# HKUST-Aerial-Robotics/MIND

Hardware: AMD Instinct MI355X
Metric: sim steps/sec (whole node) + scenario-tree nodes expanded/sec, AV2 demo scenes (higher is better)
Workload: dtype f32-class (bf16 hi+mid+lo split operands = 24 significand bits, six products, fp32 accumulate) pair kernel + ActorNet, f32 elsewhere in the predictor, f64 iLQR

## Files before the change

### include/mind_hip.h

```cpp
#ifndef MIND_HIP_H
#define MIND_HIP_H

#include <stddef.h>
#include <stdint.h>

#ifdef __cplusplus
extern "C" {
#endif

#define MIND_OK 0
#define MIND_EINVAL (-1)
#define MIND_ENOMEM (-2)
#define MIND_EHIP (-3)
#define MIND_ESTATE (-4)
#define MIND_ENOTFOUND (-5)

typedef struct mind_ctx mind_ctx;

int mind_ctx_create(int device, void *stream, mind_ctx **out);
int mind_ctx_destroy(mind_ctx *ctx);
const char *mind_last_error_string(mind_ctx *ctx);
int mind_ctx_synchronize(mind_ctx *ctx);

typedef struct {
// ... 31 lines not shown

int mind_predict_batch(mind_ctx *ctx, const mind_scene_batch *in, mind_pred_out *out);

typedef struct {
  float *cov_vel;
  float *param;
} mind_pred_aux;
int mind_predict_batch_aux(mind_ctx *ctx, const mind_scene_batch *in, mind_pred_out *out, const mind_pred_aux *aux);

#define MIND_BASIS_BEZIER 0
#define MIND_BASIS_MONOMIAL 1
int mind_set_decoder_basis(mind_ctx *ctx, int basis);
int mind_get_decoder_basis(mind_ctx *ctx);

#define MIND_CURVE_MAX_POINTS (1LL << 26)
int mind_curve_eval(mind_ctx *ctx, int basis, const float *param, long long n_rows, const double *tau, int n_tau,
                    float *reg, float *vel, float *cov_vel);
int mind_debug_curve_basis(int basis, const double *tau, int n_tau, float *T, float *Tp);

int mind_last_fusion_stats(mind_ctx *ctx, int *n_launches, float *total_ms, double *pairs_processed);
int mind_last_actor_stats(mind_ctx *ctx, int *layerwise, int *n_launches, int *n_chunks, float *total_ms);
int mind_last_token_stats(mind_ctx *ctx, int *layerwise, int *n_launches, int *n_chunks, float *total_ms);
int mind_last_token_stage_ms(mind_ctx *ctx, float *out_ms, int cap);
int mind_last_ilqr_stats(mind_ctx *ctx, float *kernel_ms, int *n_trees, int *workgroups_per_tree);
int mind_last_ilqr_profile(mind_ctx *ctx, double *out9);
int mind_last_ilqr_trace(mind_ctx *ctx, int tree, int phase, double *out, int cap_rows, int *n_rows);
int mind_set_profiling(mind_ctx *ctx, int enable);
int mind_debug_launch_times(mind_ctx *ctx, int kind, float *clock_ms, float *event_ms, int cap, int *n_clock, int *n_event);
int mind_debug_launch_clock(int n_blocks, int block_slots, int rate_khz, const long long *ops, int n_ops, const unsigned long long *stamps,
                            long long n_slots, double *out, int cap);

#define MIND_PAIR_F32 0
#define MIND_PAIR_BF16X3 1
#define MIND_PAIR_BF16 2
#define MIND_PAIR_BF16X6 3
int mind_set_pair_precision(mind_ctx *ctx, int mode);

int mind_set_tuning(mind_ctx *ctx, const char *name, int value);
int mind_get_pair_precision(mind_ctx *ctx);
int mind_debug_pack_bfrag(const float *w, int row_stride, uint32_t *out);

int mind_debug_pair_schedule(const int *scene_tokens, const int *scene_actors, int n_scenes, int n_cu, int last_layer, int *out_jobs, int cap,
                             int *out_info);

int mind_debug_predict_choice(const char *const *knob_names, const int *knob_values, int n_knobs, int pair_prec, int n_cu, int have_side,
                              const int *scene_actors, const int *scene_lanes, int n_scenes, long long *out, int cap);

int mind_debug_ilqr_plan(const char *const *knob_names, const int *knob_values, int n_knobs, int n_cu, int mode, int n_trees, const int *n_nodes,
                         const int32_t *parents, long long *out, int cap, int *bad);

int mind_debug_aime_book(int pred_len, int max_depth, int max_rounds, int n_agents, int world, int rank, int force, int n_rounds, const int *dec_len,
                         const float *dec, int n_tokens, int bytes_per_pair, int plan_chunk_mb, int per_scene, long long *out, int cap, char *msg,
                         int msg_cap);

int mind_debug_wait_word(const unsigned *word, unsigned want, double timeout_s, double (*clock)(void *user), void *user, int spins_per_look);

int mind_debug_actor_lw_plan(int n_actors, int np, int chunk, long long *out_launches, int cap, long long *out_info);

int mind_debug_token_lw_plan(int n_tokens, int mode, int chunk, long long *out_launches, int cap, long long *out_info);

int mind_debug_pack_conv_frag(const float *w, int co, int ci, int ksz, uint32_t *out, size_t cap);

int mind_debug_pack(const char *what, const float *w, int a, int b, int c, float *out, size_t cap);
int mind_debug_weight_image(const mind_tensor_desc *tensors, int n_tensors, float *blob, size_t blob_cap, char *names, size_t names_cap,
                            long long *entries, int entries_cap, long long *out_info, char *msg, int msg_cap);
int mind_debug_weight_bind(const mind_tensor_desc *tensors, int n_tensors, const char *drop, char *msg, int msg_cap);

int mind_debug_trig(mind_ctx *ctx, const double *x, int n, double *out);

int mind_debug_set_layers(mind_ctx *ctx, int n);
int64_t mind_debug_read(mind_ctx *ctx, const char *name, float *host, int64_t max_floats);

typedef struct {
  int n_nodes;
  const int32_t *parent;
  const float *prob;
  int n_agents;
  const float *agent_mean;
  const float *agent_cov;
  const double *field;
  const double *node_w;
} mind_cost_tree;

typedef struct {
  double dt, wheelbase;
  double w_des_state[6];
  double w_state_con[6];
  double state_lower[6], state_upper[6];
  double w_ctrl[2];
  double w_tgt, w_ego, w_ego_cov_offset, w_exo, w_exo_cov_offset, w_exo_cost_offset;
  double grid_res; int grid_w, grid_h;
  int max_iter;
} mind_ilqr_cfg;

typedef struct { int iterations; int converged; double J; double mu; } mind_ilqr_stats;

int mind_ilqr_solve_trees(mind_ctx *ctx, const mind_ilqr_cfg *cfg, const mind_cost_tree *trees,
                          int n_trees, const double *x0, const double *target_lane, int n_lane_pts,
                          double target_vel, int use_exo, const double *us_init, double *xs,
                          double *us, mind_ilqr_stats *stats);

int mind_ilqr_contingency(mind_ctx *ctx, const mind_ilqr_cfg *cfg_warm, const mind_ilqr_cfg *cfg_full,
                          const mind_cost_tree *trees, int n_trees, const double *x0,
                          const double *target_lane, int n_lane_pts, double target_vel, double *xs,
                          double *us, mind_ilqr_stats *stats_warm, mind_ilqr_stats *stats_full);
int mind_ilqr_contingency_begin(mind_ctx *ctx, const mind_ilqr_cfg *cfg_warm, const mind_ilqr_cfg *cfg_full,
// ... 339 lines not shown
```

### mind_amd/_lib.py

```python
import ctypes as C
import os

_HERE = os.path.dirname(os.path.abspath(__file__))
LIB_PATH = os.environ.get("MIND_HIP_LIB", os.path.join(_HERE, "libmind_hip.so"))

WAIT_CLOCK = C.CFUNCTYPE(C.c_double, C.c_void_p)
MIND_OK = 0
MIND_EINVAL, MIND_ENOMEM, MIND_EHIP, MIND_ESTATE, MIND_ENOTFOUND = -1, -2, -3, -4, -5


class TensorDesc(C.Structure):
    _fields_ = [("name", C.c_char_p), ("data", C.POINTER(C.c_float)), ("numel", C.c_int64)]


class SceneBatch(C.Structure):
    _fields_ = [("n_scenes", C.c_int), ("actor_off", C.POINTER(C.c_int32)), ("lane_off", C.POINTER(C.c_int32)),
                ("actors", C.c_void_p), ("lanes", C.c_void_p), ("lane_feat", C.c_void_p),
                ("actor_ctrs", C.c_void_p), ("actor_vecs", C.c_void_p), ("lane_ctrs", C.c_void_p),
                ("lane_vecs", C.c_void_p), ("rpe", C.POINTER(C.c_void_p)), ("tgt_nodes", C.c_void_p),
                ("tgt_rpe", C.c_void_p)]


class PredOut(C.Structure):
    _fields_ = [("cls", C.c_void_p), ("reg", C.c_void_p), ("vel", C.c_void_p), ("lane_feat", C.c_void_p),
# ... 139 lines not shown

class LoopDesc(C.Structure):
    _fields_ = [("n_tracks", C.c_int), ("n_steps", C.c_int), ("clamp_last", C.c_int), ("ego_state", C.c_void_p), ("ego_state_is_f32", C.c_int), ("ego_obs", C.c_void_p), ("ego_trig32", C.c_void_p),
                ("tan_fn", C.c_void_p), ("sincos_fn", C.c_void_p), ("exo_obs", C.c_void_p),
                ("exo_valid", C.c_void_p), ("timestep", C.c_void_p), ("type_slot", C.c_void_p),
                ("sim_step", C.c_double), ("plan_step", C.c_double), ("enable_time", C.c_double),
                ("wheelbase", C.c_double), ("max_speed", C.c_double), ("max_steer", C.c_double), ("max_acc", C.c_double), ("max_dec", C.c_double),
                ("n_lanes", C.c_int), ("lane_pts", C.c_void_p), ("lane_flags", C.c_void_p),
                ("n_lane_pts", C.c_int), ("target_lane", C.c_void_p), ("target_lane_info", C.c_void_p),
                ("time_ahead", C.c_double), ("min_vel", C.c_float), ("dist_thres", C.c_float), ("max_depth", C.c_int), ("max_rounds", C.c_int),
                ("pred_len", C.c_int), ("prob_floor", C.c_float),
                ("cfg_warm", C.c_void_p), ("cfg_full", C.c_void_p), ("solve_n_lane_pts", C.c_int), ("solve_lane", C.c_void_p), ("target_vel", C.c_double),
                ("eval_n_lane_pts", C.c_int), ("eval_lane_is_f32", C.c_int), ("eval_lane", C.c_void_p), ("speculative", C.c_int)]


class LoopTotals(C.Structure):
    _fields_ = [("plans", C.c_longlong), ("expansions", C.c_longlong), ("scen_trees", C.c_longlong), ("rounds", C.c_longlong),
                ("aime_s", C.c_double), ("ilqr_s", C.c_double), ("total_s", C.c_double),
                ("iterations", C.c_longlong), ("node_iterations", C.c_longlong), ("node_iterations_exo", C.c_longlong),
                ("warm_speculated", C.c_longlong), ("warm_hits", C.c_longlong),
                ("pair_ms", C.c_double), ("pair_launches", C.c_longlong), ("scene_n2", C.c_double), ("scene_n_a1", C.c_double),
                ("ilqr_ms", C.c_double), ("ilqr_launches", C.c_longlong), ("ilqr_trees", C.c_longlong), ("ilqr_workgroups_per_tree", C.c_int),
                ("ilqr_prof", C.c_double * 9), ("ilqr_node_steps", C.c_double)]


class LoopOut(C.Structure):
    _fields_ = [("planned", C.c_int), ("enabled", C.c_int), ("n_steps", C.c_longlong), ("n_plans", C.c_longlong), ("episode_steps", C.c_longlong),
                ("sim_time", C.c_double), ("last_trigger", C.c_double), ("state", C.c_double * 4), ("ctrl", C.c_double * 2),
                ("n_agents", C.c_int), ("n_trees", C.c_int), ("best", C.c_int), ("n_expanded", C.c_int), ("n_rounds", C.c_int), ("n_traj_nodes", C.c_int),
                ("costs", C.POINTER(C.c_double)), ("aime_s", C.c_double), ("ilqr_s", C.c_double), ("total_s", C.c_double),
                ("tot", LoopTotals)]


PLANNER_EGO_KEY = -(1 << 63)


class PlannerDesc(C.Structure):
    _fields_ = [("time_ahead", C.c_double), ("min_vel", C.c_float), ("dist_thres", C.c_float), ("max_depth", C.c_int), ("max_rounds", C.c_int),
                ("pred_len", C.c_int), ("prob_floor", C.c_float), ("cfg_warm", C.c_void_p), ("cfg_full", C.c_void_p), ("speculative", C.c_int),
                ("ego_type_slot", C.c_int)]


class PlannerOut(C.Structure):
    _fields_ = [("n_plans", C.c_longlong),
                ("n_agents", C.c_int), ("n_trees", C.c_int), ("best", C.c_int), ("n_expanded", C.c_int), ("n_rounds", C.c_int), ("n_traj_nodes", C.c_int),
                ("costs", C.POINTER(C.c_double)), ("ctrl", C.c_double * 2), ("aime_s", C.c_double), ("ilqr_s", C.c_double), ("total_s", C.c_double),
                ("tot", LoopTotals)]


EXPORTS = ["mind_ctx_create", "mind_ctx_destroy", "mind_last_error_string", "mind_ctx_synchronize",
           "mind_weights_load", "mind_predict_batch", "mind_last_fusion_stats", "mind_last_actor_stats", "mind_debug_actor_lw_plan", "mind_last_token_stats", "mind_last_token_stage_ms", "mind_debug_token_lw_plan", "mind_set_profiling", "mind_debug_launch_times", "mind_debug_launch_clock",
           "mind_ilqr_solve_trees", "mind_ilqr_contingency", "mind_ilqr_solve_fields", "mind_cost_eval", "mind_ilqr_score_trees", "mind_ilqr_gains", "mind_ilqr_policy_rollouts", "mind_lane_dist_field", "mind_aime_world", "mind_aime_rebase", "mind_debug_aime_decide", "mind_debug_set_layers",
           "mind_debug_read", "mind_set_pair_precision", "mind_get_pair_precision", "mind_debug_pack_bfrag", "mind_debug_pack_conv_frag", "mind_debug_pack", "mind_debug_weight_image", "mind_debug_weight_bind", "mind_debug_pair_schedule", "mind_debug_predict_choice", "mind_debug_ilqr_plan", "mind_debug_aime_book", "mind_set_tuning", "mind_last_ilqr_stats", "mind_aime_plan", "mind_last_ilqr_profile", "mind_eval_traj_trees", "mind_last_ilqr_trace", "mind_ilqr_contingency_begin", "mind_ilqr_finish", "mind_fill_tracks", "mind_ilqr_contingency_begin_plan", "mind_debug_trig", "mind_aime_plan_begin", "mind_aime_plan_poll", "mind_aime_plan_finish", "mind_ctx_busy", "mind_ilqr_finish_plan",
           "mind_set_exchange", "mind_last_exchange_stats", "mind_debug_wait_word",
           "mind_predict_batch_aux", "mind_set_decoder_basis", "mind_get_decoder_basis", "mind_curve_eval", "mind_debug_curve_basis",
           "mind_audit_plan", "mind_audit_episode", "mind_debug_box_clearance",
           "mind_forecast_score", "mind_debug_forecast_score",
           "mind_audit_road_plan", "mind_audit_road_episode", "mind_debug_road_margin",
           "mind_loop_create", "mind_loop_destroy", "mind_loop_reset", "mind_loop_advance", "mind_loop_state", "mind_loop_last_plan", "mind_loop_export",
           "mind_planner_create", "mind_planner_destroy", "mind_planner_reset", "mind_planner_observe", "mind_planner_set_lanes", "mind_planner_set_target_lane",
           "mind_planner_set_solve_lane", "mind_planner_set_eval_lane", "mind_planner_plan", "mind_planner_last_plan", "mind_planner_export"]

EXCHANGE_FN = C.CFUNCTYPE(C.c_int, C.c_void_p, C.c_int, C.c_void_p, C.c_void_p, C.c_int64)
XCHG_ALLGATHER, XCHG_ALLREDUCE, XCHG_ALLTOALLV = 0, 1, 2

_lib = None


def load():
    global _lib
    if _lib is not None:
        return _lib
    if not os.path.exists(LIB_PATH):
        raise ImportError(f"{LIB_PATH} is missing: the HIP extension must be built (hipcc --offload-arch=gfx950); "
                          "there is no CPU fallback for the product path")
    lib = C.CDLL(LIB_PATH)
    lib.mind_ctx_create.argtypes = [C.c_int, C.c_void_p, C.POINTER(C.c_void_p)]
    lib.mind_ctx_destroy.argtypes = [C.c_void_p]
    lib.mind_last_error_string.argtypes = [C.c_void_p]
    lib.mind_last_error_string.restype = C.c_char_p
    lib.mind_ctx_synchronize.argtypes = [C.c_void_p]
    lib.mind_weights_load.argtypes = [C.c_void_p, C.POINTER(TensorDesc), C.c_int]
    lib.mind_predict_batch.argtypes = [C.c_void_p, C.POINTER(SceneBatch), C.POINTER(PredOut)]
    lib.mind_predict_batch_aux.argtypes = [C.c_void_p, C.POINTER(SceneBatch), C.POINTER(PredOut), C.POINTER(PredAux)]
    lib.mind_set_decoder_basis.argtypes = [C.c_void_p, C.c_int]
    lib.mind_get_decoder_basis.argtypes = [C.c_void_p]
    lib.mind_curve_eval.argtypes = [C.c_void_p, C.c_int, C.c_void_p, C.c_longlong, C.POINTER(C.c_double), C.c_int, C.c_void_p, C.c_void_p, C.c_void_p]
    lib.mind_debug_curve_basis.argtypes = [C.c_int, C.POINTER(C.c_double), C.c_int, C.POINTER(C.c_float), C.POINTER(C.c_float)]
    lib.mind_last_fusion_stats.argtypes = [C.c_void_p, C.POINTER(C.c_int), C.POINTER(C.c_float), C.POINTER(C.c_double)]
    lib.mind_last_actor_stats.argtypes = [C.c_void_p, C.POINTER(C.c_int), C.POINTER(C.c_int), C.POINTER(C.c_int), C.POINTER(C.c_float)]
    lib.mind_debug_actor_lw_plan.argtypes = [C.c_int, C.c_int, C.c_int, C.POINTER(C.c_longlong), C.c_int, C.POINTER(C.c_longlong)]
    lib.mind_last_token_stats.argtypes = [C.c_void_p, C.POINTER(C.c_int), C.POINTER(C.c_int), C.POINTER(C.c_int), C.POINTER(C.c_float)]
    lib.mind_last_token_stage_ms.argtypes = [C.c_void_p, C.POINTER(C.c_float), C.c_int]
    lib.mind_debug_token_lw_plan.argtypes = [C.c_int, C.c_int, C.c_int, C.POINTER(C.c_longlong), C.c_int, C.POINTER(C.c_longlong)]
    lib.mind_set_profiling.argtypes = [C.c_void_p, C.c_int]
    lib.mind_debug_launch_times.argtypes = [C.c_void_p, C.c_int, C.POINTER(C.c_float), C.POINTER(C.c_float), C.c_int, C.POINTER(C.c_int), C.POINTER(C.c_int)]
    lib.mind_debug_launch_clock.argtypes = [C.c_int, C.c_int, C.c_int, C.POINTER(C.c_longlong), C.c_int, C.POINTER(C.c_ulonglong), C.c_longlong,
                                            C.POINTER(C.c_double), C.c_int]
    lib.mind_ilqr_solve_trees.argtypes = [C.c_void_p, C.POINTER(IlqrCfg), C.POINTER(CostTree), C.c_int,
                                          C.POINTER(C.c_double), C.POINTER(C.c_double), C.c_int, C.c_double, C.c_int,
                                          C.POINTER(C.c_double), C.POINTER(C.c_double), C.POINTER(C.c_double),
                                          C.POINTER(IlqrStats)]
    lib.mind_ilqr_contingency.argtypes = [C.c_void_p, C.POINTER(IlqrCfg), C.POINTER(IlqrCfg), C.POINTER(CostTree), C.c_int,
                                          C.POINTER(C.c_double), C.POINTER(C.c_double), C.c_int, C.c_double,
                                          C.POINTER(C.c_double), C.POINTER(C.c_double), C.POINTER(IlqrStats), C.POINTER(IlqrStats)]
    lib.mind_ilqr_contingency_begin.argtypes = [C.c_void_p, C.POINTER(IlqrCfg), C.POINTER(IlqrCfg), C.POINTER(CostTree), C.c_int,
                                          C.POINTER(C.c_double), C.POINTER(C.c_double), C.c_int, C.c_double,
                                          C.POINTER(C.c_double), C.POINTER(C.c_double), C.POINTER(IlqrStats), C.POINTER(IlqrStats)]
    lib.mind_ilqr_finish.argtypes = [C.c_void_p]
    lib.mind_ilqr_contingency_begin_plan.argtypes = [C.c_void_p, C.POINTER(IlqrCfg), C.POINTER(IlqrCfg), C.c_void_p, C.c_void_p, C.c_int, C.c_double,
                                                     C.c_void_p, C.c_void_p, C.c_void_p, C.c_void_p]
    lib.mind_fill_tracks.argtypes = [C.c_void_p, C.c_int, C.c_int, C.c_void_p, C.c_void_p, C.c_void_p, C.c_void_p, C.c_void_p, C.c_void_p]
    lib.mind_ilqr_solve_fields.argtypes = [C.c_void_p, C.POINTER(IlqrCfg), C.POINTER(FieldGrid), C.POINTER(CostTree), C.c_int,
                                           C.POINTER(C.c_double), C.POINTER(C.c_double), C.POINTER(C.c_double),
                                           C.POINTER(C.c_double), C.POINTER(IlqrStats)]
    lib.mind_cost_eval.argtypes = [C.c_void_p, C.POINTER(IlqrCfg), C.POINTER(FieldGrid), C.POINTER(CostTree),
                                   C.POINTER(C.c_double), C.POINTER(C.c_double), C.c_int, C.c_double, C.c_int, C.c_int,
                                   C.POINTER(C.c_int32), C.POINTER(C.c_double), C.POINTER(C.c_double), C.POINTER(C.c_double)]
    lib.mind_ilqr_score_trees.argtypes = [C.c_void_p, C.POINTER(IlqrCfg), C.POINTER(FieldGrid), C.POINTER(CostTree), C.c_int,
                                          C.POINTER(C.c_double), C.POINTER(C.c_double), C.c_int, C.c_double, C.c_int, C.c_int,
                                          C.POINTER(C.c_double), C.POINTER(C.c_double), C.POINTER(C.c_double), C.POINTER(C.c_double)]
    lib.mind_ilqr_gains.argtypes = [C.c_void_p, C.POINTER(IlqrCfg), C.POINTER(FieldGrid), C.POINTER(CostTree), C.c_int,
                                    C.POINTER(C.c_double), C.POINTER(C.c_double), C.c_int, C.c_double, C.c_int,
                                    C.POINTER(C.c_double), C.POINTER(C.c_double), C.POINTER(IlqrGainsOut)]
    lib.mind_ilqr_policy_rollouts.argtypes = [C.c_void_p, C.POINTER(IlqrCfg), C.POINTER(FieldGrid), C.POINTER(CostTree), C.c_int,
                                              C.POINTER(C.c_double), C.POINTER(C.c_double), C.c_int, C.c_double, C.c_int,
                                              C.POINTER(C.c_double), C.POINTER(C.c_double), C.POINTER(C.c_double), C.c_int,
                                              C.POINTER(C.c_double), C.POINTER(C.c_double), C.POINTER(C.c_double), C.POINTER(C.c_double),
                                              C.POINTER(C.c_double), C.POINTER(C.c_double)]
    lib.mind_lane_dist_field.argtypes = [C.c_void_p, C.POINTER(C.c_double), C.POINTER(C.c_double), C.c_int, C.c_int, C.c_int,
                                         C.c_double] + [C.POINTER(C.c_double)] * 4
    lib.mind_aime_world.argtypes = [C.c_void_p, C.POINTER(WorldIn), C.POINTER(WorldOut)]
    lib.mind_aime_rebase.argtypes = [C.c_void_p, C.POINTER(RebaseIn), C.POINTER(RebaseOut)]
    lib.mind_debug_aime_decide.argtypes = [C.c_void_p, C.c_int, C.POINTER(C.c_int32), C.POINTER(C.c_int32), C.c_void_p, C.POINTER(C.c_float), C.c_void_p,
                                           C.c_void_p, C.c_void_p, C.c_int, C.c_float, C.c_float, C.c_int, C.c_int, C.c_void_p, C.c_void_p, C.c_void_p]
    lib.mind_aime_plan.argtypes = [C.c_void_p, C.POINTER(AimePlanIn), C.POINTER(AimePlanOut)]
    lib.mind_aime_plan_begin.argtypes = [C.c_void_p, C.POINTER(AimePlanIn)]
    lib.mind_aime_plan_poll.argtypes = [C.c_void_p]
    lib.mind_aime_plan_finish.argtypes = [C.c_void_p, C.POINTER(AimePlanOut)]
    lib.mind_ctx_busy.argtypes = [C.c_void_p]
    lib.mind_ilqr_finish_plan.argtypes = [C.c_void_p, C.c_int, C.c_int, C.c_void_p, C.c_void_p, C.c_void_p, C.c_void_p]
    lib.mind_set_pair_precision.argtypes = [C.c_void_p, C.c_int]
    lib.mind_set_tuning.argtypes = [C.c_void_p, C.c_char_p, C.c_int]
    lib.mind_last_ilqr_stats.argtypes = [C.c_void_p, C.POINTER(C.c_float), C.POINTER(C.c_int), C.POINTER(C.c_int)]
    lib.mind_last_ilqr_profile.argtypes = [C.c_void_p, C.POINTER(C.c_double)]
    lib.mind_last_ilqr_trace.argtypes = [C.c_void_p, C.c_int, C.c_int, C.POINTER(C.c_double), C.c_int, C.POINTER(C.c_int)]
    lib.mind_eval_traj_trees.argtypes = [C.POINTER(C.c_double), C.POINTER(C.c_double), C.POINTER(C.c_int32), C.c_int, C.c_void_p, C.c_int, C.c_int,
                                         C.c_double, C.POINTER(C.c_double)]
    lib.mind_get_pair_precision.argtypes = [C.c_void_p]
    lib.mind_debug_pack_bfrag.argtypes = [C.POINTER(C.c_float), C.c_int, C.POINTER(C.c_uint32)]
    lib.mind_debug_pair_schedule.argtypes = [C.POINTER(C.c_int), C.POINTER(C.c_int), C.c_int, C.c_int, C.c_int, C.POINTER(C.c_int), C.c_int, C.POINTER(C.c_int)]
    lib.mind_debug_predict_choice.argtypes = [C.POINTER(C.c_char_p), C.POINTER(C.c_int), C.c_int, C.c_int, C.c_int, C.c_int, C.POINTER(C.c_int), C.POINTER(C.c_int),
                                              C.c_int, C.POINTER(C.c_longlong), C.c_int]
    lib.mind_debug_ilqr_plan.argtypes = [C.POINTER(C.c_char_p), C.POINTER(C.c_int), C.c_int, C.c_int, C.c_int, C.c_int, C.POINTER(C.c_int), C.POINTER(C.c_int32),
                                         C.POINTER(C.c_longlong), C.c_int, C.POINTER(C.c_int)]
    lib.mind_debug_wait_word.argtypes = [C.POINTER(C.c_uint), C.c_uint, C.c_double, WAIT_CLOCK, C.c_void_p, C.c_int]
    lib.mind_debug_aime_book.argtypes = [C.c_int] * 8 + [C.POINTER(C.c_int), C.POINTER(C.c_float)] + [C.c_int] * 4 + [C.POINTER(C.c_longlong), C.c_int, C.c_char_p, C.c_int]
    lib.mind_debug_trig.argtypes = [C.c_void_p, C.POINTER(C.c_double), C.c_int, C.POINTER(C.c_double)]
    lib.mind_debug_pack_conv_frag.argtypes = [C.POINTER(C.c_float), C.c_int, C.c_int, C.c_int, C.POINTER(C.c_uint32), C.c_size_t]
    lib.mind_debug_pack.argtypes = [C.c_char_p, C.POINTER(C.c_float), C.c_int, C.c_int, C.c_int, C.POINTER(C.c_float), C.c_size_t]
    lib.mind_debug_weight_image.argtypes = [C.POINTER(TensorDesc), C.c_int, C.POINTER(C.c_float), C.c_size_t, C.c_char_p, C.c_size_t,
                                            C.POINTER(C.c_longlong), C.c_int, C.POINTER(C.c_longlong), C.c_char_p, C.c_int]
    lib.mind_debug_weight_bind.argtypes = [C.POINTER(TensorDesc), C.c_int, C.c_char_p, C.c_char_p, C.c_int]
    lib.mind_debug_set_layers.argtypes = [C.c_void_p, C.c_int]
    lib.mind_debug_read.argtypes = [C.c_void_p, C.c_char_p, C.POINTER(C.c_float), C.c_int64]
    lib.mind_set_exchange.argtypes = [C.c_void_p, C.c_int, C.c_int, EXCHANGE_FN, C.c_void_p, C.c_int]
    lib.mind_last_exchange_stats.argtypes = [C.c_void_p, C.POINTER(C.c_longlong), C.POINTER(C.c_longlong)]
    lib.mind_loop_create.argtypes = [C.c_void_p, C.POINTER(LoopDesc), C.POINTER(C.c_void_p)]
    lib.mind_loop_destroy.argtypes = [C.c_void_p]
    lib.mind_loop_reset.argtypes = [C.c_void_p]
    lib.mind_loop_advance.argtypes = [C.c_void_p, C.c_int, C.c_double, C.c_longlong, C.POINTER(LoopOut)]
    lib.mind_loop_state.argtypes = [C.c_void_p, C.POINTER(LoopOut)]
    lib.mind_loop_last_plan.argtypes = [C.c_void_p, C.POINTER(AimePlanOut)] + [C.POINTER(C.c_void_p)] * 6 + [C.c_void_p]
    lib.mind_loop_export.argtypes = [C.c_void_p, C.c_int, C.POINTER(C.c_int), C.c_void_p, C.c_void_p, C.c_void_p]
    lib.mind_planner_create.argtypes = [C.c_void_p, C.POINTER(PlannerDesc), C.POINTER(C.c_void_p)]
    lib.mind_planner_destroy.argtypes = [C.c_void_p]
    lib.mind_planner_reset.argtypes = [C.c_void_p]
    lib.mind_planner_observe.argtypes = [C.c_void_p, C.c_int, C.c_void_p, C.c_int, C.c_void_p, C.c_void_p, C.c_void_p]
    lib.mind_planner_set_lanes.argtypes = [C.c_void_p, C.c_int, C.c_void_p, C.c_void_p]
    lib.mind_planner_set_target_lane.argtypes = [C.c_void_p, C.c_int, C.c_void_p, C.c_void_p]
    lib.mind_planner_set_solve_lane.argtypes = [C.c_void_p, C.c_int, C.c_void_p, C.c_double]
    lib.mind_planner_set_eval_lane.argtypes = [C.c_void_p, C.c_int, C.c_void_p, C.c_int]
    lib.mind_planner_plan.argtypes = [C.c_void_p, C.c_void_p, C.c_void_p, C.POINTER(PlannerOut)]
    lib.mind_planner_last_plan.argtypes = [C.c_void_p, C.POINTER(AimePlanOut)] + [C.POINTER(C.c_void_p)] * 6 + [C.c_void_p]
    lib.mind_planner_export.argtypes = [C.c_void_p, C.c_int, C.POINTER(C.c_int), C.c_void_p, C.c_void_p, C.c_void_p]
    lib.mind_audit_plan.argtypes = [C.c_void_p, C.POINTER(AuditBox), C.c_double, C.POINTER(CostTree), C.c_int, C.c_int, C.POINTER(C.c_double),
                                    C.POINTER(AuditPlanOut)]
    lib.mind_audit_episode.argtypes = [C.c_void_p, C.POINTER(AuditBox), C.c_int, C.c_int, C.c_int, C.POINTER(C.c_double), C.POINTER(C.c_double),
                                       C.POINTER(C.c_uint8), C.POINTER(C.c_double), C.POINTER(AuditEpisodeOut)]
    lib.mind_debug_box_clearance.argtypes = [C.c_int, C.c_int, C.POINTER(C.c_double), C.POINTER(C.c_double), C.POINTER(C.c_double), C.POINTER(C.c_double)]
    fc_tail = [C.POINTER(ForecastCfg), C.c_int, C.POINTER(C.c_int32), C.c_void_p, C.c_void_p, C.POINTER(C.c_double), C.POINTER(C.c_uint8),
               C.POINTER(C.c_uint8), C.POINTER(ForecastOut)]
    lib.mind_forecast_score.argtypes = [C.c_void_p] + fc_tail
    lib.mind_debug_forecast_score.argtypes = fc_tail
    road = [C.POINTER(C.c_double), C.POINTER(C.c_int32), C.c_int]
    lib.mind_audit_road_plan.argtypes = [C.c_void_p, C.POINTER(AuditBox)] + road + [C.POINTER(CostTree), C.c_int, C.c_int, C.POINTER(C.c_double),
                                                                                   C.POINTER(AuditRoadPlanOut)]
    lib.mind_audit_road_episode.argtypes = [C.c_void_p, C.POINTER(AuditBox)] + road + [C.c_int, C.c_int, C.POINTER(C.c_double),
                                                                                      C.POINTER(AuditRoadEpisodeOut)]
    lib.mind_debug_road_margin.argtypes = [C.c_int, C.POINTER(C.c_double), C.POINTER(AuditBox)] + road + [C.POINTER(C.c_double), C.POINTER(C.c_double)] + \
        [C.POINTER(C.c_int32)] * 3
    for n in EXPORTS:
        getattr(lib, n)
        if n not in ("mind_last_error_string", "mind_debug_read"):
            getattr(lib, n).restype = C.c_int
    lib.mind_debug_read.restype = C.c_int64
    _lib = lib
    return lib


# ... 282 lines not shown
```

### mind_amd/csrc/actor_mfma_kernels.hip

```cpp
#include <hip/hip_runtime.h>
#include <stdint.h>

#define AM_T 1024
#ifdef MIND_ACTOR_TRACE
__device__ long long am_tr_[64];
__device__ int am_trn_;
#define AM_MARK() do { if (blockIdx.x == 0 && threadIdx.x == 0) { const long long n_ = clock64(); am_tr_[am_trn_ & 63] = n_; ++am_trn_; } } while (0)
#else
#define AM_MARK() do {} while (0)
#endif
#define AM_WAVES 16
#define AM_MAXT 2
#define AM_RSD(C) (3 * (C) / 2 + 4)
#define AM_BUF 2496
#define AM_XIN 0
#define AM_O0 1344
#define AM_FA (AM_O0 + 7 * AM_BUF)
#define AM_RED (AM_FA + 48 * AM_RSD(128))
#define AM_LDS_DWORDS (AM_RED + 64)

#include "weight_tables.h"
#include "launch_clock.h"
typedef u32 u32x2 __attribute__((ext_vector_type(2)));

// ... 136 lines not shown
#pragma unroll
      for (int e = 0; e < 4; ++e) y[e] += (1.0f - l1) * a0[e] + l1 * a1[e];
    }
    if (relu) {
#pragma unroll
      for (int e = 0; e < 4; ++e) y[e] = fmaxf(y[e], 0.f);
    }
    if (gout) {
      if (t == Tout - 1) *(f32x4 *)(gout + co) = y;
    } else if (outf) {
      *(f32x4 *)(outf + t * 132 + co) = y;
    } else {
      am_store_split<NP>(outs + t * RSD + (co >> 1), PLANE, y);
    }
  }
  __syncthreads();
}

template <int NP, int LGCI, int LGCO, int STRIDE, bool DS>
__device__ __forceinline__ void am_res(const u32 *in, int Tin, const AmRes &W, u32 *out, u32 *t1, u32 *t2, float *red) {
  constexpr int Cout = 1 << LGCO;
  const int Tout = Tin / STRIDE;
  f32x4 acc[AM_MAXT];
  am_conv<NP, LGCI, 3, STRIDE>(in, Tin, W.c1, Cout, Tout, acc);
  AM_MARK();
  am_gn<NP>(acc, Cout, Tout, W.g1, W.b1, nullptr, nullptr, true, t1, nullptr, nullptr, red);
  AM_MARK();
  const u32 *resid = in;
  if (DS) {
    am_conv<NP, LGCI, 1, STRIDE>(in, Tin, W.ds, Cout, Tout, acc);
    AM_MARK();
    am_gn<NP>(acc, Cout, Tout, W.gd, W.bd, nullptr, nullptr, false, t2, nullptr, nullptr, red);
    AM_MARK();
    resid = t2;
  }
  am_conv<NP, LGCO, 3, 1>(t1, Tout, W.c2, Cout, Tout, acc);
  AM_MARK();
  am_gn<NP>(acc, Cout, Tout, W.g2, W.b2, resid, nullptr, true, out, nullptr, nullptr, red);
  AM_MARK();
}

template <int NP, int LGC>
__device__ __forceinline__ void am_lateral(const u32 *src, int T, const AmLat &W, const float *up, float *dstf, u32 *dsts,
                                           float *red) {
  f32x4 acc[AM_MAXT];
  am_conv<NP, LGC, 3, 1>(src, T, W.w, 128, T, acc);
  AM_MARK();
  am_gn<NP>(acc, 128, T, W.g, W.b, nullptr, up, false, dsts, dstf, nullptr, red);
  AM_MARK();
}

template <int NP>
__global__ __launch_bounds__(AM_T) void k_actor_mfma(const float *__restrict__ actors , int n_actors,
                                                     float *__restrict__ out , AmW W, LcSlot *clk) {
  lc_stamp_in(clk);
  extern __shared__ __attribute__((aligned(16))) u32 smu[];
  u32 *xin = smu + AM_XIN;
  u32 *o0 = smu + AM_O0, *o1 = o0 + AM_BUF, *o2 = o1 + AM_BUF, *o3 = o2 + AM_BUF;
  u32 *ta = o3 + AM_BUF, *tb = ta + AM_BUF, *tc = tb + AM_BUF;
  u32 *fa = smu + AM_FA;
  float *red = (float *)(smu + AM_RED);
  const int tid = threadIdx.x;
  const int a = blockIdx.x;
  if (a >= n_actors) { lc_stamp_both(clk); return; }
  if (tid < 48 * 8) {
    const int t = tid >> 3, c = (tid & 7) * 2;
    const float v0 = c < 14 ? actors[((size_t)a * 14 + c) * 48 + t] : 0.f;
    const float v1 = c + 1 < 14 ? actors[((size_t)a * 14 + c + 1) * 48 + t] : 0.f;
    u32 *p = xin + t * AM_RSD(16) + (c >> 1);
    const u32 h = pk_bf16(v0, v1);
    const float r0 = v0 - bf_lo_f32(h), r1 = v1 - bf_hi_f32(h);
    const u32 m = pk_bf16(r0, r1);
    p[0] = h; p[8] = m; p[16] = pk_bf16(r0 - bf_lo_f32(m), r1 - bf_hi_f32(m));
  }
  __syncthreads();
#ifdef MIND_ACTOR_TRACE
  if (blockIdx.x == 0 && tid == 0) am_trn_ = 0;
#endif
  AM_MARK();
  am_res<NP, 4, 5, 1, true>(xin, 48, W.res[0], ta, tb, tc, red);
  am_res<NP, 5, 5, 1, false>(ta, 48, W.res[1], o0, tb, tc, red);
  am_res<NP, 5, 6, 2, true>(o0, 48, W.res[2], ta, tb, tc, red);
  am_res<NP, 6, 6, 1, false>(ta, 24, W.res[3], o1, tb, tc, red);
  am_res<NP, 6, 7, 2, true>(o1, 24, W.res[4], ta, tb, tc, red);
  am_res<NP, 7, 7, 1, false>(ta, 12, W.res[5], o2, tb, tc, red);
  am_res<NP, 7, 8, 2, true>(o2, 12, W.res[6], ta, tb, tc, red);
  am_res<NP, 8, 8, 1, false>(ta, 6, W.res[7], o3, tb, tc, red);
  am_lateral<NP, 8>(o3, 6, W.lat[3], nullptr, (float *)ta, nullptr, red);
  am_lateral<NP, 7>(o2, 12, W.lat[2], (const float *)ta, (float *)tb, nullptr, red);
  am_lateral<NP, 6>(o1, 24, W.lat[1], (const float *)tb, (float *)o2, nullptr, red);
  am_lateral<NP, 5>(o0, 48, W.lat[0], (const float *)o2, nullptr, fa, red);
  {
    const AmRes &R = W.res[8];
    f32x4 acc[AM_MAXT];
    am_conv<NP, 7, 3, 1>(fa, 48, R.c1, 128, 48, acc);
    AM_MARK();
    am_gn<NP>(acc, 128, 48, R.g1, R.b1, nullptr, nullptr, true, o0, nullptr, nullptr, red);
    AM_MARK();
    am_conv<NP, 7, 3, 1>(o0, 48, R.c2, 128, 48, acc);
    AM_MARK();
    am_gn<NP>(acc, 128, 48, R.g2, R.b2, fa, nullptr, true, nullptr, nullptr, out + (size_t)a * 128, red);
    AM_MARK();
  }
#ifdef MIND_ACTOR_TRACE
  if (blockIdx.x == 0 && tid == 0) {
    printf("[k_actor_mfma<%d>] cycles conv/gn per stage:", NP);
    for (int q = 1; q < am_trn_ && q < 64; ++q) printf(" %lld", am_tr_[q] - am_tr_[q - 1]);
// ... 7 lines not shown
```

### mind_amd/csrc/aime_book.h

```cpp
#pragma once
#include <algorithm>
#include <cstddef>
#include <cstdint>
#include <cstring>
#include <vector>

#include "../../include/mind_hip.h"

constexpr int PL_K = 6;
constexpr int PL_OBS = 50;

struct PlScene {
  int node;
  float prob;
  int cur_t, end_t;
  float rot[4], orig[2], tgt[22];
};

struct PlNode {
  int round, scene, mode, parent, depth;
  int owner, lscene;
  float prob;
  int cur_t, end_t;
  bool branch, end, term, rebased;
  unsigned long long hit;
  float tgt[22];
};

inline void pl_block(int n, int r, int w, int &lo, int &hi) {
  const int base = n / w, rem = n % w;
  lo = r * base + (r < rem ? r : rem);
  hi = lo + base + (r < rem ? 1 : 0);
}
inline int pl_owner(int n, int w, int b) {
  for (int r = 0; r < w; ++r) { int lo, hi; pl_block(n, r, w, lo, hi); if (b >= lo && b < hi) return r; }
  return w - 1;
}

inline bool pl_exchanges(bool have_transport, int world, bool force) { return have_transport && (world > 1 || force); }

inline int pl_chunk(int n_tokens, int bytes_per_pair, int plan_chunk_mb, int Bk) {
  const double edge_mb = (double)n_tokens * (((n_tokens + 15) / 16) * 16) * bytes_per_pair / (1024.0 * 1024.0);
  return std::max(1, (int)std::min<double>((double)(Bk > 0 ? Bk : 1), (double)plan_chunk_mb / edge_mb));
}

typedef double (*pl_clock_fn)(void *user);
inline bool pl_wait_word(const volatile unsigned *word, unsigned want, double timeout_s, pl_clock_fn now, void *user, unsigned spins_per_look) {
  if (__atomic_load_n((const unsigned *)word, __ATOMIC_ACQUIRE) == want) return true;
  const double t0 = now(user);
  for (unsigned spins = 0;;) {
    if (__atomic_load_n((const unsigned *)word, __ATOMIC_ACQUIRE) == want) return true;
    if (++spins < spins_per_look) continue;
    spins = 0;
    if (now(user) - t0 > timeout_s) return false;
  }
}

enum { PL_OK = 0, PL_E_ROUNDS, PL_E_ROOT, PL_E_TRIMMED, PL_E_AGAIN, PL_E_ORDER, PL_E_NO_END };
struct PlErr { int code = PL_OK, a0 = 0, a1 = 0; explicit operator bool() const { return code != PL_OK; } };
inline const char *pl_err_format(int code) {
  switch (code) {
    case PL_E_ROUNDS: return "unsupported: more than %d AIME rounds";
    case PL_E_ROOT: return "unsupported: the root is a branching candidate";
// ... 75 lines not shown
};

struct PlGeom { int B, lo, hi, Bk, Bmax; };

struct PlRound {
  std::vector<int> todo;
  std::vector<int> cnt_r, s0_r;
  std::vector<int> win;
  int S = 0, s0 = 0, Sm = 0;
};

struct AimeBook {
  int HZ = 0, max_depth = 0, a = 0, XW = 1, XR = 0;
  bool dist = false;
  int n_rounds = 0;
  std::vector<PlNode> nodes;
  std::vector<int> leaves;
  std::vector<PlScene> batch;
  PlRound rec;
  std::vector<mind_aime_node> table;
  int64_t n_rows = 0;
  JobTable gather, flat;
  std::vector<int32_t> tree_top, tree_off, flat_parent;
  std::vector<float> flat_prob;
  std::vector<int> cand, queue, last, stack;
  std::vector<std::vector<int>> kids;
  std::vector<float> pr;

  AimeBook() {}
  AimeBook(int pred_len, int max_depth_, int n_agents, int world, int rank, bool dist_) { reset(pred_len, max_depth_, n_agents, world, rank, dist_); }

  void reset(int pred_len, int max_depth_, int n_agents, int world, int rank, bool dist_) {
    HZ = pred_len; max_depth = max_depth_; a = n_agents; XW = world; XR = rank; dist = dist_;
    n_rounds = 0;
    nodes.assign(1, PlNode());
    PlNode &r = nodes[0];
    memset(&r, 0, sizeof(r));
    r.round = -1; r.parent = -1; r.prob = 1.f; r.end_t = HZ; r.branch = true;
    leaves.assign(1, 0);
    batch.assign(1, PlScene());
    PlScene &s = batch[0];
    s.node = 0; s.prob = 1.f; s.cur_t = 0; s.end_t = HZ;
    tree_top.clear();
  }

  PlErr begin_round(int max_rounds, PlGeom &g) const {
    PlErr e;
    if (n_rounds >= max_rounds) { e.code = PL_E_ROUNDS; e.a0 = max_rounds; return e; }
    g.B = (int)batch.size();
    pl_block(g.B, XR, XW, g.lo, g.hi);
    g.Bk = g.hi - g.lo;
    g.Bmax = (g.B + XW - 1) / XW;
    return e;
  }

  static int flags_of(const PlNode &n) { return (n.branch ? MIND_AIME_BRANCH : 0) | (n.end ? MIND_AIME_END : 0) | (n.term ? MIND_AIME_TERMINATE : 0); }
  int root_flags() const { return flags_of(nodes[0]); }

  PlErr round(const float *h_dec, int Bmax) {
    PlErr err;
    const int B = (int)batch.size(), round = n_rounds;
    const size_t n_back = (size_t)Bmax * 6 * 4;
    for (int b = 0; b < B; ++b) {
      const int owner = dist ? pl_owner(B, XW, b) : 0;
      int olo, ohi;
      pl_block(B, owner, XW, olo, ohi);
      if (!dist) { olo = 0; }
      const float *h_sel = h_dec + (size_t)owner * n_back, *h_selp = h_sel + (size_t)Bmax * 6;
      const unsigned *h_hit = (const unsigned *)(h_selp + (size_t)Bmax * 6);
      const int bl = b - olo;
      for (int j = 0; j < PL_K; ++j) {
        const int k = (int)h_sel[(size_t)bl * 6 + j];
        if (k < 0) continue;
        PlNode n;
        memset(&n, 0, sizeof(n));
        n.round = round; n.scene = b; n.mode = k; n.parent = batch[b].node; n.depth = nodes[n.parent].depth + 1;
        n.owner = owner; n.lscene = bl;
        n.prob = h_selp[(size_t)bl * 6 + j]; n.cur_t = batch[b].cur_t; n.end_t = batch[b].end_t;
        n.hit = (unsigned long long)h_hit[2 * ((size_t)bl * 6 + j)] | ((unsigned long long)h_hit[2 * ((size_t)bl * 6 + j) + 1] << 32);
        memcpy(n.tgt, batch[b].tgt, sizeof(n.tgt));
        const int idx = (int)nodes.size();
        nodes.push_back(n);
        for (size_t q = 0; q < leaves.size(); ++q)
          if (leaves[q] == n.parent) { leaves.erase(leaves.begin() + q); break; }
        leaves.push_back(idx);
      }
    }
    n_rounds += 1;
    std::vector<int> &todo = rec.todo;
    cand.clear(); todo.clear();
    for (int li : leaves) {
      PlNode &n = nodes[li];
      if (n.branch) { n.branch = false; n.term = true; }
      else if (!n.end) {
        if (n.depth >= max_depth) n.term = true;
        else cand.push_back(li);
      }
    }
    for (int li : cand) {
      PlNode &n = nodes[li];
      if (li == 0) { err.code = PL_E_ROOT; return err; }
      if (n.rebased && n.cur_t > 0) { err.code = PL_E_TRIMMED; return err; }
      int t_b = n.end_t;
      for (int t = n.cur_t + 1 + (n.cur_t + 1) % 2; t < n.end_t; t += 2)
        if ((n.hit >> t) & 1ull) { t_b = t; break; }
      if (t_b < n.end_t) n.end_t = t_b;
      if (t_b < HZ) todo.push_back(li);
      else n.end = true;
    }
    const int S = rec.S = (int)todo.size();
    rec.cnt_r.assign(XW, 0); rec.s0_r.assign(XW + 1, 0); rec.win.clear();
    rec.s0 = rec.Sm = 0;
    if (todo.empty()) return err;
    for (int li : todo)
      if (nodes[li].round != round) { err.code = PL_E_AGAIN; err.a0 = nodes[li].round; err.a1 = round + 1; return err; }
    for (int s = 0; s < S; ++s) {
      if (s > 0 && nodes[todo[s]].scene < nodes[todo[s - 1]].scene) { err.code = PL_E_ORDER; return err; }
      rec.cnt_r[nodes[todo[s]].owner] += 1;
    }
    for (int r = 0; r < XW; ++r) rec.s0_r[r + 1] = rec.s0_r[r] + rec.cnt_r[r];
    const int s0 = rec.s0 = rec.s0_r[XR], Sm = rec.Sm = rec.cnt_r[XR];
    rec.win.resize(3 * (size_t)Sm);
    for (int s = 0; s < Sm; ++s) {
      const PlNode &n = nodes[todo[s0 + s]];
      rec.win[s] = n.scene;
      rec.win[Sm + s] = n.lscene * a * PL_K + n.mode;
      rec.win[2 * Sm + s] = n.end_t - n.cur_t;
    }
    batch.assign(S, PlScene());
    for (int s = 0; s < S; ++s) {
      PlNode &n = nodes[todo[s]];
      n.branch = true; n.rebased = true;
      PlScene &sc = batch[s];
      sc.node = todo[s]; sc.prob = n.prob; sc.cur_t = n.end_t; sc.end_t = HZ;
    }
    return err;
  }

  PlErr finish() {
    PlErr err;
    bool any_end = false;
    for (int li : leaves) any_end |= nodes[li].end;
    if (!any_end) { err.code = PL_E_NO_END; return err; }
    for (int li : leaves) {
      if (!nodes[li].end) continue;
      for (int q = li; q > 0; q = nodes[q].parent) nodes[q].end = true;
    }
    const int N = (int)nodes.size() - 1;
    table.assign(N, mind_aime_node());
    gather.clear(); flat.clear();
    n_rows = 0;
    for (int i = 0; i < N; ++i) {
      const PlNode &n = nodes[i + 1];
      mind_aime_node &p = table[i];
      p.round = n.round; p.scene = n.scene; p.mode = n.mode; p.parent = n.parent - 1; p.prob = n.prob; p.cur_t = n.cur_t; p.end_t = n.end_t;
      p.flags = flags_of(n);
      memcpy(p.tgt_pts, n.tgt, sizeof(p.tgt_pts));
      p.dur = 0; p.row_off = -1;
      if (n.end) {
        const int dur = n.end_t - n.cur_t;
        p.dur = dur; p.row_off = n_rows;
        if (dur > 0 && (!dist || n.owner == XR))
          gather.add({n.lscene * a * PL_K + n.mode, dur, (int)n_rows, a}, n.round);
        n_rows += (int64_t)a * dur * 3;
      }
    }
    if (kids.size() < nodes.size()) kids.resize(nodes.size());
    for (size_t i = 0; i < nodes.size(); ++i) kids[i].clear();
    for (int i = 1; i < (int)nodes.size(); ++i) kids[nodes[i].parent].push_back(i);
    tree_top.clear(); tree_off.assign(1, 0); flat_parent.clear(); flat_prob.clear();
    for (int top : kids[0]) {
      if (!nodes[top].end) continue;
      pr.assign(nodes.size(), 0.f);
      pr[top] = 1.f;
      queue.assign(1, top);
      for (size_t qh = 0; qh < queue.size(); ++qh) {
        const int cur = queue[qh];
        float total = 0.f;
        for (int ch : kids[cur]) if (nodes[ch].end) total = total + nodes[ch].prob;
        for (int ch : kids[cur]) if (nodes[ch].end) { pr[ch] = nodes[ch].prob / total * pr[cur]; queue.push_back(ch); }
// ... 30 lines not shown
```

### mind_amd/csrc/aime_kernels.hip

```cpp
#include <hip/hip_runtime.h>
#include <stdint.h>

struct AimeScene {
  int a0, a1;
  int last, cmp;
  float r00, r01, r10, r11;
  float ox, oy, theta_g, pad2;
};

#define AIME_SMALL 8
struct AimeSmall {
  AimeScene s[AIME_SMALL];
  float prob[AIME_SMALL];
  int n, a, pad0, pad1;
};

#define AIME_T 60
#define AIME_K 6
#define AIME_PK 6

__device__ __forceinline__ void aime_to_world(float lx, float ly, float c, float s, float cx, float cy, const AimeScene &S,
                                              bool translate, float &wx, float &wy) {
  float ax = lx * c + ly * (-s), ay = lx * s + ly * c;
  if (translate) { ax += cx; ay += cy; }
  wx = ax * S.r00 + ay * S.r01;
  wy = ax * S.r10 + ay * S.r11;
  if (translate) { wx += S.ox; wy += S.oy; }
}

__global__ __launch_bounds__(64) void k_aime_world(const AimeScene *__restrict__ scenes, const int *__restrict__ agent_scene,
                                                   const float *__restrict__ reg, const float *__restrict__ vel,
                                                   const float *__restrict__ ctrs, const float *__restrict__ vecs,
                                                   const float *__restrict__ cov_last, float *__restrict__ world,
                                                   float *__restrict__ topo, float *__restrict__ ego_end,
                                                   const float *__restrict__ lane, int n_lane, const AimeSmall sm) {
  const int i = blockIdx.x / AIME_K, k = blockIdx.x % AIME_K, t = threadIdx.x;
  const int b = sm.n ? i / sm.a : agent_scene[i];
  const AimeScene S = sm.n ? sm.s[b] : scenes[b];
  const bool live = t < AIME_T;
  const int tc = live ? t : AIME_T - 1;
  const float th = atan2f(vecs[2 * i + 1], vecs[2 * i]);
  const float c = cosf(th), s = sinf(th);
  const size_t e = ((size_t)i * AIME_K + k) * AIME_T + tc;
  const float lx = reg[e * 5], ly = reg[e * 5 + 1], sgx = reg[e * 5 + 2], sgy = reg[e * 5 + 3];
  const float lvx = vel[e * 2], lvy = vel[e * 2 + 1];
  float wx, wy, wvx, wvy;
  aime_to_world(lx, ly, c, s, ctrs[2 * i], ctrs[2 * i + 1], S, true, wx, wy);
  aime_to_world(lvx, lvy, c, s, 0.f, 0.f, S, false, wvx, wvy);
  const float ang = atan2f(lvy, lvx) + th + S.theta_g;
  const float cv = fmaxf(sgx, sgy) + cov_last[i];
  if (live) {
    float *w = world + e * AIME_PK;
    w[0] = wx; w[1] = wy; w[2] = wvx; w[3] = wvy; w[4] = ang; w[5] = cv;
  }
// ... 90 lines not shown
    int best = -1, brank = AIME_K;
    float bp = 0.f;
    unsigned brow = 0;
#pragma unroll
    for (int k = 0; k < AIME_K; ++k)
      if (((alive >> k) & 1u) && rank[k] < brank) {
        best = k; brank = rank[k]; bp = pr[k];
        unsigned row = 0;
#pragma unroll
        for (int j = 0; j < AIME_K; ++j) {
          const int lo = k < j ? k : j, hi = k < j ? j : k;
          if (j != k && ((mask >> (lo * AIME_K + hi)) & 1u)) row |= 1u << j;
        }
        brow = row;
      }
    if (best >= 0) {
#pragma unroll
      for (int q = 0; q < AIME_K; ++q) if (q == ns) { so[q] = (float)best; po[q] = bp; }
      ++ns;
      alive &= brow;
    }
  }
}

__global__ __launch_bounds__(64) void k_aime_select(const AimeScene *__restrict__ scenes, const float *__restrict__ cls,
                                                    const float *__restrict__ scen_prob, const float *__restrict__ topo,
                                                    const float *__restrict__ ego_end, int lane_check, float dist_thres,
                                                    float *__restrict__ sel, float *__restrict__ sel_prob, float prob_floor, const AimeSmall sm) {
  const int b = blockIdx.x, t = threadIdx.x;
  const AimeScene S = sm.n ? sm.s[b] : scenes[b];
  const float sp = sm.n ? sm.prob[b] : scen_prob[b];
  float so[AIME_K], po[AIME_K];
  aime_select_scene(S, sp, b, t, cls, topo, ego_end, lane_check, dist_thres, prob_floor, so, po);
  if (t != 0) return;
#pragma unroll
  for (int k = 0; k < AIME_K; ++k) { sel[(size_t)b * AIME_K + k] = so[k]; sel_prob[(size_t)b * AIME_K + k] = po[k]; }
}

#define RB_THREADS 256
#define RB_FEAT_BLOCKS(a) ((int)(((size_t)(a) * 48 + RB_THREADS - 1) / RB_THREADS))
#define RB_T 50
#define RB_LANE_LDS 1024

struct RebaseArgs {
  int a, l, n_lane, pad_ones;
  const float *pos, *ang, *vel;
  const float *types;
  const float *pad;
  const float *lane_ctrs0, *lane_vecs0;
  const float *tlane, *tinfo;
  float time_ahead, min_vel;
  float *actors, *actor_ctrs, *actor_vecs, *lane_ctrs, *lane_vecs, *tgt_nodes, *tgt_rpe, *frames;
  float travel0;
};

__device__ __forceinline__ void rb_cs(float ax, float ay, float bx, float by, float &c, float &s) {
  const float den = sqrtf(ax * ax + ay * ay) * sqrtf(bx * bx + by * by) + 1e-10f;
  c = (ax * bx + ay * by) / den;
  s = (ax * by - ay * bx) / den;
}

__global__ __launch_bounds__(64) void k_aime_windows(const float *__restrict__ prev_pos, const float *__restrict__ prev_ang,
                                                     const float *__restrict__ prev_vel, const float *__restrict__ rows,
                                                     const int *__restrict__ parent_slot, const int *__restrict__ row0,
                                                     const int *__restrict__ dur, int a, float *__restrict__ pos,
                                                     float *__restrict__ ang, float *__restrict__ vel, int row_stride,
                                                     float *__restrict__ cov_last) {
  const int s = blockIdx.x / a, i = blockIdx.x - s * a, t = threadIdx.x;
  if (t >= RB_T) return;
  const int d = dur[s];
  const int src = t + d;
  float x, y, vx, vy, h;
  if (src < RB_T) {
    const size_t p = ((size_t)parent_slot[s] * a + i) * RB_T + src;
    x = prev_pos[2 * p]; y = prev_pos[2 * p + 1]; vx = prev_vel[2 * p]; vy = prev_vel[2 * p + 1]; h = prev_ang[p];
  } else {
    const float *r = rows + (((size_t)row0[s] + (size_t)i * row_stride) * AIME_T + (src - RB_T)) * AIME_PK;
    x = r[0]; y = r[1]; vx = r[2]; vy = r[3]; h = r[4];
    if (cov_last && t == RB_T - 1) cov_last[(size_t)s * a + i] = r[5];
  }
  const size_t o = ((size_t)s * a + i) * RB_T + t;
  pos[2 * o] = x; pos[2 * o + 1] = y; vel[2 * o] = vx; vel[2 * o + 1] = vy; ang[o] = h;
}

struct AimeDone { unsigned *cnt; unsigned *h_gen; unsigned gen; };
__device__ __forceinline__ void aime_decisions_done(const AimeDone D) {
  if (!D.h_gen) return;
  __threadfence_system();
  const unsigned prev = __hip_atomic_fetch_add(D.cnt, 1u, __ATOMIC_ACQ_REL, __HIP_MEMORY_SCOPE_AGENT);
  if (prev + 1u != gridDim.x) return;
  __hip_atomic_store(D.cnt, 0u, __ATOMIC_RELAXED, __HIP_MEMORY_SCOPE_AGENT);
  __threadfence_system();
  __hip_atomic_store(D.h_gen, D.gen, __ATOMIC_RELEASE, __HIP_MEMORY_SCOPE_SYSTEM);
}

__global__ __launch_bounds__(64) void k_aime_branch(const AimeScene *__restrict__ scenes, const float *__restrict__ sel,
                                                    const float *__restrict__ world, unsigned *__restrict__ hit,
                                                    const float *__restrict__ sel_prob, float *__restrict__ h_sel, float *__restrict__ h_selp,
                                                    unsigned *__restrict__ h_hit, const AimeSmall sm, const AimeDone done) {
  const int b = blockIdx.x / AIME_K, j = blockIdx.x % AIME_K, t = threadIdx.x;
  const AimeScene S = sm.n ? sm.s[b] : scenes[b];
  const int k = (int)sel[(size_t)b * AIME_K + j];
  bool h = false;
  if (k >= 0 && t < AIME_T) {
    for (int i = S.a0; i < S.a1; ++i) {
      const float *r = world + ((size_t)i * AIME_K + k) * AIME_T * AIME_PK;
      h |= (r[t * AIME_PK + 5] / r[S.cmp * AIME_PK + 5]) > 9.0f;
    }
  }
  const unsigned long long m = __ballot(h);
  if (t == 0) { hit[2 * (size_t)blockIdx.x] = (unsigned)m; hit[2 * (size_t)blockIdx.x + 1] = (unsigned)(m >> 32); }
  if (h_sel && t == 0) {
    h_hit[2 * (size_t)blockIdx.x] = (unsigned)m; h_hit[2 * (size_t)blockIdx.x + 1] = (unsigned)(m >> 32);
    h_sel[blockIdx.x] = sel[blockIdx.x]; h_selp[blockIdx.x] = sel_prob[blockIdx.x];
    aime_decisions_done(done);
  }
}

__global__ __launch_bounds__(64) void k_aime_select_branch(const AimeScene *__restrict__ scenes, const float *__restrict__ cls,
                                                           const float *__restrict__ scen_prob, const float *__restrict__ topo,
                                                           const float *__restrict__ ego_end, int lane_check, float dist_thres, float prob_floor,
                                                           const float *__restrict__ world, float *__restrict__ sel, float *__restrict__ sel_prob,
                                                           unsigned *__restrict__ hit, float *__restrict__ h_sel, float *__restrict__ h_selp,
                                                           unsigned *__restrict__ h_hit, const AimeSmall sm, const AimeDone done) {
  const int b = blockIdx.x / AIME_K, j = blockIdx.x % AIME_K, t = threadIdx.x;
  const AimeScene S = sm.n ? sm.s[b] : scenes[b];
  const float sp = sm.n ? sm.prob[b] : scen_prob[b];
  float so[AIME_K], po[AIME_K];
  aime_select_scene(S, sp, b, t, cls, topo, ego_end, lane_check, dist_thres, prob_floor, so, po);
  float kf = -1.f, pj = 0.f;
#pragma unroll
  for (int q = 0; q < AIME_K; ++q) if (q == j) { kf = so[q]; pj = po[q]; }
  const int k = (int)kf;
  bool h = false;
  if (k >= 0 && t < AIME_T) {
    for (int i0 = S.a0; i0 < S.a1; i0 += 8) {
      float num[8], den[8];
#pragma unroll
      for (int q = 0; q < 8; ++q) {
        const int i = i0 + q < S.a1 ? i0 + q : S.a1 - 1;
        const float *r = world + ((size_t)i * AIME_K + k) * AIME_T * AIME_PK;
        num[q] = r[t * AIME_PK + 5]; den[q] = r[S.cmp * AIME_PK + 5];
      }
#pragma unroll
      for (int q = 0; q < 8; ++q) if (i0 + q < S.a1) h |= (num[q] / den[q]) > 9.0f;
    }
  }
  const unsigned long long m = __ballot(h);
  if (t == 0) {
    hit[2 * (size_t)blockIdx.x] = (unsigned)m; hit[2 * (size_t)blockIdx.x + 1] = (unsigned)(m >> 32);
    sel[blockIdx.x] = kf; sel_prob[blockIdx.x] = pj;
    if (h_sel) {
      h_hit[2 * (size_t)blockIdx.x] = (unsigned)m; h_hit[2 * (size_t)blockIdx.x + 1] = (unsigned)(m >> 32);
      h_sel[blockIdx.x] = kf; h_selp[blockIdx.x] = pj;
      aime_decisions_done(done);
    }
  }
}

struct AimeGather { int row0, dur, dst, a; };
__global__ __launch_bounds__(64) void k_aime_gather(const AimeGather *__restrict__ jobs, const int *__restrict__ job_of_block,
                                                    const int *__restrict__ agent_of_block, const float *const *__restrict__ world_of_job,
                                                    float *__restrict__ out) {
  const AimeGather J = jobs[job_of_block[blockIdx.x]];
  const int i = agent_of_block[blockIdx.x], t = threadIdx.x;
  if (t >= J.dur) return;
  const float *r = world_of_job[job_of_block[blockIdx.x]] + (((size_t)J.row0 + (size_t)i * AIME_K) * AIME_T + t) * AIME_PK;
  float *o = out + (size_t)J.dst + ((size_t)i * J.dur + t) * 3;
  o[0] = r[0]; o[1] = r[1]; o[2] = r[5];
}

struct AimeFlat { int row0, n, dst, a; };
__global__ __launch_bounds__(64) void k_aime_flat(const AimeFlat *__restrict__ jobs, const int *__restrict__ job_of_block,
                                                  const int *__restrict__ agent_of_block, const float *const *__restrict__ world_of_job,
                                                  float *__restrict__ mean, float *__restrict__ cov) {
  const AimeFlat J = jobs[job_of_block[blockIdx.x]];
  const int i = agent_of_block[blockIdx.x], m = threadIdx.x;
  if (m >= J.n) return;
  const float *r = world_of_job[job_of_block[blockIdx.x]] + (((size_t)J.row0 + (size_t)i * AIME_K) * AIME_T + 2 * m) * AIME_PK;
  const size_t o = (size_t)(J.dst + m) * J.a + i;
  mean[2 * o] = r[0]; mean[2 * o + 1] = r[1];
  cov[o] = r[5];
}

__global__ void k_repeat_rows(const float *__restrict__ src, size_t n, int times, float *__restrict__ dst) {
  const size_t i = (size_t)blockIdx.x * blockDim.x + threadIdx.x;
  if (i >= n * (size_t)times) return;
  dst[i] = src[i % n];
}

__global__ __launch_bounds__(RB_THREADS) void k_aime_rebase(RebaseArgs A) {
  const int sc = blockIdx.x, tid = threadIdx.x;
  const int a = A.a;
  extern __shared__ float rb_sm[];
  __shared__ float fr[8];
  __shared__ float rdv[RB_THREADS];
  __shared__ int rdi[RB_THREADS];
  __shared__ int s_idx;
  __shared__ float ctr[11][2];
  const float *pos = A.pos + (size_t)sc * a * RB_T * 2;
  const float *ang = A.ang + (size_t)sc * a * RB_T;
  const float *vel = A.vel + (size_t)sc * a * RB_T * 2;
  if (tid == 0) {
    const float th = ang[RB_T - 1];
    fr[0] = pos[(RB_T - 1) * 2]; fr[1] = pos[(RB_T - 1) * 2 + 1]; fr[2] = th; fr[3] = cosf(th); fr[4] = sinf(th);
  }
  __syncthreads();
  const float ox = fr[0], oy = fr[1], th0 = fr[2], c0 = fr[3], s0 = fr[4];
  for (int i = tid; i < a; i += RB_THREADS) {
    const float dx = pos[(i * RB_T + RB_T - 1) * 2] - ox, dy = pos[(i * RB_T + RB_T - 1) * 2 + 1] - oy;
    const float cx = dx * c0 + dy * s0, cy = dx * (-s0) + dy * c0;
    const float thi = ang[i * RB_T + RB_T - 1] - th0;
    const float ci = cosf(thi), si = sinf(thi);
    float *o = rb_sm + 5 * i;
    o[0] = cx; o[1] = cy; o[2] = thi; o[3] = ci; o[4] = si;
    if (blockIdx.y == 0) {
      A.actor_ctrs[((size_t)sc * a + i) * 2] = cx; A.actor_ctrs[((size_t)sc * a + i) * 2 + 1] = cy;
      A.actor_vecs[((size_t)sc * a + i) * 2] = ci; A.actor_vecs[((size_t)sc * a + i) * 2 + 1] = si;
    }
  }
  __syncthreads();
  const int fb = (int)blockIdx.y - 1, nfb = (int)gridDim.y - 1;
  for (int e = (nfb > 0 ? fb * RB_THREADS : 0) + tid; nfb > 0 ? (fb >= 0 && e < min(a * 48, (fb + 1) * RB_THREADS)) : e < a * 48; e += RB_THREADS) {
    const int i = e / 48, t = e % 48 + 2;
    const float *f = rb_sm + 5 * i;
    float pn[2][2];
#pragma unroll
    for (int q = 0; q < 2; ++q) {
      const int tt = t - 1 + q;
      const float dx = pos[(i * RB_T + tt) * 2] - ox, dy = pos[(i * RB_T + tt) * 2 + 1] - oy;
      const float x1 = (dx * c0 + dy * s0) - f[0], y1 = (dx * (-s0) + dy * c0) - f[1];
      pn[q][0] = x1 * f[3] + y1 * f[4];
      pn[q][1] = x1 * (-f[4]) + y1 * f[3];
    }
    const float an = (ang[i * RB_T + t] - th0) - f[2];
    const float vx0 = vel[(i * RB_T + t) * 2], vy0 = vel[(i * RB_T + t) * 2 + 1];
    const float vx1 = vx0 * c0 + vy0 * s0, vy1 = vx0 * (-s0) + vy0 * c0;
    float *o = A.actors + ((size_t)sc * a + i) * 14 * 48 + (t - 2);
    o[0 * 48] = pn[1][0] - pn[0][0];
    o[1 * 48] = pn[1][1] - pn[0][1];
    o[2 * 48] = cosf(an);
    o[3 * 48] = sinf(an);
    o[4 * 48] = vx1 * f[3] + vy1 * f[4];
    o[5 * 48] = vx1 * (-f[4]) + vy1 * f[3];
#pragma unroll
    for (int k = 0; k < 7; ++k) o[(6 + k) * 48] = A.types[(i * RB_T + t) * 7 + k];
// ... 184 lines not shown
```

### mind_amd/csrc/aime_plan.hip

```cpp
#include <chrono>
namespace {

int pl_pin(mind_ctx *c, int which, size_t bytes) {
  if (bytes <= c->pl_pin_cap[which]) return MIND_OK;
  if (c->pl_pin[which]) (void)hipHostFree(c->pl_pin[which]);
  c->pl_pin[which] = nullptr; c->pl_pin_cap[which] = 0;
  const size_t want = bytes < ((size_t)64 << 20) ? std::max<size_t>(2 * bytes, (size_t)1 << 20) : bytes + bytes / 2 + 4096;
  if (hipHostMalloc(&c->pl_pin[which], want, hipHostMallocDefault) != hipSuccess)
    return fail(c, MIND_ENOMEM, "hipHostMalloc(%zu) failed", want);
  c->pl_pin_cap[which] = want;
  return MIND_OK;
}

struct CopySeg { const float *src; float *dst; long long n; };
__global__ __launch_bounds__(256) void k_copy_segs(const CopySeg *__restrict__ segs) {
  const CopySeg S = segs[blockIdx.y];
  const long long i0 = (long long)blockIdx.x * 2048 + threadIdx.x;
#pragma unroll
  for (int k = 0; k < 8; ++k) {
    const long long i = i0 + k * 256;
    if (i < S.n) S.dst[i] = S.src[i];
  }
}

// ... 25 lines not shown
  if ((rc = pl_pin(c, 6, segs.size() * sizeof(CopySeg)))) return rc;
  memcpy(c->pl_pin[6], segs.data(), segs.size() * sizeof(CopySeg));
  HIPCHK(c, hipMemcpyAsync(c->x_seg.p, c->pl_pin[6], segs.size() * sizeof(CopySeg), hipMemcpyHostToDevice, c->stream));
  hipLaunchKernelGGL(k_copy_segs, dim3((unsigned)((mx + 2047) / 2048), (unsigned)segs.size()), dim3(256), 0, c->stream, (const CopySeg *)c->x_seg.p);
  HIPCHK(c, hipGetLastError());
  return MIND_OK;
}

static_assert(PL_K == AIME_K && PL_OBS == RB_T, "aime_book.h restates the kernels' constants");
static_assert(sizeof(PlJob) == sizeof(AimeGather) && sizeof(PlJob) == sizeof(AimeFlat) && offsetof(PlJob, row0) == offsetof(AimeGather, row0) &&
                  offsetof(PlJob, row0) == offsetof(AimeFlat, row0) && offsetof(PlJob, n) == offsetof(AimeGather, dur) && offsetof(PlJob, n) == offsetof(AimeFlat, n) &&
                  offsetof(PlJob, dst) == offsetof(AimeGather, dst) && offsetof(PlJob, dst) == offsetof(AimeFlat, dst) && offsetof(PlJob, a) == offsetof(AimeGather, a) &&
                  offsetof(PlJob, a) == offsetof(AimeFlat, a), "JobTable holds the packing kernels' job records");

struct PlTrace {
  std::chrono::steady_clock::time_point t0 = std::chrono::steady_clock::now();
  void operator()(const char *what) const {
    static const bool on = getenv("MIND_PLAN_TRACE") != nullptr;
    if (on) fprintf(stderr, "[plan] %8.1f us  %s\n", std::chrono::duration<double, std::micro>(std::chrono::steady_clock::now() - t0).count(), what);
  }
};

double pl_steady_now(void *) { return std::chrono::duration<double>(std::chrono::steady_clock::now().time_since_epoch()).count(); }

struct PlanRun {
  mind_ctx *c;
  const mind_aime_plan_in *in;
  mind_aime_plan_out *out;
  hipStream_t st;
  AimeBook &book;
  const int a, l, P, HZ;
  const bool raw;
  const int XW, XR;
  const bool dist;
  const RootLayout ro;
  const float *droot = nullptr;
  int cur_in = -1;
  const float *prev_pos = nullptr, *prev_ang = nullptr, *prev_vel = nullptr, *cov_last_dev = nullptr;
  bool frames_pending = false;
  int n_expanded = 0, pair_launches = 0;
  int lc_n = 0;
  PlGeom g = {0, 0, 0, 0, 0};
  int chunk = 1;
  bool all_small = false, tables_done = false;
  size_t bS = 0, bI = 0, bP = 0, tab_bytes = 0, n_back = 0;
  DevBuf *tabb = nullptr;
  float *d_topo = nullptr, *d_ego = nullptr, *d_sel = nullptr, *d_selp = nullptr, *h_mirror = nullptr, *d_world = nullptr;
  unsigned *d_hit = nullptr;
  unsigned *h_gen = nullptr, want_gen = 0;
  int round_no = 0;
  int nxt = 0;
  InLayout q{0, 0, 0};
  float *d_in = nullptr, *w_pos = nullptr, *w_ang = nullptr, *w_vel = nullptr;
  bool want_solves = false, solves_tried = false;
  int solves_rc = MIND_OK;
  PlTrace TR;

  PlanRun(mind_ctx *c_, const mind_aime_plan_in *in_, mind_aime_plan_out *out_)
      : c(c_), in(in_), out(out_), st(c_->stream), book(c_->plan.book), a(in_->n_agents), l(in_->n_lanes), P(in_->n_lane_pts), HZ(in_->pred_len),
        raw(in_->raw_pos != nullptr), XW(c_->xfn ? c_->xw : 1), XR(c_->xfn ? c_->xr : 0), dist(pl_exchanges(c_->xfn != nullptr, c_->xw, c_->xforce)),
        ro(in_->n_agents, in_->n_lanes, in_->n_lane_pts, in_->raw_pos != nullptr) {}
  bool solves_asked() const { return in->solve_cfg_full && in->solve_x0 && in->solve_lane && in->solve_n_lane_pts >= 2 && !dist; }
  int fail_book(const PlErr &e) const { return fail(c, MIND_ESTATE, pl_err_format(e.code), e.a0, e.a1); }
  int pl_root(), pl_root_raw(), pl_root_host(), pl_presize_next();
  int pl_round_buffers(int round), pl_round_launch(), pl_round_tables(), pl_round_decisions(const float *&h_dec);
  int pl_predict_chunk(int g0, int cb, float *d_cls, float *d_reg, float *d_vel, const float *&d_ctrs, const float *&d_vecs);
  int pl_rebase_next(), pl_exchange_next(int round), pl_next_inputs(), pl_pack_results(), pl_hand_out();
  void pl_begin_solves();
  int pl_side_hop(hipStream_t &rs), pl_frames_back(const float *d_fr, size_t S, hipStream_t rs);
  template <class Layout> RebaseArgs pl_rebase_args(float *base, const Layout &q, size_t s0, int l) const;
};

int PlanRun::pl_side_hop(hipStream_t &rs) {
  rs = st;
  if (c->side && !dist) {
    if (!c->ev_root) HIPCHK(c, hipEventCreateWithFlags(&c->ev_root, hipEventDisableTiming));
    HIPCHK(c, hipEventRecord(c->ev_root, st));
    HIPCHK(c, hipStreamWaitEvent(c->side, c->ev_root, 0));
    rs = c->side;
  }
  return MIND_OK;
}

int PlanRun::pl_frames_back(const float *d_fr, size_t S, hipStream_t rs) {
  int rc;
  if ((rc = pl_pin(c, 3, S * 28 * sizeof(float)))) return rc;
  HIPCHK(c, hipMemcpyAsync(c->pl_pin[3], d_fr, S * 28 * sizeof(float), hipMemcpyDeviceToHost, rs));
  HIPCHK(c, hipEventRecord(c->ev_pl, rs));
  frames_pending = true;
  return MIND_OK;
}

template <class Layout>
RebaseArgs PlanRun::pl_rebase_args(float *base, const Layout &q, size_t s0, int l) const {
  RebaseArgs R;
  R.a = a; R.l = l; R.n_lane = P;
  R.types = droot + ro.types; R.tlane = droot + ro.tl; R.tinfo = droot + ro.ti;
  R.time_ahead = in->time_ahead; R.min_vel = in->min_vel;
  R.actors = base + q.actors + s0 * a * 14 * 48; R.actor_ctrs = base + q.ctrs + s0 * a * 2; R.actor_vecs = base + q.vecs + s0 * a * 2;
  R.lane_ctrs = l ? base + q.lc + s0 * l * 2 : nullptr; R.lane_vecs = l ? base + q.lv + s0 * l * 2 : nullptr;
  R.tgt_nodes = base + q.tn + s0 * 160; R.tgt_rpe = base + q.tr + s0 * 20; R.frames = base + q.fr + s0 * 28;
  return R;
}

int pl_check(mind_ctx *c, const mind_aime_plan_in *in) {
  if (!c->have_weights) return fail(c, MIND_ESTATE, "weights not loaded");
  if (c->il_finish) {
    if (!c->il_finish_owned)
      return fail(c, MIND_ESTATE, "mind_aime_plan: a tree-iLQR call begun with mind_ilqr_contingency_begin is pending on this context (mind_ilqr_finish first)");
    (void)mind_ilqr_finish(c);
    c->pl_sol_xs.clear(); c->pl_sol_us.clear(); c->pl_sol_stw.clear(); c->pl_sol_stf.clear();
  }
  const bool raw = in->raw_pos != nullptr;
  if (in->n_agents <= 0 || in->n_lanes <= 0 || in->n_lane_pts < 12 || !in->types || !in->target_lane || !in->target_lane_info ||
      (raw ? (!in->raw_ang || !in->raw_vel || !in->raw_pad || !in->lane_pts || !in->lane_flags || !(in->travel0 >= 0.f))
           : (!in->actors || !in->actor_ctrs || !in->actor_vecs || !in->lanes || !in->lane_ctrs || !in->lane_vecs || !in->tgt_nodes ||
              !in->tgt_rpe || !in->rot || !in->orig || !in->tgt_pts || !in->hist)) || in->max_depth < 0 || in->max_rounds <= 0 || in->max_rounds > 32 || in->pred_len < 2 || in->pred_len > AIME_T)
    return fail(c, MIND_EINVAL, "mind_aime_plan: bad argument");
  if (in->script_cls && (!in->script_reg || !in->script_vel)) return fail(c, MIND_EINVAL, "mind_aime_plan: scripted modes need cls, reg and vel");
// ... 85 lines not shown
    const auto field = [this]() { return il_field_prepare(c, in->solve_cfg_full, in->solve_x0, in->solve_lane, in->solve_n_lane_pts, c->pl_copy); };
    if (c->enc_post) {
      const std::function<int(hipStream_t)> hist = std::move(c->enc_post);
      c->enc_post = [hist, field](hipStream_t rs) { const int rc_ = hist(rs); return rc_ ? rc_ : field(); };
    } else if ((rc = field())) return rc;
  }
  prev_pos = droot + ro.wpos; prev_ang = droot + ro.wang; prev_vel = droot + ro.wvel;
  cov_last_dev = droot + ro.cov;
  return MIND_OK;
}

int PlanRun::pl_round_buffers(int round) {
  const int Bk = g.Bk, Bmax = g.Bmax, A = Bk * a;
  int rc;
  const size_t n_topo = ((size_t)A * 6 + 3) & ~(size_t)3, n_ego = (size_t)Bk * 24;
  n_back = (size_t)Bmax * 6 * 4;
  if ((rc = ensure(c, c->pl_small, (n_topo + n_ego + n_back) * sizeof(float)))) return rc;
  d_topo = (float *)c->pl_small.p; d_ego = d_topo + n_topo; d_sel = d_ego + n_ego; d_selp = d_sel + (size_t)Bmax * 6;
  d_hit = (unsigned *)(d_selp + (size_t)Bmax * 6);
  h_mirror = nullptr; h_gen = nullptr;
  round_no = round;
  if (!dist && c->dec_mirror) {
    if ((rc = pl_pin(c, 2, n_back * sizeof(float) + 64))) return rc;
    h_mirror = (float *)c->pl_pin[2];
  }
  tabb = &c->pl_tab[round & 1];
  bS = ((size_t)Bk * sizeof(AimeScene) + 15) & ~(size_t)15; bI = ((size_t)A * sizeof(int) + 15) & ~(size_t)15;
  bP = ((size_t)Bk * sizeof(float) + 15) & ~(size_t)15;
  tab_bytes = bS + bI + bP;
  if ((rc = ensure(c, *tabb, tab_bytes + 3 * (size_t)6 * Bmax * sizeof(int) + 64))) return rc;
  if ((rc = pl_pin(c, 1, tab_bytes + 3 * (size_t)6 * Bmax * sizeof(int) + 64))) return rc;
  if ((int)c->pl_world.size() <= round) c->pl_world.resize(round + 1);
  d_world = nullptr;
  chunk = pl_chunk(a + l + 1, pred_edge_pair_bytes(c->pt, c->pair_prec), c->plan_chunk_mb, Bk);
  if (Bk > 0) {
    if ((rc = ensure(c, c->pl_world[round], (size_t)A * 6 * AIME_T * 6 * sizeof(float)))) return rc;
    d_world = (float *)c->pl_world[round].p;
    const int cbm = std::min(chunk, Bk);
    const size_t n_cls = ((size_t)cbm * 6 + 3) & ~(size_t)3;
    if ((rc = ensure(c, c->pl_pred, (n_cls + (size_t)cbm * a * 6 * AIME_T * 7) * sizeof(float)))) return rc;
  }
  tables_done = false;
  all_small = c->tab_small && std::min(chunk, std::max(Bk, 1)) <= AIME_SMALL;
  if (h_mirror && c->dec_poll && Bk > 0 && chunk >= Bk) {
    if (!c->pl_cnt.p) {
      if ((rc = ensure(c, c->pl_cnt, 64))) return rc;
      HIPCHK(c, hipMemsetAsync(c->pl_cnt.p, 0, 64, st));
    }
    h_gen = (unsigned *)(h_mirror + n_back);
    if (++c->dec_gen == 0u) c->dec_gen = 1u;
    want_gen = c->dec_gen;
    __atomic_store_n(h_gen, 0u, __ATOMIC_RELEASE);
  }
  return MIND_OK;
}

int PlanRun::pl_round_tables() {
  std::vector<PlScene> &batch = book.batch;
  const int Bk = g.Bk;
  tables_done = true;
  if (frames_pending) {
    HIPCHK(c, hipEventSynchronize(c->ev_pl));
    const float *fr = (const float *)c->pl_pin[3];
    for (int b = 0; b < g.B; ++b) {
      memcpy(batch[b].rot, fr + (size_t)b * 28, 4 * sizeof(float));
      memcpy(batch[b].orig, fr + (size_t)b * 28 + 4, 2 * sizeof(float));
      memcpy(batch[b].tgt, fr + (size_t)b * 28 + 6, 22 * sizeof(float));
    }
    frames_pending = false;
  }
  if (Bk <= 0) return MIND_OK;
  char *h = (char *)c->pl_pin[1];
  AimeScene *hs = (AimeScene *)h;
  int *as = (int *)(h + bS);
  float *sp = (float *)(h + bS + bI);
  for (int b = 0; b < Bk; ++b) {
    AimeScene &S = hs[b];
    const PlScene &q = batch[g.lo + b];
    const int bc = b % chunk;
    S.a0 = a * bc; S.a1 = a * (bc + 1); S.last = HZ - 1;      S.cmp = q.cur_t == 0 ? 1 : q.cur_t; S.pad2 = 0.f;
    S.r00 = q.rot[0]; S.r01 = q.rot[1]; S.r10 = q.rot[2]; S.r11 = q.rot[3];
    S.ox = q.orig[0]; S.oy = q.orig[1];
    S.theta_g = atan2f(S.r10, S.r00);
    for (int i = 0; i < a; ++i) as[(size_t)b * a + i] = bc;
    sp[b] = q.prob;
  }
  if (all_small) {
  } else if (c->pl_tab_side) {
    HIPCHK(c, hipMemcpyAsync(tabb->p, h, tab_bytes, hipMemcpyHostToDevice, c->pl_copy));
    HIPCHK(c, hipEventRecord(c->ev_tab, c->pl_copy));
    HIPCHK(c, hipStreamWaitEvent(st, c->ev_tab, 0));
  } else {
    HIPCHK(c, hipMemcpyAsync(tabb->p, h, tab_bytes, hipMemcpyHostToDevice, st));
  }
  return MIND_OK;
}

int PlanRun::pl_predict_chunk(int g0, int cb, float *d_cls, float *d_reg, float *d_vel, const float *&d_ctrs, const float *&d_vecs) {
  std::vector<int32_t> ao(cb + 1), lof(cb + 1);
  for (int b = 0; b <= cb; ++b) { ao[b] = a * b; lof[b] = l * b; }
  mind_scene_batch sb;
  memset(&sb, 0, sizeof(sb));
  mind_pred_out po;
  memset(&po, 0, sizeof(po));
  sb.n_scenes = cb; sb.actor_off = ao.data(); sb.lane_off = lof.data();
  if (cur_in < 0) {
    const RootLayout &o = ro;
    sb.actors = droot + o.actors; sb.lanes = droot + o.lanes; sb.actor_ctrs = d_ctrs = droot + o.ctrs; sb.actor_vecs = d_vecs = droot + o.vecs;
    sb.lane_ctrs = droot + o.lc; sb.lane_vecs = droot + o.lv; sb.tgt_nodes = droot + o.tn; sb.tgt_rpe = droot + o.tr;
    po.lane_feat = (float *)c->pl_lf.p;
  } else {
    const InLayout q(g.B, a, l);
    const float *d = (const float *)c->pl_in[cur_in].p;
    sb.actors = d + q.actors + (size_t)g0 * a * 14 * 48; sb.actor_ctrs = d_ctrs = d + q.ctrs + (size_t)g0 * a * 2; sb.actor_vecs = d_vecs = d + q.vecs + (size_t)g0 * a * 2;
    sb.lane_ctrs = d + q.lc + (size_t)g0 * l * 2; sb.lane_vecs = d + q.lv + (size_t)g0 * l * 2;
    sb.tgt_nodes = d + q.tn + (size_t)g0 * 160; sb.tgt_rpe = d + q.tr + (size_t)g0 * 20;
    sb.lane_feat = cb == 1 ? (const float *)c->pl_lf.p : (const float *)c->pl_lrep.p;
  }
  po.cls = d_cls; po.reg = d_reg; po.vel = d_vel;
  TR("round: predictor launch begins");
  const int rc = mind_predict_batch(c, &sb, &po);
  if (!rc) TR("round: predictor launched");
  return rc;
}

int PlanRun::pl_round_launch() {
  const int T = AIME_T, Bk = g.Bk, Bmax = g.Bmax;
  const char *dtab = (const char *)tabb->p;
  int rc;
  for (int c0 = 0; c0 < Bk; c0 += chunk) {
    const int cb = std::min(chunk, Bk - c0), g0 = g.lo + c0, Ac = cb * a;
    const size_t n_cls = ((size_t)cb * 6 + 3) & ~(size_t)3;
    float *d_cls = (float *)c->pl_pred.p, *d_reg = d_cls + n_cls, *d_vel = d_reg + (size_t)Ac * 6 * T * 5;
    const float *d_ctrs, *d_vecs;
    if ((rc = pl_predict_chunk(g0, cb, d_cls, d_reg, d_vel, d_ctrs, d_vecs))) return rc;
    if (!tables_done && (rc = pl_round_tables())) return rc;
    TR("round: tables prepared");
    n_expanded += cb;
    if (c->profiling) pair_launches += c->n_pair_launch;
    if (in->script_cls) {
      const size_t nr = (size_t)a * 6 * T * 5, nv = (size_t)a * 6 * T * 2;
      hipLaunchKernelGGL(k_repeat_rows, dim3((unsigned)((6 * (size_t)cb + 255) / 256)), dim3(256), 0, st, in->script_cls, (size_t)6, cb, d_cls);
      hipLaunchKernelGGL(k_repeat_rows, dim3((unsigned)((nr * cb + 255) / 256)), dim3(256), 0, st, in->script_reg, nr, cb, d_reg);
      hipLaunchKernelGGL(k_repeat_rows, dim3((unsigned)((nv * cb + 255) / 256)), dim3(256), 0, st, in->script_vel, nv, cb, d_vel);
    }
    const AimeScene *t_sc = (const AimeScene *)dtab + c0;
    const float *t_prob = (const float *)(dtab + bS + bI) + c0;
    float *w_c = d_world + (size_t)c0 * a * 6 * T * 6, *topo_c = d_topo + (size_t)c0 * a * 6, *ego_c = d_ego + (size_t)c0 * 24;
    float *sel_c = d_sel + (size_t)c0 * 6, *selp_c = d_selp + (size_t)c0 * 6;
    unsigned *hit_c = d_hit + (size_t)c0 * 12;
    AimeSmall sm;
    memset(&sm, 0, sizeof(sm));
    if (all_small) {
      const char *h = (const char *)c->pl_pin[1];
      memcpy(sm.s, (const AimeScene *)h + c0, (size_t)cb * sizeof(AimeScene));
      memcpy(sm.prob, (const float *)(h + bS + bI) + c0, (size_t)cb * sizeof(float));
      sm.n = cb; sm.a = a;
    }
    hipLaunchKernelGGL(k_aime_world, dim3(Ac * AIME_K), dim3(64), 0, st, t_sc, (const int *)(dtab + bS) + (size_t)c0 * a, d_reg, d_vel, d_ctrs, d_vecs,
                       cov_last_dev + (size_t)g0 * a, w_c, topo_c, ego_c, droot + ro.tl, P, sm);
    float *hs_ = h_mirror ? h_mirror + (size_t)c0 * 6 : nullptr, *hp_ = h_mirror ? h_mirror + (size_t)Bmax * 6 + (size_t)c0 * 6 : nullptr;
    unsigned *hh_ = h_mirror ? (unsigned *)(h_mirror + (size_t)Bmax * 12) + (size_t)c0 * 12 : nullptr;
    const float pf_ = in->prob_floor > 0.f ? in->prob_floor : 0.001f;
    const AimeDone dn{h_gen ? (unsigned *)c->pl_cnt.p : nullptr, h_gen, want_gen};
    if (c->glue_fused) {
      hipLaunchKernelGGL(k_aime_select_branch, dim3(cb * AIME_K), dim3(64), 0, st, t_sc, d_cls, t_prob, topo_c, ego_c, 1, in->dist_thres, pf_, w_c, sel_c, selp_c,
                         hit_c, hs_, hp_, hh_, sm, dn);
    } else {
      hipLaunchKernelGGL(k_aime_select, dim3(cb), dim3(64), 0, st, t_sc, d_cls, t_prob, topo_c, ego_c, 1, in->dist_thres, sel_c, selp_c, pf_, sm);
      hipLaunchKernelGGL(k_aime_branch, dim3(cb * AIME_K), dim3(64), 0, st, t_sc, sel_c, w_c, hit_c, (const float *)selp_c, hs_, hp_, hh_, sm, dn);
    }
    HIPCHK(c, hipGetLastError());
  }
  if (!tables_done && (rc = pl_round_tables())) return rc;
  return MIND_OK;
}

int PlanRun::pl_round_decisions(const float *&h_dec) {
  int rc;
  if (dist) {
    if ((rc = ensure(c, c->x_recv, (size_t)XW * n_back * sizeof(float)))) return rc;
    if ((rc = pl_exchange(c, MIND_XCHG_ALLGATHER, d_sel, c->x_recv.p, n_back * sizeof(float)))) return rc;
    if ((rc = pl_pin(c, 2, (size_t)XW * n_back * sizeof(float)))) return rc;
    HIPCHK(c, hipMemcpyAsync(c->pl_pin[2], c->x_recv.p, (size_t)XW * n_back * sizeof(float), hipMemcpyDeviceToHost, st));
  } else if (!h_mirror) {
    if ((rc = pl_pin(c, 2, n_back * sizeof(float)))) return rc;
    HIPCHK(c, hipMemcpyAsync(c->pl_pin[2], d_sel, n_back * sizeof(float), hipMemcpyDeviceToHost, st));
  }
  TR("round: glue launched, waiting for the decisions");
  if (h_gen) {
    if ((rc = pl_presize_next())) return rc;
    if (!pl_wait_word(h_gen, want_gen, 0.25, pl_steady_now, nullptr, 1024)) {
      HIPCHK(c, hipStreamSynchronize(st));
      HIPCHK(c, hipMemsetAsync(c->pl_cnt.p, 0, 64, st));
    }
  } else {
    HIPCHK(c, hipStreamSynchronize(st));
  }
  TR("round: decisions on the host");
  h_dec = (const float *)c->pl_pin[2];
  return MIND_OK;
}

int PlanRun::pl_presize_next() {
  if (round_no + 1 >= in->max_rounds) return MIND_OK;
  const size_t OBS = RB_T, S = (size_t)g.B * AIME_K;
  const int n = cur_in < 0 ? 0 : cur_in ^ 1;
  const size_t b_in = InLayout(S, a, l).total * sizeof(float), b_win = S * a * OBS * 5 * sizeof(float), b_rep = S * l * 128 * sizeof(float);
  if (std::max(b_in, std::max(b_win, b_rep)) >= ((size_t)64 << 20)) return MIND_OK;
  int rc;
  if (b_in > c->pl_in[n].cap || b_win > c->pl_win[n].cap || b_rep > c->pl_lrep.cap) HIPCHK(c, hipStreamSynchronize(st));
  if ((rc = ensure(c, c->pl_in[n], b_in)) || (rc = ensure(c, c->pl_win[n], b_win)) || (rc = ensure(c, c->pl_lrep, b_rep))) return rc;
  return pl_pin(c, 3, S * 28 * sizeof(float));
}

int PlanRun::pl_rebase_next() {
  const PlRound &r = book.rec;
  const size_t OBS = RB_T, S = r.S, s0 = r.s0;
  const int Sm = r.Sm;
  int rc;
  nxt = cur_in < 0 ? 0 : cur_in ^ 1;
  q = InLayout(S, a, l);
  if ((rc = ensure(c, c->pl_in[nxt], q.total * sizeof(float)))) return rc;
  const size_t n_wpos = S * a * OBS * 2, n_wang = S * a * OBS;
  if ((rc = ensure(c, c->pl_win[nxt], (2 * n_wpos + n_wang) * sizeof(float)))) return rc;
  w_pos = (float *)c->pl_win[nxt].p; w_ang = w_pos + n_wpos; w_vel = w_ang + n_wang;
  d_in = (float *)c->pl_in[nxt].p;
  if (Sm <= 0) return MIND_OK;
  int *hi_ = (int *)((char *)c->pl_pin[1] + tab_bytes);
  memcpy(hi_, r.win.data(), 3 * (size_t)Sm * sizeof(int));
  const bool tab_host = c->tab_host_max > 0 && (size_t)Sm * a <= (size_t)c->tab_host_max;
  if (!tab_host) HIPCHK(c, hipMemcpyAsync((char *)tabb->p + tab_bytes, hi_, 3 * (size_t)Sm * sizeof(int), hipMemcpyHostToDevice, st));
  const int *d_idx = tab_host ? (const int *)hi_ : (const int *)((const char *)tabb->p + tab_bytes);
  float *pos0 = w_pos + s0 * a * OBS * 2, *ang0 = w_ang + s0 * a * OBS, *vel0 = w_vel + s0 * a * OBS * 2;
  hipLaunchKernelGGL(k_aime_windows, dim3((unsigned)(Sm * a)), dim3(64), 0, st, prev_pos, prev_ang, prev_vel, (const float *)d_world, d_idx, d_idx + Sm,
                     d_idx + 2 * Sm, a, pos0, ang0, vel0, AIME_K, d_in + q.cov + s0 * a);
  RebaseArgs R = pl_rebase_args(d_in, q, s0, l);
  R.pad_ones = 1;
  R.pos = pos0; R.ang = ang0; R.vel = vel0; R.pad = nullptr;
  R.lane_ctrs0 = droot + ro.lc; R.lane_vecs0 = droot + ro.lv; R.travel0 = -1.f;
  hipLaunchKernelGGL(k_aime_rebase, dim3((unsigned)Sm, 1 + RB_FEAT_BLOCKS(a)), dim3(RB_THREADS), 5 * a * sizeof(float), st, R);
  HIPCHK(c, hipGetLastError());
  return MIND_OK;
}

int PlanRun::pl_exchange_next(int round) {
  const PlRound &r = book.rec;
  const size_t OBS = RB_T;
  float *fr_base = d_in + q.fr;
  int rc;
  struct Arr { float *base; size_t per; };
  const size_t na = a, nl = l;
  const Arr arrs[11] = {{d_in + q.actors, na * 14 * 48}, {d_in + q.ctrs, na * 2}, {d_in + q.vecs, na * 2}, {d_in + q.lc, nl * 2}, {d_in + q.lv, nl * 2}, {d_in + q.tn, 160},
                        {d_in + q.tr, 20}, {d_in + q.cov, na}, {w_pos, na * OBS * 2}, {w_ang, na * OBS}, {w_vel, na * OBS * 2}};
  std::vector<CopySeg> segs;
  {
    int cmax = 0;
    for (int k = 0; k < XW; ++k) cmax = std::max(cmax, r.cnt_r[k]);
    const size_t n_hdr = round == 0 ? nl * 128 : 0;
    const size_t n_pay = (n_hdr + (size_t)cmax * 28 + 3) & ~(size_t)3;
    if ((rc = ensure(c, c->x_send, n_pay * sizeof(float)))) return rc;
    if ((rc = ensure(c, c->x_recv, (size_t)XW * n_pay * sizeof(float)))) return rc;
    float *snd = (float *)c->x_send.p, *rcv = (float *)c->x_recv.p;
    if (n_hdr && XR == 0) segs.push_back({(const float *)c->pl_lf.p, snd, (long long)n_hdr});
    if (r.Sm > 0) segs.push_back({fr_base + (size_t)r.s0 * 28, snd + n_hdr, (long long)r.Sm * 28});
    if ((rc = pl_copy_segs(c, segs))) return rc;
    if ((rc = pl_exchange(c, MIND_XCHG_ALLGATHER, snd, rcv, n_pay * sizeof(float)))) return rc;
    segs.clear();
    if (n_hdr && XR != 0) segs.push_back({rcv, (float *)c->pl_lf.p, (long long)n_hdr});
    for (int k = 0; k < XW; ++k) {
      if (k == XR || r.cnt_r[k] == 0) continue;
      segs.push_back({rcv + (size_t)k * n_pay + n_hdr, fr_base + (size_t)r.s0_r[k] * 28, (long long)r.cnt_r[k] * 28});
    }
    if ((rc = pl_copy_segs(c, segs))) return rc;
  }
  size_t per_scene = 0;
  for (int k = 0; k < 11; ++k) per_scene += arrs[k].per;
  PlRoute rt;
  pl_route(r.S, XW, XR, r.cnt_r, r.s0_r, per_scene, c->xforce != 0, rt);
  if (rt.any <= 0) return MIND_OK;
  size_t n_snd = 0, n_rcv = 0;
  for (int k = 0; k < XW; ++k) { n_snd += (size_t)rt.tab[k] / sizeof(float); n_rcv += (size_t)rt.tab[(size_t)XW + k] / sizeof(float); }
  if ((rc = ensure(c, c->x_send, (n_snd + 4) * sizeof(float)))) return rc;
  if ((rc = ensure(c, c->x_recv, (n_rcv + 4) * sizeof(float)))) return rc;
  float *snd = (float *)c->x_send.p, *rcv = (float *)c->x_recv.p;
  const auto pair_segs = [&](const std::vector<int> &range, float *packed, bool unpack) {
    segs.clear();
    size_t o = 0;
    for (int k = 0; k < XW; ++k) {
      const size_t i0 = range[2 * k], n = range[2 * k + 1] - range[2 * k];
      for (int e = 0; e < 11 && n > 0; ++e) {
        float *arr = arrs[e].base + arrs[e].per * i0;
        segs.push_back(unpack ? CopySeg{packed + o, arr, (long long)(arrs[e].per * n)} : CopySeg{arr, packed + o, (long long)(arrs[e].per * n)});
        o += arrs[e].per * n;
      }
    }
  };
  pair_segs(rt.snd, snd, false);
  if ((rc = pl_copy_segs(c, segs))) return rc;
  if ((rc = pl_exchange_v(c, snd, rcv, rt.tab.data()))) return rc;
  pair_segs(rt.rcv, rcv, true);
  return pl_copy_segs(c, segs);
}

int PlanRun::pl_next_inputs() {
  const int S = book.rec.S;
  int nlo, nhi, rc;
  pl_block(S, XR, XW, nlo, nhi);
  const int n_rep = nhi - nlo;
  if (n_rep > 1 && (rc = ensure(c, c->pl_lrep, (size_t)n_rep * l * 128 * sizeof(float)))) return rc;
  const auto rep = [this, n_rep](hipStream_t rs) {
    if (n_rep > 1) {
      const size_t n = (size_t)l * 128;
      hipLaunchKernelGGL(k_repeat_rows, dim3((unsigned)((n * n_rep + 255) / 256)), dim3(256), 0, rs, (const float *)c->pl_lf.p, n, n_rep, (float *)c->pl_lrep.p);
      HIPCHK(c, hipGetLastError());
    }
    return (int)MIND_OK;
  };
  const float *d_fr = d_in + q.fr;
  const auto back = [this, d_fr, S](hipStream_t rs) { return pl_frames_back(d_fr, (size_t)S, rs); };
  if (c->round_head && c->side && !dist) {
    c->enc_pre = rep; c->enc_post = back;
  } else {
    hipStream_t rs;
    if ((rc = pl_side_hop(rs)) || (rc = rep(rs)) || (rc = back(rs))) return rc;
  }
  prev_pos = w_pos; prev_ang = w_ang; prev_vel = w_vel;
  cov_last_dev = d_in + q.cov;
  cur_in = nxt;
  return MIND_OK;
}

void PlanRun::pl_begin_solves() {
  const size_t Mtot = (size_t)book.tree_off.back(), nt = book.tree_top.size();
  c->pl_sol_xs.resize(Mtot * 6); c->pl_sol_us.resize(Mtot * 2);
  c->pl_sol_stw.resize(nt); c->pl_sol_stf.resize(nt);
  solves_tried = true;
  solves_rc = mind_ilqr_contingency_begin_plan(c, in->solve_cfg_warm, in->solve_cfg_full, in->solve_x0, in->solve_lane, in->solve_n_lane_pts,
                                               in->solve_target_vel, c->pl_sol_xs.data(), c->pl_sol_us.data(), c->pl_sol_stw.data(), c->pl_sol_stf.data());
  c->il_finish_owned = solves_rc == MIND_OK;
}

int PlanRun::pl_pack_results() {
  const size_t Mtot = (size_t)book.tree_off.back(), n_rows = (size_t)book.n_rows, n_flat = Mtot * a * 3, n_res = n_rows + n_flat;
  want_solves = solves_asked() && !book.tree_top.empty();
  lc_n = lc_on(c) ? (int)c->lc.pending.size() : 0;
  int rc;
  c->plan.agents = a;
  c->plan.rows_p = c->plan.fmean_p = c->plan.fcov_p = nullptr;
  c->plan.dev_fmean = c->plan.dev_fcov = nullptr;
  if (n_res > 0) {
    const JobTable &F = book.flat, &G = book.gather;
    const size_t o_g = F.bytes(), n_tab = o_g + G.bytes();
    const size_t o_rows = (n_tab + 255) & ~(size_t)255;
    if ((rc = ensure(c, c->pl_flat, o_rows + n_res * sizeof(float)))) return rc;
    if ((rc = pl_pin(c, 0, n_tab))) return rc;
    char *h = (char *)c->pl_pin[0];
    const float *world_of_round[32];
    for (size_t i = 0; i < c->pl_world.size() && i < 32; ++i) world_of_round[i] = (const float *)c->pl_world[i].p;
    F.pack(h, world_of_round);
    G.pack(h + o_g, world_of_round);
    TR("end: trees flattened on the host");
    const bool tab_host = !dist && c->tab_host_max > 0 && F.job_of_block.size() + G.job_of_block.size() <= (size_t)c->tab_host_max;
    if (n_tab && !tab_host) HIPCHK(c, hipMemcpyAsync(c->pl_flat.p, h, n_tab, hipMemcpyHostToDevice, st));
    char *d = tab_host ? h : (char *)c->pl_flat.p;
    float *d_rows = (float *)((char *)c->pl_flat.p + o_rows), *d_fmean = d_rows + n_rows, *d_fcov = d_fmean + Mtot * a * 2;
    if (dist) HIPCHK(c, hipMemsetAsync(d_rows, 0, n_res * sizeof(float), st));
    if (!F.jobs.empty())
      hipLaunchKernelGGL(k_aime_flat, dim3((unsigned)F.job_of_block.size()), dim3(64), 0, st, (const AimeFlat *)d, (const int *)(d + F.off_job()),
                         (const int *)(d + F.off_agent()), (const float *const *)(d + F.off_world()), d_fmean, d_fcov);
    const auto gather = [&](hipStream_t gs) {
      if (!G.jobs.empty())
        hipLaunchKernelGGL(k_aime_gather, dim3((unsigned)G.job_of_block.size()), dim3(64), 0, gs, (const AimeGather *)(d + o_g), (const int *)(d + o_g + G.off_job()),
                           (const int *)(d + o_g + G.off_agent()), (const float *const *)(d + o_g + G.off_world()), d_rows);
    };
    if (!want_solves) gather(st);
    HIPCHK(c, hipGetLastError());
    if (dist && (rc = pl_exchange(c, MIND_XCHG_ALLREDUCE, d_rows, d_rows, n_res * sizeof(float)))) return rc;
    c->plan.dev_fmean = d_fmean; c->plan.dev_fcov = d_fcov;
    if ((rc = pl_pin(c, 2, n_res * sizeof(float)))) return rc;
    float *hp = (float *)c->pl_pin[2];
    if (want_solves) {
// ... 13 lines not shown
    } else {
      HIPCHK(c, hipMemcpyAsync(hp, d_rows, n_res * sizeof(float), hipMemcpyDeviceToHost, st));
      if (lc_n > 0 && (rc = lc_copy_async(c, st, 0, lc_n))) return rc;
      HIPCHK(c, hipStreamSynchronize(st));
    }
    c->plan.rows_p = hp; c->plan.fmean_p = hp + n_rows; c->plan.fcov_p = hp + n_rows + Mtot * a * 2;
  } else {
    if (lc_n > 0 && (rc = lc_copy_async(c, st, 0, lc_n))) return rc;
    HIPCHK(c, hipStreamSynchronize(st));
  }
  return MIND_OK;
}

int PlanRun::pl_hand_out() {
  float pair_ms = 0.f;
  int rc;
  out->nodes = book.table.data(); out->n_nodes = (int)book.table.size();
  out->rows = c->plan.rows_p; out->n_row_floats = book.n_rows;
  out->n_expanded = n_expanded; out->n_rounds = book.n_rounds;
  out->root_flags = book.root_flags();
  if (c->profiling && (rc = mind_pair_events_resolve(c, &pair_ms))) return rc;
  if (lc_on(c)) {
    double ms[LC_KINDS];
    int n[LC_KINDS];
    if ((rc = lc_resolve(c, lc_n, 1u << LC_PAIR, ms, n))) return rc;
    pair_ms = (float)ms[LC_PAIR];
  }
  out->pair_ms = pair_ms; out->pair_launches = pair_launches;
  out->n_trees = (int)book.tree_top.size(); out->tree_top = book.tree_top.data(); out->tree_off = book.tree_off.data();
  out->flat_parent = book.flat_parent.data(); out->flat_prob = book.flat_prob.data();
  out->flat_mean = c->plan.fmean_p; out->flat_cov = c->plan.fcov_p;
  if (want_solves) {
    if (!solves_tried) pl_begin_solves();
    out->solves_begun = solves_rc == MIND_OK ? 1 : 0;
  }
  TR("end: result handed out");
  return MIND_OK;
}

}

extern "C" int mind_aime_plan(mind_ctx *c, const mind_aime_plan_in *in, mind_aime_plan_out *out) {
  if (!c || !in || !out) return MIND_EINVAL;
  int rc;
  if ((rc = pl_check(c, in))) return rc;
  HIPCHK(c, hipSetDevice(c->device));
  PlanRun p(c, in, out);
  c->plan.agents = 0;
  c->plan.gen += 1;
  p.book.reset(in->pred_len, in->max_depth, p.a, p.XW, p.XR, p.dist);
  if (!c->ev_pl) HIPCHK(c, hipEventCreateWithFlags(&c->ev_pl, hipEventDisableTiming));
  if (!c->ev_tab) HIPCHK(c, hipEventCreateWithFlags(&c->ev_tab, hipEventDisableTiming));
  if (!c->pl_copy) HIPCHK(c, hipStreamCreateWithFlags(&c->pl_copy, hipStreamNonBlocking));
  struct HookGuard { mind_ctx *c; ~HookGuard() { c->enc_pre = nullptr; c->enc_post = nullptr; } } hook_guard{c};
  if ((rc = p.pl_root())) return rc;
  memset(out, 0, sizeof(*out));
  p.TR.t0 = std::chrono::steady_clock::now();
  struct DeferGuard { mind_ctx *c; ~DeferGuard() { c->ev_defer = false; c->ev_pending.clear(); c->ev_pool_used = 0; } } defer_guard{c};
  c->ev_defer = c->profiling;
  c->ev_pending.clear(); c->ev_pool_used = 0;
  if (!c->lc.pending.empty() && (rc = lc_flush(c, false))) return rc;
  for (int k = 0; k < LC_KINDS; ++k) { c->lc_carry_ms[k] = 0.0; c->lc_carry_n[k] = 0; }
  for (int round = 0;; ++round) {
    PlErr e = p.book.begin_round(in->max_rounds, p.g);
    if (e) return p.fail_book(e);
    out->round_scenes[round] = p.g.Bk;
    const float *h_dec;
    if ((rc = p.pl_round_buffers(round)) || (rc = p.pl_round_launch()) || (rc = p.pl_round_decisions(h_dec))) return rc;
    if ((e = p.book.round(h_dec, p.g.Bmax))) return p.fail_book(e);
    if (p.book.rec.todo.empty()) break;
    if ((rc = p.pl_rebase_next())) return rc;
    if (p.dist && (rc = p.pl_exchange_next(round))) return rc;
    if ((rc = p.pl_next_inputs())) return rc;
  }
  p.TR("rounds done");
  const PlErr e = p.book.finish();
  if (e) return p.fail_book(e);
  if ((rc = p.pl_pack_results())) return rc;
  return p.pl_hand_out();
}

extern "C" int mind_ilqr_finish_plan(mind_ctx *c, int n_nodes, int n_trees, double *xs, double *us, mind_ilqr_stats *stats_warm, mind_ilqr_stats *stats_full) {
  if (!c || !xs || !us || !stats_full) return MIND_EINVAL;
  if (!c->il_finish || !c->il_finish_owned) return fail(c, MIND_ESTATE, "mind_ilqr_finish_plan: no plan-begun tree-iLQR call is pending on this context");
  const int rc = mind_ilqr_finish(c);
  if (rc) return rc;
  if ((size_t)n_nodes * 6 != c->pl_sol_xs.size() || (size_t)n_trees != c->pl_sol_stf.size() || (size_t)n_trees + 1 != c->plan.book.tree_off.size() ||
      c->plan.book.tree_off[(size_t)n_trees] != n_nodes)
    return fail(c, MIND_EINVAL, "mind_ilqr_finish_plan: the caller expects %d nodes in %d trees, the pending solves hold %zu in %zu", n_nodes, n_trees,
                c->pl_sol_xs.size() / 6, c->pl_sol_stf.size());
  memcpy(xs, c->pl_sol_xs.data(), c->pl_sol_xs.size() * sizeof(double));
  memcpy(us, c->pl_sol_us.data(), c->pl_sol_us.size() * sizeof(double));
  if (stats_warm) memcpy(stats_warm, c->pl_sol_stw.data(), c->pl_sol_stw.size() * sizeof(mind_ilqr_stats));
  memcpy(stats_full, c->pl_sol_stf.data(), c->pl_sol_stf.size() * sizeof(mind_ilqr_stats));
  return MIND_OK;
}


extern "C" int mind_aime_plan_begin(mind_ctx *c, const mind_aime_plan_in *in) {
  if (!c || !in) return MIND_EINVAL;
  if (c->pa_state.load(std::memory_order_acquire) == 1) return fail(c, MIND_ESTATE, "mind_aime_plan_begin: a plan is running on this context");
  if (c->pa_thread.joinable()) c->pa_thread.join();
  c->pa_in = *in;
  memset(&c->pa_out, 0, sizeof(c->pa_out));
  c->pa_state.store(1, std::memory_order_release);
  try {
    c->pa_thread = std::thread([c] {
      c->pa_rc = mind_aime_plan(c, &c->pa_in, &c->pa_out);
      c->pa_state.store(2, std::memory_order_release);
    });
  } catch (...) {
    c->pa_state.store(0, std::memory_order_release);
    return fail(c, MIND_ESTATE, "mind_aime_plan_begin: no thread");
  }
  return MIND_OK;
}

extern "C" int mind_aime_plan_poll(mind_ctx *c) {
  if (!c) return MIND_EINVAL;
  return c->pa_state.load(std::memory_order_acquire) == 1 ? 1 : 0;
}

extern "C" int mind_aime_plan_finish(mind_ctx *c, mind_aime_plan_out *out) {
  if (!c || !out) return MIND_EINVAL;
  if (c->pa_state.load(std::memory_order_acquire) == 0) return fail(c, MIND_ESTATE, "mind_aime_plan_finish: no plan was begun");
  if (c->pa_thread.joinable()) c->pa_thread.join();
  *out = c->pa_out;
  c->pa_state.store(0, std::memory_order_release);
  return c->pa_rc;
}

extern "C" int mind_ctx_busy(mind_ctx *c) {
  if (!c) return MIND_EINVAL;
  if (c->pa_state.load(std::memory_order_acquire) == 1) return 1;
  (void)hipSetDevice(c->device);
  const hipError_t e = hipStreamQuery(c->stream);
  if (e == hipErrorNotReady) return 1;
  if (e != hipSuccess) return fail(c, MIND_EHIP, "mind_ctx_busy: %s", hipGetErrorString(e));
  return 0;
}

extern "C" int mind_debug_wait_word(const unsigned *word, unsigned want, double timeout_s, double (*clock)(void *), void *user, int spins_per_look) {
  if (!word || !(timeout_s >= 0.0) || spins_per_look <= 0) return MIND_EINVAL;
  return pl_wait_word(word, want, timeout_s, clock ? clock : pl_steady_now, user, (unsigned)spins_per_look) ? 1 : 0;
}

constexpr int PL_BOOK_HEADER = 16;
extern "C" int mind_debug_aime_book(int pred_len, int max_depth, int max_rounds, int n_agents, int world, int rank, int force, int n_rounds, const int *dec_len,
                                    const float *dec, int n_tokens, int bytes_per_pair, int plan_chunk_mb, int per_scene, long long *out, int cap, char *msg,
                                    int msg_cap) {
  if (pred_len < 2 || pred_len > AIME_T || max_depth < 0 || max_rounds <= 0 || max_rounds > 32 || n_agents <= 0 || world < 1 || rank < 0 || rank >= world ||
      n_rounds < 0 || (n_rounds > 0 && (!dec_len || !dec)) || n_tokens < 0 || (n_tokens > 0 && (bytes_per_pair <= 0 || plan_chunk_mb <= 0)) || per_scene < 0 ||
      cap < 0 || (cap > 0 && !out) || msg_cap < 0 || (msg_cap > 0 && !msg))
    return MIND_EINVAL;
  const bool dist = pl_exchanges(true, world, force != 0);
  const auto bits = [](float f) { uint32_t u; memcpy(&u, &f, 4); return (long long)u; };
  AimeBook book(pred_len, max_depth, n_agents, world, rank, dist);
  std::vector<long long> rec(PL_BOOK_HEADER, 0);
  const auto put = [&rec](const auto &v) { rec.insert(rec.end(), v.begin(), v.end()); };
  PlErr e;
  PlGeom g;
  PlRoute rt;
  int rounds = 0;
  for (const float *d = dec; rounds < n_rounds; d += dec_len[rounds++]) {
    if ((e = book.begin_round(max_rounds, g))) break;
    if (dec_len[rounds] != (dist ? world : 1) * g.Bmax * 24) return MIND_EINVAL;
    if ((e = book.round(d, g.Bmax))) break;
    const PlRound &q = book.rec;
    pl_route(q.S, world, rank, q.cnt_r, q.s0_r, (size_t)per_scene, force != 0, rt);
    rec.insert(rec.end(), {g.B, g.lo, g.hi, g.Bmax, n_tokens ? pl_chunk(n_tokens, bytes_per_pair, plan_chunk_mb, g.Bk) : 0, q.S, q.s0, q.Sm, rt.any});
    put(q.todo); put(q.cnt_r); put(q.s0_r); put(q.win); put(rt.tab); put(rt.snd); put(rt.rcv);
  }
  if (!e) e = book.finish();
  if (msg_cap > 0) snprintf(msg, (size_t)msg_cap, pl_err_format(e.code), e.a0, e.a1);
  if (!e) {
    for (size_t i = 0; i < book.table.size(); ++i) {
      const mind_aime_node &n = book.table[i];
      const PlNode &m = book.nodes[i + 1];
      rec.insert(rec.end(), {n.round, n.scene, n.mode, n.parent, bits(n.prob), n.cur_t, n.end_t, n.flags, n.dur, n.row_off, m.owner, m.lscene});
    }
    for (const JobTable *t : {&book.gather, &book.flat}) {
      rec.insert(rec.end(), {(long long)t->jobs.size(), (long long)t->job_of_block.size(), (long long)t->bytes()});
      for (size_t i = 0; i < t->jobs.size(); ++i) rec.insert(rec.end(), {t->jobs[i].row0, t->jobs[i].n, t->jobs[i].dst, t->jobs[i].a, t->world[i]});
      put(t->job_of_block); put(t->agent_of_block);
    }
    put(book.tree_top); put(book.tree_off); put(book.flat_parent);
    for (float f : book.flat_prob) rec.push_back(bits(f));
  }
  const long long hdr[12] = {PL_BOOK_HEADER, e.code, e.a0, e.a1, rounds, e ? 0 : (long long)book.table.size(), e ? 0 : (long long)book.tree_top.size(),
                             e ? 0 : (long long)book.flat_parent.size(), e ? 0 : book.n_rows, book.root_flags(), dist, world};
  std::copy(hdr, hdr + 12, rec.begin());
  for (size_t i = 0; i < rec.size() && (int)i < cap; ++i) out[i] = rec[i];
  return (int)rec.size();
}
```

### mind_amd/csrc/mind_hip.hip

```cpp
#include <hip/hip_runtime.h>

#include <cmath>
#include <cstdarg>
#include <cstdio>
#include <cstdlib>
#include <algorithm>
#include <cstring>
#include <map>
#include <string>
#include <thread>
#include <atomic>
#include <functional>
#include <vector>

#include "../../include/mind_hip.h"
#include "encdec_kernels.hip"
#include "fusion_kernels.hip"
#include "pair_bf16_kernels.hip"
#include "pair_tile_kernels.hip"
#include "pair_tile6_kernels.hip"
#include "token_mfma_kernels.hip"
#include "actor_mfma_kernels.hip"
#include "actor_lw_kernels.hip"
#include "token_lw_kernels.hip"
// ... 18 lines not shown

struct DevBuf {
  void *p = nullptr;
  size_t cap = 0;
};

}

struct TableSet {
  std::vector<int> key;
  DevBuf meta, jobs, jobs5, rows;
  std::vector<int> actor_row, cls_row, scene_n;
  long long edge_pairs = 0, edge_pairs_t = 0, stamp = 0;
  int ntok = 0, slot = 0, njobs = 0, njobs5 = 0;
  double pairs_full = 0, pairs_l5 = 0;
};
#define MIND_TABLE_SETS 8

struct mind_ctx {
  int device = 0;
  hipStream_t stream = nullptr;
  bool own_stream = false;
  hipStream_t side = nullptr;
  hipEvent_t ev_side = nullptr, ev_main = nullptr, ev_stage = nullptr, ev_tgt = nullptr, ev_cls = nullptr;
  std::vector<char> aime_stage;
  bool aime_stage_busy = false;
  std::string err;
  float *wdev = nullptr;
  bool have_weights = false;
  WeightTables W = {};
  PredTuning pt;
  int dec_basis = MIND_BASIS_BEZIER;
  DevBuf curve_tab;
  std::vector<double> curve_tau;
  int curve_tab_basis = -1;
  DevBuf tok_lw_arena;
  std::vector<TlLaunch> tok_lw_plan;
  int last_tok_lw = 0, last_tok_launches = 0, last_tok_chunks = 0;
  float tok_ms = 0.f, tok_stage_ms[TL_NSTAGE + 1] = {};
  std::vector<hipEvent_t> ev_tok;
  std::vector<int> ev_tok_tag;
  TableSet tabs[MIND_TABLE_SETS];
  long long tab_clock = 0;
  long long n_table_hits = 0;
  IlqrTuning it;
  int upload_kernel_max = 1 << 20;
  bool dec_mirror = true;
  bool glue_fused = true;
  bool dec_poll = true;
  unsigned dec_gen = 0;
  DevBuf pl_cnt;
  bool root_head = true, round_head = true;
  std::function<int(hipStream_t)> enc_pre, enc_post;
  bool early_eval = true;
  int tab_host_max = 4096;
  bool tab_small = true;
  std::vector<IlTables> il_tab;
  struct IlImage { std::vector<double> hD; std::vector<float> hF; std::vector<int> hI; } il_img;
  struct IlEarly { const double *xs = nullptr, *us = nullptr; volatile unsigned *done = nullptr; unsigned gen = 0; int n_trees = 0; long nodes = 0; } il_early;
  unsigned il_gen = 0;
  long long il_spec_req = 0, il_spec_hit = 0;
  DevBuf actor_lw_arena;
  std::vector<LwLaunch> actor_lw_plan;
  int last_actor_lw = 0, last_actor_launches = 0, last_actor_chunks = 0;
  float actor_ms = 0.f;
  hipEvent_t ev_act0 = nullptr, ev_act1 = nullptr;
  int pair_prec = 3;
  int plan_chunk_mb = 96 * 1024;
  std::vector<int> last_scene_n;
  bool last_edge_tiled = false, last_edge_bf16 = false;
  DevBuf edge, x, ST, QK, part, tokpos, meta, jobs, actor_feat, lane_feat, tgt_feat, cmode, tgt_emb,
      rows, rpe_ptrs;
  DevBuf ilqr_dev, aime_dev, rebase_dev2[2], dec_h2;
  DevBuf audit_dev;
  DevBuf pl_root, pl_in[2], pl_lf, pl_lrep, pl_pred, pl_small, pl_tab[2], pl_win[2];
  std::vector<DevBuf> pl_world;
  void *pl_pin[8] = {nullptr, nullptr, nullptr, nullptr, nullptr, nullptr, nullptr, nullptr};
  size_t pl_pin_cap[8] = {0, 0, 0, 0, 0, 0, 0, 0};
  hipEvent_t ev_pl = nullptr, ev_tab = nullptr, ev_root = nullptr;
  DevBuf il_field;
  void *il_field_pin = nullptr;
  size_t il_field_pin_cap = 0;
  hipEvent_t ev_field = nullptr;
  bool il_field_valid = false;
  double il_field_key[5] = {0, 0, 0, 0, 0};
  std::vector<double> il_field_lane;
  int xr = 0, xw = 1;
  mind_exchange_fn xfn = nullptr;
  void *xuser = nullptr;
  bool xforce = false;
  DevBuf x_send, x_recv, x_seg;
  long long x_collectives = 0, x_bytes = 0;
  hipStream_t pl_copy = nullptr;
  bool pl_tab_side = false;
  std::vector<double> pl_sol_xs, pl_sol_us;
  std::vector<mind_ilqr_stats> pl_sol_stw, pl_sol_stf;
  std::thread pa_thread;
  std::atomic<int> pa_state{0};
  mind_aime_plan_in pa_in;
  mind_aime_plan_out pa_out;
  int pa_rc = 0;
  struct Plan {
    AimeBook book;
    int agents = 0;
    long long gen = 0;
    const float *rows_p = nullptr, *fmean_p = nullptr, *fcov_p = nullptr;
// ... 117 lines not shown
  if (const char *te = getenv("MIND_PAIR_TILE")) c->pt.pair_tile = !(te[0] == '0');
  if (const char *xe = getenv("MIND_XCD_ORDER")) c->pt.xcd_order = !(xe[0] == '0');

  if (const char *pe = getenv("MIND_PAIR_PREC")) {
    const std::string v = pe;
    if (v == "f32" || v == "0") c->pair_prec = 0;
    else if (v == "bf16x3" || v == "1") c->pair_prec = 1;
    else if (v == "bf16" || v == "2") c->pair_prec = 2;
    else if (v == "bf16x6" || v == "3") c->pair_prec = 3;
  }
  (void)hipFuncSetAttribute((const void *)k_actor_net, hipFuncAttributeMaxDynamicSharedMemorySize, (int)mind_actor_lds_bytes());
  (void)hipFuncSetAttribute((const void *)k_actor_mfma<3>, hipFuncAttributeMaxDynamicSharedMemorySize, (int)mind_actor_mfma_lds_bytes());
  (void)hipFuncSetAttribute((const void *)k_actor_mfma<6>, hipFuncAttributeMaxDynamicSharedMemorySize, (int)mind_actor_mfma_lds_bytes());
  (void)hipFuncSetAttribute((const void *)k_dec_actor_mfma<1>, hipFuncAttributeMaxDynamicSharedMemorySize, (int)mind_dec_actor_mfma_lds_bytes());
  (void)hipFuncSetAttribute((const void *)k_dec_actor_mfma<3>, hipFuncAttributeMaxDynamicSharedMemorySize, (int)mind_dec_actor_mfma_lds_bytes());
  (void)hipFuncSetAttribute((const void *)k_dec_actor_mfma<6>, hipFuncAttributeMaxDynamicSharedMemorySize, (int)mind_dec_actor_mfma_lds_bytes());
  if (const char *se = getenv("MIND_ACTOR_SPLIT")) c->pt.actor_np = atoi(se) == 3 ? 3 : 6;
  (void)hipFuncSetAttribute((const void *)k_actor_mfma<1>, hipFuncAttributeMaxDynamicSharedMemorySize, (int)mind_actor_mfma_lds_bytes());
  if (const char *me = getenv("MIND_ENC_MFMA")) c->pt.enc_mfma = !(me[0] == '0');
  if (const char *me = getenv("MIND_ACTOR_F32")) c->pt.actor_f32 = !(me[0] == '0');
  if (const char *me = getenv("MIND_ACTOR_F32_MIN")) c->pt.actor_f32_min = atoi(me);
  if (const char *me = getenv("MIND_ACTOR_LW_MIN")) c->pt.actor_lw_min = atoi(me);
  lw_set_attributes();
  (void)hipFuncSetAttribute((const void *)k_actor_f32<1>, hipFuncAttributeMaxDynamicSharedMemorySize, (int)mind_actor_f32_lds_bytes(1));
  (void)hipFuncSetAttribute((const void *)k_actor_f32<2>, hipFuncAttributeMaxDynamicSharedMemorySize, (int)mind_actor_f32_lds_bytes(2));
  if (const char *de = getenv("MIND_DEC_MFMA_MIN")) c->pt.dec_mfma_min = atoi(de);
  if (const char *oe = getenv("MIND_DEC_OVERLAP")) c->pt.dec_overlap = !(oe[0] == '0');
  (void)hipFuncSetAttribute((const void *)k_ilqr<true, 0>, hipFuncAttributeMaxDynamicSharedMemorySize, (int)il_lds_bytes(0));
  (void)hipFuncSetAttribute((const void *)k_ilqr<false, 1>, hipFuncAttributeMaxDynamicSharedMemorySize, (int)il_lds_bytes(0));
  (void)hipFuncSetAttribute((const void *)k_ilqr<false, 0>, hipFuncAttributeMaxDynamicSharedMemorySize, (int)il_lds_bytes(0));
  (void)hipFuncSetAttribute((const void *)k_ilqr<false, 2>, hipFuncAttributeMaxDynamicSharedMemorySize, (int)il_lds_bytes(0));
  if (const char *te = getenv("MIND_TOK_MFMA")) c->pt.tok_mfma = !(te[0] == '0');
  if (const char *te = getenv("MIND_TOK_SMALL_MAX")) c->pt.tok_small_max = atoi(te);
  if (const char *te = getenv("MIND_TOK_MERGE")) c->pt.tok_merge = !(te[0] == '0');
  if (const char *te = getenv("MIND_DEC_MW")) c->pt.dec_mw = !(te[0] == '0');
  if (const char *te = getenv("MIND_DEC_CLS_SIDE")) c->pt.dec_cls_side = !(te[0] == '0');
  if (const char *te = getenv("MIND_TOK_BF_MIN_N")) c->pt.tok_bf_min_n = atoi(te);
  if (const char *te = getenv("MIND_TOK_LW_MIN_N")) c->pt.tok_lw_min_n = atoi(te);
  if (const char *te = getenv("MIND_TOK_LW_MIN")) c->pt.tok_lw_min = atoi(te);
  if (const char *te = getenv("MIND_TGT_SIDE")) c->pt.tgt_side = !(te[0] == '0');
  if (const char *te = getenv("MIND_PL_TAB_SIDE")) c->pl_tab_side = !(te[0] == '0');
  (void)hipFuncSetAttribute((const void *)k_token_mfma<0>, hipFuncAttributeMaxDynamicSharedMemorySize, (int)mind_token_mfma_lds_bytes());
  (void)hipFuncSetAttribute((const void *)k_token_mfma<1>, hipFuncAttributeMaxDynamicSharedMemorySize, (int)mind_token_mfma_lds_bytes());
  if (const char *ce = getenv("MIND_PLAN_CHUNK_MB")) { const long v = atol(ce); if (v > 0) c->plan_chunk_mb = v; }
  if (const char *we = getenv("MIND_TAB_SMALL")) c->tab_small = atoi(we) != 0;
  if (const char *we = getenv("MIND_TAB_HOST_MAX")) c->tab_host_max = std::max(0, atoi(we));
  if (const char *we = getenv("MIND_EARLY_EVAL")) c->early_eval = atoi(we) != 0;
  if (const char *we = getenv("MIND_GLUE_FUSED")) c->glue_fused = atoi(we) != 0;
  if (const char *we = getenv("MIND_DEC_MIRROR")) c->dec_mirror = atoi(we) != 0;
  if (const char *we = getenv("MIND_DEC_POLL")) c->dec_poll = atoi(we) != 0;
  if (const char *we = getenv("MIND_ROOT_HEAD")) c->root_head = atoi(we) != 0;
  if (const char *we = getenv("MIND_ROUND_HEAD")) c->round_head = atoi(we) != 0;
  if (const char *we = getenv("MIND_UPLOAD_KERNEL_MAX")) c->upload_kernel_max = std::max(0, atoi(we));
  const char *const il_env[][2] = {{"MIND_ILQR_CHUNK", "ilqr_chunk"}, {"MIND_ILQR_WGS", "ilqr_wgs"}, {"MIND_ILQR_SPEC_DERIV", "ilqr_spec_deriv"},
                                   {"MIND_ILQR_HOST_OUT_MAX", "ilqr_host_out_max"}, {"MIND_ILQR_SLOTS", "ilqr_slots"}};
  for (const auto &e : il_env)
    if (const char *we = getenv(e[0])) (void)ilqr_tuning_set(c->it, e[1], atoi(we));
  (void)hipFuncSetAttribute((const void *)k_dec_scene, hipFuncAttributeMaxDynamicSharedMemorySize, (int)mind_dec_scene_lds_bytes());
  (void)hipFuncSetAttribute((const void *)k_dec_scene_mw, hipFuncAttributeMaxDynamicSharedMemorySize, (int)mind_dec_scene_lds_bytes());
  (void)hipFuncSetAttribute((const void *)k_dec_scene_c, hipFuncAttributeMaxDynamicSharedMemorySize, (int)mind_dec_scene_lds_bytes());
  (void)hipFuncSetAttribute((const void *)k_dec_cls, hipFuncAttributeMaxDynamicSharedMemorySize, (int)mind_dec_scene_lds_bytes());
  (void)hipFuncSetAttribute((const void *)k_dec_tgt, hipFuncAttributeMaxDynamicSharedMemorySize, (int)mind_dec_scene_lds_bytes());
  (void)hipFuncSetAttribute((const void *)k_dec_actor<0>, hipFuncAttributeMaxDynamicSharedMemorySize, (int)mind_dec_actor_lds_bytes());
  (void)hipFuncSetAttribute((const void *)k_dec_actor<1>, hipFuncAttributeMaxDynamicSharedMemorySize, (int)mind_dec_actor_lds_bytes());
  (void)hipFuncSetAttribute((const void *)k_dec_actor<2>, hipFuncAttributeMaxDynamicSharedMemorySize, (int)mind_dec_actor_lds_bytes());
  (void)hipFuncSetAttribute((const void *)k_dec_actor<2, 1>, hipFuncAttributeMaxDynamicSharedMemorySize, (int)mind_dec_actor_lds_bytes());
  (void)hipFuncSetAttribute((const void *)k_dec_actor<2, 2>, hipFuncAttributeMaxDynamicSharedMemorySize, (int)mind_dec_actor_lds_bytes());
  if (const char *te = getenv("MIND_DEC_HEAD_RA")) (void)pred_tuning_set(c->pt, "dec_head_ra", atoi(te));
  *out = c;
  return MIND_OK;
}

extern "C" int mind_ctx_destroy(mind_ctx *c) {
  if (!c) return MIND_EINVAL;
  if (c->pa_thread.joinable()) c->pa_thread.join();
  (void)hipSetDevice(c->device);
  (void)hipStreamSynchronize(c->stream);
  DevBuf *bufs[] = {&c->edge, &c->x, &c->ST, &c->QK, &c->part, &c->tokpos, &c->meta, &c->jobs, &c->actor_feat,
                    &c->lane_feat, &c->tgt_feat, &c->cmode, &c->tgt_emb, &c->rows, &c->rpe_ptrs, &c->ilqr_dev, &c->aime_dev, &c->rebase_dev2[0], &c->rebase_dev2[1], &c->dec_h2,
                    &c->curve_tab, &c->audit_dev};
  for (DevBuf *b : bufs)
    if (b->p) (void)hipFree(b->p);
  for (TableSet &t : c->tabs)
    for (DevBuf *b : {&t.meta, &t.jobs, &t.jobs5, &t.rows})
      if (b->p) (void)hipFree(b->p);
  if (c->wdev) (void)hipFree(c->wdev);
  for (DevBuf *b : {&c->dec_xbuf, &c->dec_bars})
    if (b->p) (void)hipFree(b->p);
  if (c->dec_abort) (void)hipHostFree(c->dec_abort);
  if (c->lc_dev.p) (void)hipFree(c->lc_dev.p);
  if (c->lc_host) (void)hipHostFree(c->lc_host);
  for (DevBuf *b : {&c->pl_root, &c->pl_in[0], &c->pl_in[1], &c->pl_lf, &c->pl_lrep, &c->pl_pred, &c->pl_small, &c->pl_tab[0], &c->pl_tab[1], &c->pl_win[0],
                    &c->pl_win[1], &c->pl_flat, &c->x_send, &c->x_recv, &c->x_seg, &c->pl_cnt})
    if (b->p) (void)hipFree(b->p);
  for (DevBuf &b : c->pl_world)
    if (b.p) (void)hipFree(b.p);
  for (void *q : c->pl_pin)
    if (q) (void)hipHostFree(q);
  if (c->ev_pl) (void)hipEventDestroy(c->ev_pl);
  if (c->ev_root) (void)hipEventDestroy(c->ev_root);
  if (c->ev_field) (void)hipEventDestroy(c->ev_field);
  if (c->il_field.p) (void)hipFree(c->il_field.p);
  if (c->il_field_pin) (void)hipHostFree(c->il_field_pin);
  if (c->ev_tab) (void)hipEventDestroy(c->ev_tab);
  if (c->ev_rows) (void)hipEventDestroy(c->ev_rows);
  if (c->pl_copy) (void)hipStreamDestroy(c->pl_copy);
  for (hipEvent_t e : c->ev) (void)hipEventDestroy(e);
  for (hipEvent_t e : c->ev_pool) (void)hipEventDestroy(e);
  if (c->ev_side) (void)hipEventDestroy(c->ev_side);
  if (c->ev_main) (void)hipEventDestroy(c->ev_main);
  if (c->ev_tgt) (void)hipEventDestroy(c->ev_tgt);
  if (c->ev_stage) (void)hipEventDestroy(c->ev_stage);
  if (c->ev_cls) (void)hipEventDestroy(c->ev_cls);
  if (c->actor_lw_arena.p) (void)hipFree(c->actor_lw_arena.p);
  if (c->tok_lw_arena.p) (void)hipFree(c->tok_lw_arena.p);
  for (hipEvent_t e : c->ev_tok) (void)hipEventDestroy(e);
  if (c->ev_act0) (void)hipEventDestroy(c->ev_act0);
  if (c->ev_act1) (void)hipEventDestroy(c->ev_act1);
  if (c->ev_il0) (void)hipEventDestroy(c->ev_il0);
  if (c->ev_il1) (void)hipEventDestroy(c->ev_il1);
  if (c->side) { (void)hipStreamSynchronize(c->side); (void)hipStreamDestroy(c->side); }
  if (c->own_stream) (void)hipStreamDestroy(c->stream);
  delete c;
  return MIND_OK;
}

extern "C" const char *mind_last_error_string(mind_ctx *c) { return c ? c->err.c_str() : "null context"; }

extern "C" int mind_ctx_synchronize(mind_ctx *c) {
  if (!c) return MIND_EINVAL;
  HIPCHK(c, hipStreamSynchronize(c->stream));
  return MIND_OK;
}

extern "C" int mind_set_tuning(mind_ctx *c, const char *name, int value) {
  if (!c || !name) return MIND_EINVAL;
  const std::string n = name;
  if (pred_tuning_set(c->pt, name, value)) return MIND_OK;
  if (ilqr_tuning_set(c->it, name, value)) return MIND_OK;
  if (n == "plan_chunk_mb") c->plan_chunk_mb = value < 1 ? 1 : value;
  else if (n == "pl_tab_side") c->pl_tab_side = value != 0;
  else if (n == "tab_small") c->tab_small = value != 0;
  else if (n == "tab_host_max") c->tab_host_max = value < 0 ? 0 : value;
  else if (n == "early_eval") c->early_eval = value != 0;
  else if (n == "glue_fused") c->glue_fused = value != 0;
  else if (n == "dec_mirror") c->dec_mirror = value != 0;
  else if (n == "dec_poll") c->dec_poll = value != 0;
  else if (n == "root_head") c->root_head = value != 0;
  else if (n == "round_head") c->round_head = value != 0;
  else if (n == "upload_kernel_max") c->upload_kernel_max = value < 0 ? 0 : value;
  else if (n == "prof_clock") c->prof_clock = value < 0 ? 0 : (value > 2 ? 2 : value);
  else return fail(c, MIND_EINVAL, "mind_set_tuning: unknown knob '%s'", name);
  return MIND_OK;
}

extern "C" int mind_set_exchange(mind_ctx *c, int rank, int world, mind_exchange_fn fn, void *user, int force) {
  if (!c) return MIND_EINVAL;
  if (fn && (world < 1 || rank < 0 || rank >= world)) return fail(c, MIND_EINVAL, "mind_set_exchange: rank %d of %d", rank, world);
  c->xfn = fn; c->xuser = user;
  c->xr = fn ? rank : 0; c->xw = fn ? world : 1; c->xforce = fn && force != 0;
  return MIND_OK;
}

extern "C" int mind_last_exchange_stats(mind_ctx *c, long long *collectives, long long *bytes) {
  if (!c) return MIND_EINVAL;
  if (collectives) *collectives = c->x_collectives;
  if (bytes) *bytes = c->x_bytes;
  return MIND_OK;
}

extern "C" int mind_set_pair_precision(mind_ctx *c, int mode) {
  if (!c || mode < 0 || mode > 3) return MIND_EINVAL;
  c->pair_prec = mode;
  return MIND_OK;
}

extern "C" int mind_get_pair_precision(mind_ctx *c) { return c ? c->pair_prec : MIND_EINVAL; }

extern "C" int mind_debug_pack_bfrag(const float *w, int row_stride, uint32_t *out) {
  if (!w || !out || row_stride < 128) return MIND_EINVAL;
  std::vector<float> v(w, w + (size_t)127 * row_stride + 128);
  v.resize((size_t)128 * row_stride, 0.f);
  const std::vector<float> t = pack_bfrag(v, row_stride);
  memcpy(out, t.data(), 16384 * sizeof(uint32_t));
  return MIND_OK;
}

static int lc_reserve(mind_ctx *c, int records, int grid);
extern "C" int mind_set_profiling(mind_ctx *c, int enable) {
  if (!c) return MIND_EINVAL;
  c->profiling = enable != 0;
  if (c->profiling && c->prof_clock != 0 && c->wall_khz > 0 && c->lc.n_blocks == 0) {
    HIPCHK(c, hipSetDevice(c->device));
    return lc_reserve(c, 12, c->n_cu);
  }
  return MIND_OK;
}

extern "C" int mind_last_ilqr_stats(mind_ctx *c, float *kernel_ms, int *n_trees, int *workgroups_per_tree) {
  if (!c) return MIND_EINVAL;
  if (kernel_ms) *kernel_ms = c->ilqr_ms;
  if (n_trees) *n_trees = c->ilqr_trees;
  if (workgroups_per_tree) *workgroups_per_tree = c->ilqr_multi;
// ... 399 lines not shown
      !out->tgt_nodes || !out->tgt_rpe || !out->frames)
    return fail(c, MIND_EINVAL, "mind_aime_rebase: bad argument");
  HIPCHK(c, hipSetDevice(c->device));
  hipStream_t st = c->stream;
  const size_t S = in->n_scenes, a = in->n_agents, l = in->n_lanes, P = in->n_lane_pts;
  if (dev_src) {
    if (in->prev_gen != c->rb_gen || c->rb_gen == 0 || c->rb_a != a)
      return fail(c, MIND_ESTATE, "mind_aime_rebase: the parents' windows (generation %d, %zu agents) are not the previous call's (%d, %zu)",
                  in->prev_gen, a, c->rb_gen, c->rb_a);
    for (size_t s_ = 0; s_ < S; ++s_)
      if (in->parent_slot[s_] < 0 || (size_t)in->parent_slot[s_] >= c->rb_S || in->row0[s_] < 0 || in->dur[s_] < 0 || in->dur[s_] > AIME_T)
        return fail(c, MIND_EINVAL, "mind_aime_rebase: scene %zu: parent slot %d / row %d / dur %d out of range", s_, in->parent_slot[s_],
                    in->row0[s_], in->dur[s_]);
  }
  const size_t n_pos = S * a * 50 * 2, n_ang = S * a * 50, n_types = a * 50 * 7, n_pad = in->pad ? S * a * 50 : 0;
  const size_t o_pos = 0, o_ang = o_pos + n_pos, o_vel = o_ang + n_ang, o_types = o_vel + n_pos, o_pad = o_types + n_types;
  const size_t o_lc = o_pad + n_pad, o_lv = o_lc + 2 * l, o_tl = o_lv + 2 * l, o_ti = o_tl + 2 * P, o_idx = o_ti + 12 * P;
  const size_t total = o_idx + (dev_src ? 3 * S : 0);
  DevBuf &cur = c->rebase_dev2[c->rb_cur ^ 1];
  const float *prev = (const float *)c->rebase_dev2[c->rb_cur].p;
  const size_t prev_o_ang = c->rb_S * c->rb_a * 50 * 2, prev_o_vel = prev_o_ang + c->rb_S * c->rb_a * 50;
  int rc;
  if ((rc = ensure(c, cur, total * sizeof(float)))) return rc;
  float *d = (float *)cur.p;
  const bool one_copy = !dev_src && total * sizeof(float) <= ((size_t)1 << 20);
  const size_t s0 = one_copy ? 0 : o_types;
  std::vector<float> small(total - s0);
  if (one_copy) {
    memcpy(small.data() + o_pos, in->pos, n_pos * sizeof(float));
    memcpy(small.data() + o_ang, in->ang, n_ang * sizeof(float));
    memcpy(small.data() + o_vel, in->vel, n_pos * sizeof(float));
  } else if (!dev_src) {
    HIPCHK(c, hipMemcpyAsync(d + o_pos, in->pos, n_pos * sizeof(float), hipMemcpyHostToDevice, st));
    HIPCHK(c, hipMemcpyAsync(d + o_ang, in->ang, n_ang * sizeof(float), hipMemcpyHostToDevice, st));
    HIPCHK(c, hipMemcpyAsync(d + o_vel, in->vel, n_pos * sizeof(float), hipMemcpyHostToDevice, st));
  }
  memcpy(small.data() + (o_types - s0), in->types, n_types * sizeof(float));
  if (in->pad) memcpy(small.data() + (o_pad - s0), in->pad, n_pad * sizeof(float));
  if (l) {
    memcpy(small.data() + (o_lc - s0), in->lane_ctrs, 2 * l * sizeof(float));
    memcpy(small.data() + (o_lv - s0), in->lane_vecs, 2 * l * sizeof(float));
  }
  memcpy(small.data() + (o_tl - s0), in->target_lane, 2 * P * sizeof(float));
  memcpy(small.data() + (o_ti - s0), in->target_lane_info, 12 * P * sizeof(float));
  if (dev_src) {
    memcpy(small.data() + (o_idx - s0), in->parent_slot, S * sizeof(int));
    memcpy(small.data() + (o_idx - s0) + S, in->row0, S * sizeof(int));
    memcpy(small.data() + (o_idx - s0) + 2 * S, in->dur, S * sizeof(int));
  }
  HIPCHK(c, hipMemcpyAsync(d + s0, small.data(), small.size() * sizeof(float), hipMemcpyHostToDevice, st));
  if (dev_src) {
    const int *di = (const int *)(d + o_idx);
    hipLaunchKernelGGL(k_aime_windows, dim3((unsigned)(S * a)), dim3(64), 0, st, prev, prev + prev_o_ang, prev + prev_o_vel, in->rows_dev,
                       di, di + S, di + 2 * S, (int)a, d + o_pos, d + o_ang, d + o_vel, 1, (float *)nullptr);
  }
  c->rb_cur ^= 1; c->rb_gen += 1; c->rb_S = S; c->rb_a = a;
  if (out->gen) *out->gen = c->rb_gen;
  RebaseArgs A;
  A.a = (int)a; A.l = (int)l; A.n_lane = (int)P; A.pad_ones = in->pad ? 0 : 1;
  A.pos = d + o_pos; A.ang = d + o_ang; A.vel = d + o_vel; A.types = d + o_types; A.pad = in->pad ? d + o_pad : nullptr;
  A.lane_ctrs0 = d + o_lc; A.lane_vecs0 = d + o_lv; A.tlane = d + o_tl; A.tinfo = d + o_ti;
  A.time_ahead = in->time_ahead; A.min_vel = in->min_vel; A.travel0 = -1.f;
  A.actors = out->actors; A.actor_ctrs = out->actor_ctrs; A.actor_vecs = out->actor_vecs; A.lane_ctrs = out->lane_ctrs;
  A.lane_vecs = out->lane_vecs; A.tgt_nodes = out->tgt_nodes; A.tgt_rpe = out->tgt_rpe; A.frames = out->frames;
  hipLaunchKernelGGL(k_aime_rebase, dim3((unsigned)S, 1 + RB_FEAT_BLOCKS(a)), dim3(RB_THREADS), 5 * a * sizeof(float), st, A);
  HIPCHK(c, hipGetLastError());
  HIPCHK(c, hipStreamSynchronize(st));
  return MIND_OK;
}

extern "C" int mind_debug_aime_decide(mind_ctx *c, int n_scenes, const int32_t *actor_off, const int32_t *cmp, const float *cls, const float *scen_prob,
                                      const float *topo, const float *ego_end, const float *world, int lane_check, float dist_thres,
                                      float prob_floor, int fused, int by_value, float *sel, float *sel_prob, uint32_t *hit) {
  if (!c || n_scenes <= 0 || !actor_off || !cmp || !cls || !scen_prob || !topo || !ego_end || !world || !sel || !sel_prob || !hit)
    return fail(c, MIND_EINVAL, "mind_debug_aime_decide: bad argument");
  const int B = n_scenes;
  std::vector<AimeScene> hs(B);
  for (int b = 0; b < B; ++b) {
    AimeScene &S = hs[b];
    memset(&S, 0, sizeof(S));
    S.a0 = actor_off[b]; S.a1 = actor_off[b + 1]; S.last = AIME_T - 1; S.cmp = cmp[b];
    S.r00 = S.r11 = 1.f;
    if (S.a0 < 0 || S.a1 <= S.a0) return fail(c, MIND_EINVAL, "mind_debug_aime_decide: scene %d has no agents", b);
    if (S.cmp < 0 || S.cmp >= AIME_T) return fail(c, MIND_EINVAL, "mind_debug_aime_decide: scene %d: compare step %d out of range", b, S.cmp);
  }
  AimeSmall sm;
  memset(&sm, 0, sizeof(sm));
  if (by_value) {
    const int a = hs[0].a1 - hs[0].a0;
    if (B > AIME_SMALL) return fail(c, MIND_EINVAL, "mind_debug_aime_decide: tables by value hold at most %d scenes (%d given)", AIME_SMALL, B);
    for (int b = 0; b < B; ++b)
      if (hs[b].a1 - hs[b].a0 != a || hs[b].a0 != b * a)
        return fail(c, MIND_EINVAL, "mind_debug_aime_decide: tables by value need the same agent count in every scene");
    memcpy(sm.s, hs.data(), (size_t)B * sizeof(AimeScene));
    memcpy(sm.prob, scen_prob, (size_t)B * sizeof(float));
    sm.n = B; sm.a = a;
  }
  HIPCHK(c, hipSetDevice(c->device));
  hipStream_t st = c->stream;
  const size_t bS = ((size_t)B * sizeof(AimeScene) + 15) & ~(size_t)15;
  std::vector<char> stage(bS + (size_t)B * sizeof(float), 0);
  memcpy(stage.data(), hs.data(), (size_t)B * sizeof(AimeScene));
  memcpy(stage.data() + bS, scen_prob, (size_t)B * sizeof(float));
  if (by_value) {
    for (int b = 0; b < B; ++b) {
      AimeScene S = hs[b];
      S.a1 = S.a0 + 1; S.cmp = (S.cmp + 29) % AIME_T;
// ... 273 lines not shown
```

### mind_amd/csrc/predict.hip

```cpp
__global__ void k_tokpos(const TokMeta *__restrict__ meta, int n_tok, const float *__restrict__ actr,
                         const float *__restrict__ avec, const float *__restrict__ lctr,
                         const float *__restrict__ lvec, float *__restrict__ tokpos) {
  const int t = blockIdx.x * blockDim.x + threadIdx.x;
  if (t >= n_tok) return;
  const TokMeta m = meta[t];
  float4 o = make_float4(0.f, 0.f, 0.f, 0.f);
  if (m.type == 0 && actr) o = make_float4(actr[m.src * 2], actr[m.src * 2 + 1], avec[m.src * 2], avec[m.src * 2 + 1]);
  if (m.type == 1 && lctr) o = make_float4(lctr[m.src * 2], lctr[m.src * 2 + 1], lvec[m.src * 2], lvec[m.src * 2 + 1]);
  ((float4 *)tokpos)[t] = o;
}

struct PairTables {
  std::vector<TokMeta> meta;
  std::vector<PairJob> jobs, jobs5;
  std::vector<int> actor_row, actor_scene, cls_row, scene_n;
  long long edge_pairs = 0, edge_pairs_t = 0;
  int ntok = 0, slot = 0;
  double pairs_full = 0, pairs_l5 = 0;
};

static void pair_tables_build(int Bn, const int *scene_actors, const int *scene_lanes, bool xcd_order, int n_cu, PairTables &T) {
  int A = 0;
  for (int b = 0; b < Bn; ++b) A += scene_actors[b];
  T.actor_row.assign(A, 0); T.actor_scene.assign(A, 0); T.cls_row.assign(Bn, 0); T.scene_n.assign(Bn, 0);
// ... 220 lines not shown
  }
  PairTables T;
  pair_tables_build(Bn, scene_actors, scene_lanes, c->pt.xcd_order, c->n_cu, T);
  int rc;
  ts->key.clear();
  if ((rc = ensure(c, ts->meta, T.meta.size() * sizeof(TokMeta)))) return rc;
  if ((rc = ensure(c, ts->jobs, T.jobs.size() * sizeof(PairJob)))) return rc;
  if ((rc = ensure(c, ts->jobs5, T.jobs5.size() * sizeof(PairJob)))) return rc;
  if ((rc = ensure(c, ts->rows, (size_t)(2 * A + Bn) * sizeof(int)))) return rc;
  HIPCHK(c, hipMemcpyAsync(ts->meta.p, T.meta.data(), T.meta.size() * sizeof(TokMeta), hipMemcpyHostToDevice, p.st));
  HIPCHK(c, hipMemcpyAsync(ts->jobs.p, T.jobs.data(), T.jobs.size() * sizeof(PairJob), hipMemcpyHostToDevice, p.st));
  HIPCHK(c, hipMemcpyAsync(ts->jobs5.p, T.jobs5.data(), T.jobs5.size() * sizeof(PairJob), hipMemcpyHostToDevice, p.st));
  std::vector<int> rows(2 * A + Bn);
  memcpy(rows.data(), T.actor_row.data(), A * sizeof(int));
  memcpy(rows.data() + A, T.actor_scene.data(), A * sizeof(int));
  memcpy(rows.data() + 2 * A, T.cls_row.data(), Bn * sizeof(int));
  HIPCHK(c, hipMemcpyAsync(ts->rows.p, rows.data(), rows.size() * sizeof(int), hipMemcpyHostToDevice, p.st));
  HIPCHK(c, hipStreamSynchronize(p.st));
  ts->actor_row.swap(T.actor_row);
  ts->cls_row.swap(T.cls_row);
  ts->scene_n.swap(T.scene_n);
  ts->edge_pairs = T.edge_pairs; ts->edge_pairs_t = T.edge_pairs_t; ts->ntok = T.ntok; ts->slot = T.slot; ts->njobs = (int)T.jobs.size();
  ts->njobs5 = (int)T.jobs5.size();
  ts->pairs_full = T.pairs_full; ts->pairs_l5 = T.pairs_l5;
  ts->key.swap(key);
  return MIND_OK;
}

static int pred_workspaces(PredCall &p) {
  mind_ctx *c = p.c;
  const TableSet *ts = p.ts;
  const int ntok = ts->ntok, Bn = p.Bn;
  int rc;
  if ((rc = ensure(c, c->edge, (size_t)(p.ch.tiled ? ts->edge_pairs_t : ts->edge_pairs) * 128 * sizeof(float)))) return rc;
  if ((rc = ensure(c, c->x, (size_t)ntok * 128 * sizeof(float)))) return rc;
  if ((rc = ensure(c, c->ST, (size_t)ntok * 256 * sizeof(float)))) return rc;
  if ((rc = ensure(c, c->QK, (size_t)(ntok + 1) * p.ch.qk_stride * sizeof(float)))) return rc;
  if ((rc = ensure(c, c->part, (size_t)ts->slot * PART_STRIDE * sizeof(float)))) return rc;
  if ((rc = ensure(c, c->tokpos, (size_t)ntok * 4 * sizeof(float)))) return rc;
  if ((rc = ensure(c, c->actor_feat, (size_t)p.A * 128 * sizeof(float)))) return rc;
  if ((rc = ensure(c, c->lane_feat, (size_t)(p.Ltot > 0 ? p.Ltot : 1) * 128 * sizeof(float)))) return rc;
  if ((rc = ensure(c, c->tgt_feat, (size_t)Bn * 128 * sizeof(float)))) return rc;
  if ((rc = ensure(c, c->cmode, (size_t)Bn * 768 * sizeof(float)))) return rc;
  if ((rc = ensure(c, c->tgt_emb, (size_t)Bn * 128 * sizeof(float)))) return rc;
  if (p.in->rpe) {
    if ((rc = ensure(c, c->rpe_ptrs, (size_t)Bn * sizeof(float *)))) return rc;
    HIPCHK(c, hipMemcpyAsync(c->rpe_ptrs.p, p.in->rpe, (size_t)Bn * sizeof(float *), hipMemcpyHostToDevice, p.st));
    HIPCHK(c, hipStreamSynchronize(p.st));
    p.rpe_dev = (const float *const *)c->rpe_ptrs.p;
  }
  return MIND_OK;
}

static int pred_actor_net(PredCall &p, LcSlot *clk) {
  mind_ctx *c = p.c;
  const PredChoice &ch = p.ch;
  const float *actors = p.in->actors;
  float *actor_feat = (float *)c->actor_feat.p;
  const int A = p.A;
  const dim3 grid(ch.actor_grid);
  switch (ch.actor_form) {
  case PRED_ACTOR_F32:
    if (ch.actor_arg == 2) hipLaunchKernelGGL(k_actor_f32<2>, grid, dim3(AF_T), mind_actor_f32_lds_bytes(2), p.st, actors, A, actor_feat, c->W.actorF, clk);
    else hipLaunchKernelGGL(k_actor_f32<1>, grid, dim3(AF_T), mind_actor_f32_lds_bytes(1), p.st, actors, A, actor_feat, c->W.actorF, clk);
    break;
  case PRED_ACTOR_VALU:
    hipLaunchKernelGGL(k_actor_net, grid, dim3(AT), mind_actor_lds_bytes(), p.st, actors, A, actor_feat, c->W.actor, clk);
    break;
  case PRED_ACTOR_LW: {
    int rc;
    if ((rc = ensure_exact(c, c->actor_lw_arena, lw_arena_bytes(ch.actor_chunk), "the layer-wise ActorNet's arena"))) return rc;
    lw_build_plan(A, ch.actor_chunk, c->actor_lw_plan);
    u32 *arena = (u32 *)c->actor_lw_arena.p;
    const int nl = ch.np == 6 ? lw_run<6>(c->actor_lw_plan, p.st, arena, actors, actor_feat, c->W.actorB)
                 : ch.np == 3 ? lw_run<3>(c->actor_lw_plan, p.st, arena, actors, actor_feat, c->W.actorB)
                              : lw_run<1>(c->actor_lw_plan, p.st, arena, actors, actor_feat, c->W.actorB);
    if (nl < 0) return fail(c, MIND_ESTATE, "layer-wise ActorNet: a stage has no kernel");
    c->last_actor_lw = 1; c->last_actor_launches = nl; c->last_actor_chunks = ch.actor_chunks;
    break;
  }
  default:
    if (ch.np == 6) hipLaunchKernelGGL(k_actor_mfma<6>, grid, dim3(AM_T), mind_actor_mfma_lds_bytes(), p.st, actors, A, actor_feat, c->W.actorB, clk);
    else if (ch.np == 3) hipLaunchKernelGGL(k_actor_mfma<3>, grid, dim3(AM_T), mind_actor_mfma_lds_bytes(), p.st, actors, A, actor_feat, c->W.actorB, clk);
    else hipLaunchKernelGGL(k_actor_mfma<1>, grid, dim3(AM_T), mind_actor_mfma_lds_bytes(), p.st, actors, A, actor_feat, c->W.actorB, clk);
  }
  return MIND_OK;
}

static int pred_encoders(PredCall &p) {
  mind_ctx *c = p.c;
  const mind_scene_batch *in = p.in;
  hipStream_t st = p.st, ss = p.ss;
  const int Bn = p.Bn, Ltot = p.Ltot, ntok = p.ts->ntok;
  if (c->side) {
    HIPCHK(c, hipEventRecord(c->ev_main, st));
    HIPCHK(c, hipStreamWaitEvent(c->side, c->ev_main, 0));
  }
  const bool act_timed = c->profiling && !c->ev_defer;
  int rc;
  LcSlot *act_clk = nullptr;
  if (act_timed && lc_on(c) && p.ch.actor_form != PRED_ACTOR_LW) {
    if ((rc = lc_reserve(c, 1, p.ch.actor_grid))) return rc;
    act_clk = lc_take(c, p.ch.actor_grid, LC_ACTOR);
  }
  p.act_ev = act_timed && (lc_events(c) || !act_clk);
  if (p.act_ev && !c->ev_act0) {
    HIPCHK(c, hipEventCreate(&c->ev_act0));
    HIPCHK(c, hipEventCreate(&c->ev_act1));
  }
  c->last_actor_lw = 0; c->last_actor_launches = 1; c->last_actor_chunks = 1; c->actor_ms = 0.f;
  if (p.act_ev) HIPCHK(c, hipEventRecord(c->ev_act0, st));
  if ((rc = pred_actor_net(p, act_clk))) return rc;
  if (p.act_ev) HIPCHK(c, hipEventRecord(c->ev_act1, st));
  if (c->enc_pre) {
    const std::function<int(hipStream_t)> pre = std::move(c->enc_pre);
    c->enc_pre = nullptr;
    if ((rc = pre(ss))) return rc;
  }
  p.lane_feat = in->lane_feat;
  if (!p.lane_feat) {
    float *lf = p.out->lane_feat ? p.out->lane_feat : (float *)c->lane_feat.p;
    if (Ltot > 0)
      hipLaunchKernelGGL(k_lane_net, dim3((Ltot + PL - 1) / PL), dim3(DT), 0, ss, in->lanes, Ltot, lf, c->W.lane);
    p.lane_feat = lf;
  } else if (p.out->lane_feat && p.out->lane_feat != in->lane_feat && Ltot > 0) {
    HIPCHK(c, hipMemcpyAsync(p.out->lane_feat, in->lane_feat, (size_t)Ltot * 128 * sizeof(float), hipMemcpyDeviceToDevice, ss));
  }
  hipLaunchKernelGGL(k_tokpos, dim3((ntok + 255) / 256), dim3(256), 0, ss, (const TokMeta *)p.ts->meta.p, ntok, in->actor_ctrs, in->actor_vecs,
                     in->lane_ctrs, in->lane_vecs, (float *)c->tokpos.p);
  if (c->side) {
    HIPCHK(c, hipEventRecord(c->ev_side, c->side));
    HIPCHK(c, hipStreamWaitEvent(st, c->ev_side, 0));
  }
  hipLaunchKernelGGL(k_lane_net, dim3((Bn + PL - 1) / PL), dim3(DT), 0, ss, in->tgt_nodes, Bn, (float *)c->tgt_feat.p, c->W.lane);
  hipLaunchKernelGGL(k_dec_tgt, dim3(Bn), dim3(DT), mind_dec_scene_lds_bytes(), ss, (const float *)c->tgt_feat.p, in->tgt_rpe, (float *)c->tgt_emb.p,
                     c->W.dec);
  if (c->enc_post) {
    const std::function<int(hipStream_t)> post = std::move(c->enc_post);
    c->enc_post = nullptr;
    if ((rc = post(ss))) return rc;
  }
  if (c->side) HIPCHK(c, hipEventRecord(c->ev_tgt, c->side));
  if (p.ch.tgt_wait_first) HIPCHK(c, hipStreamWaitEvent(st, c->ev_tgt, 0));
  return MIND_OK;
}

static hipError_t pred_tok_mark(PredCall &p, int tag) {
  mind_ctx *c = p.c;
  if (!p.tok_timed) return hipSuccess;
  if (p.ev_tok_used == c->ev_tok.size()) {
    hipEvent_t e;
    const hipError_t rc_ = hipEventCreate(&e);
    if (rc_ != hipSuccess) return rc_;
    c->ev_tok.push_back(e);
    c->ev_tok_tag.push_back(0);
  }
  c->ev_tok_tag[p.ev_tok_used] = tag;
  return hipEventRecord(c->ev_tok[p.ev_tok_used++], p.st);
}

static int pred_token_step(PredCall &p, int mode, int Lw) {
  mind_ctx *c = p.c;
  hipStream_t st = p.st;
  const size_t qk_stride = p.ch.qk_stride, tokm_lds = mind_token_mfma_lds_bytes();
  const float *actor_feat = (const float *)c->actor_feat.p, *lane_feat = p.lane_feat;
// ... 266 lines not shown
```

Measured before the change: 1874.

## Compute next-round branch windows on device and queue ActorNet ahead of host decisions

The last block of the AIME branch kernel now computes the next round's branch windows and scene count on the GPU from its own select/hit results. Using that device-side count, the rebase, window and ActorNet kernels for the next round can be enqueued before the host finishes reading decisions. The goal is to hide the host round trip between tree-expansion rounds. The path is gated by a per-round hint and a stale-candidate check, and it adds device-count indirection to several kernels plus more complex bookkeeping that could fall out of sync with the host.

```diff
diff --git a/include/mind_hip.h b/include/mind_hip.h
--- a/include/mind_hip.h
+++ b/include/mind_hip.h
@@ -107,6 +107,11 @@
 int mind_debug_aime_book(int pred_len, int max_depth, int max_rounds, int n_agents, int world, int rank, int force, int n_rounds, const int *dec_len,
                          const float *dec, int n_tokens, int bytes_per_pair, int plan_chunk_mb, int per_scene, long long *out, int cap, char *msg,
                          int msg_cap);
+
+int mind_debug_branch_scene(const float *sel, const unsigned *hit, int scene, int lscene, int a, int cur_t, int end_t, int parent_depth, int max_depth,
+                            int pred_len, int *kids);
+
+int mind_debug_round_ahead(mind_ctx *c, int round, int *out, int cap);
 
 int mind_debug_wait_word(const unsigned *word, unsigned want, double timeout_s, double (*clock)(void *user), void *user, int spins_per_look);
 
diff --git a/mind_amd/_lib.py b/mind_amd/_lib.py
--- a/mind_amd/_lib.py
+++ b/mind_amd/_lib.py
@@ -215,7 +215,7 @@
            "mind_weights_load", "mind_predict_batch", "mind_last_fusion_stats", "mind_last_actor_stats", "mind_debug_actor_lw_plan", "mind_last_token_stats", "mind_last_token_stage_ms", "mind_debug_token_lw_plan", "mind_set_profiling", "mind_debug_launch_times", "mind_debug_launch_clock",
            "mind_ilqr_solve_trees", "mind_ilqr_contingency", "mind_ilqr_solve_fields", "mind_cost_eval", "mind_ilqr_score_trees", "mind_ilqr_gains", "mind_ilqr_policy_rollouts", "mind_lane_dist_field", "mind_aime_world", "mind_aime_rebase", "mind_debug_aime_decide", "mind_debug_set_layers",
            "mind_debug_read", "mind_set_pair_precision", "mind_get_pair_precision", "mind_debug_pack_bfrag", "mind_debug_pack_conv_frag", "mind_debug_pack", "mind_debug_weight_image", "mind_debug_weight_bind", "mind_debug_pair_schedule", "mind_debug_predict_choice", "mind_debug_ilqr_plan", "mind_debug_aime_book", "mind_set_tuning", "mind_last_ilqr_stats", "mind_aime_plan", "mind_last_ilqr_profile", "mind_eval_traj_trees", "mind_last_ilqr_trace", "mind_ilqr_contingency_begin", "mind_ilqr_finish", "mind_fill_tracks", "mind_ilqr_contingency_begin_plan", "mind_debug_trig", "mind_aime_plan_begin", "mind_aime_plan_poll", "mind_aime_plan_finish", "mind_ctx_busy", "mind_ilqr_finish_plan",
-           "mind_set_exchange", "mind_last_exchange_stats", "mind_debug_wait_word",
+           "mind_set_exchange", "mind_last_exchange_stats", "mind_debug_wait_word", "mind_debug_round_ahead", "mind_debug_branch_scene",
            "mind_predict_batch_aux", "mind_set_decoder_basis", "mind_get_decoder_basis", "mind_curve_eval", "mind_debug_curve_basis",
            "mind_audit_plan", "mind_audit_episode", "mind_debug_box_clearance",
            "mind_forecast_score", "mind_debug_forecast_score",
@@ -319,6 +319,8 @@
                                          C.POINTER(C.c_longlong), C.c_int, C.POINTER(C.c_int)]
     lib.mind_debug_wait_word.argtypes = [C.POINTER(C.c_uint), C.c_uint, C.c_double, WAIT_CLOCK, C.c_void_p, C.c_int]
     lib.mind_debug_aime_book.argtypes = [C.c_int] * 8 + [C.POINTER(C.c_int), C.POINTER(C.c_float)] + [C.c_int] * 4 + [C.POINTER(C.c_longlong), C.c_int, C.c_char_p, C.c_int]
+    lib.mind_debug_round_ahead.argtypes = [C.c_void_p, C.c_int, C.POINTER(C.c_int), C.c_int]
+    lib.mind_debug_branch_scene.argtypes = [C.POINTER(C.c_float), C.POINTER(C.c_uint)] + [C.c_int] * 8 + [C.POINTER(C.c_int)]
     lib.mind_debug_trig.argtypes = [C.c_void_p, C.POINTER(C.c_double), C.c_int, C.POINTER(C.c_double)]
     lib.mind_debug_pack_conv_frag.argtypes = [C.POINTER(C.c_float), C.c_int, C.c_int, C.c_int, C.POINTER(C.c_uint32), C.c_size_t]
     lib.mind_debug_pack.argtypes = [C.c_char_p, C.POINTER(C.c_float), C.c_int, C.c_int, C.c_int, C.POINTER(C.c_float), C.c_size_t]
diff --git a/mind_amd/csrc/actor_mfma_kernels.hip b/mind_amd/csrc/actor_mfma_kernels.hip
--- a/mind_amd/csrc/actor_mfma_kernels.hip
+++ b/mind_amd/csrc/actor_mfma_kernels.hip
@@ -212,7 +212,8 @@
 
 template <int NP>
 __global__ __launch_bounds__(AM_T) void k_actor_mfma(const float *__restrict__ actors , int n_actors,
-                                                     float *__restrict__ out , AmW W, LcSlot *clk) {
+                                                     float *__restrict__ out , AmW W, LcSlot *clk, const int *__restrict__ n_dev) {
+  if (n_dev) n_actors = *n_dev;
   lc_stamp_in(clk);
   extern __shared__ __attribute__((aligned(16))) u32 smu[];
   u32 *xin = smu + AM_XIN;
diff --git a/mind_amd/csrc/aime_book.h b/mind_amd/csrc/aime_book.h
--- a/mind_amd/csrc/aime_book.h
+++ b/mind_amd/csrc/aime_book.h
@@ -6,9 +6,11 @@
 #include <vector>
 
 #include "../../include/mind_hip.h"
+#include "aime_branch.h"
 
 constexpr int PL_K = 6;
 constexpr int PL_OBS = 50;
+static_assert(PL_K == 6, "aime_branch.h visits six slots per scene");
 
 struct PlScene {
   int node;
@@ -190,6 +192,14 @@
     g.Bk = g.hi - g.lo;
     g.Bmax = (g.B + XW - 1) / XW;
     return e;
+  }
+
+  bool stale_candidate() const {
+    for (int li : leaves) {
+      const PlNode &n = nodes[li];
+      if (!n.branch && !n.end && !plb_depth_capped(n.depth, max_depth)) return true;
+    }
+    return false;
   }
 
   static int flags_of(const PlNode &n) { return (n.branch ? MIND_AIME_BRANCH : 0) | (n.end ? MIND_AIME_END : 0) | (n.term ? MIND_AIME_TERMINATE : 0); }
@@ -231,7 +241,7 @@
       PlNode &n = nodes[li];
       if (n.branch) { n.branch = false; n.term = true; }
       else if (!n.end) {
-        if (n.depth >= max_depth) n.term = true;
+        if (plb_depth_capped(n.depth, max_depth)) n.term = true;
         else cand.push_back(li);
       }
     }
@@ -239,11 +249,9 @@
       PlNode &n = nodes[li];
       if (li == 0) { err.code = PL_E_ROOT; return err; }
       if (n.rebased && n.cur_t > 0) { err.code = PL_E_TRIMMED; return err; }
-      int t_b = n.end_t;
-      for (int t = n.cur_t + 1 + (n.cur_t + 1) % 2; t < n.end_t; t += 2)
-        if ((n.hit >> t) & 1ull) { t_b = t; break; }
-      if (t_b < n.end_t) n.end_t = t_b;
-      if (t_b < HZ) todo.push_back(li);
+      const PlKid k = plb_candidate(n.hit, n.scene, n.lscene, n.mode, a, n.cur_t, n.end_t, HZ);
+      n.end_t = k.end_t;
+      if (k.what == PLB_TODO) todo.push_back(li);
       else n.end = true;
     }
     const int S = rec.S = (int)todo.size();
@@ -261,9 +269,9 @@
     rec.win.resize(3 * (size_t)Sm);
     for (int s = 0; s < Sm; ++s) {
       const PlNode &n = nodes[todo[s0 + s]];
-      rec.win[s] = n.scene;
-      rec.win[Sm + s] = n.lscene * a * PL_K + n.mode;
-      rec.win[2 * Sm + s] = n.end_t - n.cur_t;
+      int w3[3];
+      plb_win(n.scene, n.lscene, n.mode, a, n.cur_t, n.end_t, w3);
+      rec.win[s] = w3[0]; rec.win[Sm + s] = w3[1]; rec.win[2 * Sm + s] = w3[2];
     }
     batch.assign(S, PlScene());
     for (int s = 0; s < S; ++s) {
diff --git a/mind_amd/csrc/aime_branch.h b/mind_amd/csrc/aime_branch.h
--- /dev/null
+++ b/mind_amd/csrc/aime_branch.h
@@ -0,0 +1,58 @@
+#pragma once
+
+#if defined(__HIPCC__)
+#define PLB_FN __host__ __device__ __forceinline__
+#else
+#define PLB_FN static inline
+#endif
+
+enum { PLB_SKIP = 0, PLB_TERM = 1, PLB_END = 2, PLB_TODO = 3 };
+
+struct PlKid {
+  int what;
+  int end_t;
+  int win[3];
+};
+
+PLB_FN bool plb_depth_capped(int depth, int max_depth) { return depth >= max_depth; }
+
+PLB_FN int plb_branch_time(unsigned long long hit, int cur_t, int end_t) {
+  for (int t = cur_t + 1 + (cur_t + 1) % 2; t < end_t; t += 2)
+    if ((hit >> t) & 1ull) return t;
+  return end_t;
+}
+
+PLB_FN void plb_win(int scene, int lscene, int mode, int a, int cur_t, int end_t, int *w3) {
+  w3[0] = scene;
+  w3[1] = lscene * a * 6 + mode;
+  w3[2] = end_t - cur_t;
+}
+
+PLB_FN PlKid plb_candidate(unsigned long long hit, int scene, int lscene, int mode, int a, int cur_t, int end_t, int HZ) {
+  PlKid k;
+  const int t_b = plb_branch_time(hit, cur_t, end_t);
+  k.end_t = t_b < end_t ? t_b : end_t;
+  k.what = t_b < HZ ? PLB_TODO : PLB_END;
+  plb_win(scene, lscene, mode, a, cur_t, k.end_t, k.win);
+  return k;
+}
+
+PLB_FN PlKid plb_slot(float sel, unsigned hit_lo, unsigned hit_hi, int scene, int lscene, int a, int cur_t, int end_t, int parent_depth,
+                      int max_depth, int HZ) {
+  const int mode = (int)sel;
+  PlKid k;
+  k.what = PLB_SKIP; k.end_t = end_t; k.win[0] = k.win[1] = k.win[2] = 0;
+  if (mode < 0) return k;
+  if (plb_depth_capped(parent_depth + 1, max_depth)) { k.what = PLB_TERM; return k; }
+  return plb_candidate((unsigned long long)hit_lo | ((unsigned long long)hit_hi << 32), scene, lscene, mode, a, cur_t, end_t, HZ);
+}
+
+PLB_FN int plb_scene(const float *sel, const unsigned *hit, int scene, int lscene, int a, int cur_t, int end_t, int parent_depth, int max_depth,
+                     int HZ, PlKid *kids) {
+  int n = 0;
+  for (int j = 0; j < 6; ++j) {
+    kids[j] = plb_slot(sel[j], hit[2 * j], hit[2 * j + 1], scene, lscene, a, cur_t, end_t, parent_depth, max_depth, HZ);
+    n += kids[j].what == PLB_TODO;
+  }
+  return n;
+}
diff --git a/mind_amd/csrc/aime_kernels.hip b/mind_amd/csrc/aime_kernels.hip
--- a/mind_amd/csrc/aime_kernels.hip
+++ b/mind_amd/csrc/aime_kernels.hip
@@ -1,5 +1,7 @@
 #include <hip/hip_runtime.h>
 #include <stdint.h>
+
+#include "aime_branch.h"
 
 struct AimeScene {
   int a0, a1;
@@ -196,6 +198,7 @@
   float time_ahead, min_vel;
   float *actors, *actor_ctrs, *actor_vecs, *lane_ctrs, *lane_vecs, *tgt_nodes, *tgt_rpe, *frames;
   float travel0;
+  const int *n_dev = nullptr;
 };
 
 __device__ __forceinline__ void rb_cs(float ax, float ay, float bx, float by, float &c, float &s) {
@@ -209,9 +212,14 @@
                                                      const int *__restrict__ parent_slot, const int *__restrict__ row0,
                                                      const int *__restrict__ dur, int a, float *__restrict__ pos,
                                                      float *__restrict__ ang, float *__restrict__ vel, int row_stride,
-                                                     float *__restrict__ cov_last) {
+                                                     float *__restrict__ cov_last, const int *__restrict__ n_dev) {
   const int s = blockIdx.x / a, i = blockIdx.x - s * a, t = threadIdx.x;
   if (t >= RB_T) return;
+  if (n_dev) {
+    const int S = *n_dev;
+    if (s >= S) return;
+    row0 = parent_slot + S; dur = parent_slot + 2 * S;
+  }
   const int d = dur[s];
   const int src = t + d;
   float x, y, vx, vy, h;
@@ -227,15 +235,45 @@
   pos[2 * o] = x; pos[2 * o + 1] = y; vel[2 * o] = vx; vel[2 * o + 1] = vy; ang[o] = h;
 }
 
-struct AimeDone { unsigned *cnt; unsigned *h_gen; unsigned gen; };
-__device__ __forceinline__ void aime_decisions_done(const AimeDone D) {
-  if (!D.h_gen) return;
+struct AimeAhead { int *win; int *n; int hz, max_depth; int info[AIME_SMALL]; };
+struct AimeDone { unsigned *cnt; unsigned *h_gen; unsigned gen; AimeAhead ahead; };
+__device__ __forceinline__ bool aime_decisions_arrive(const AimeDone &D) {
+  if (!D.h_gen) return false;
   __threadfence_system();
   const unsigned prev = __hip_atomic_fetch_add(D.cnt, 1u, __ATOMIC_ACQ_REL, __HIP_MEMORY_SCOPE_AGENT);
-  if (prev + 1u != gridDim.x) return;
+  if (prev + 1u != gridDim.x) return false;
   __hip_atomic_store(D.cnt, 0u, __ATOMIC_RELAXED, __HIP_MEMORY_SCOPE_AGENT);
+  return true;
+}
+__device__ __forceinline__ void aime_decisions_publish(const AimeDone &D) {
   __threadfence_system();
   __hip_atomic_store(D.h_gen, D.gen, __ATOMIC_RELEASE, __HIP_MEMORY_SCOPE_SYSTEM);
+}
+__device__ __forceinline__ void aime_decisions_done(const AimeDone &D) {
+  if (aime_decisions_arrive(D)) aime_decisions_publish(D);
+}
+
+__device__ __forceinline__ void aime_branch_set(const AimeAhead &A, const AimeSmall &sm, const float *sel, const unsigned *hit, int t) {
+  __builtin_amdgcn_fence(__ATOMIC_ACQUIRE, "agent");
+  const int b = t / AIME_K;
+  PlKid k;
+  k.what = PLB_SKIP; k.end_t = 0; k.win[0] = k.win[1] = k.win[2] = 0;
+  if (t < sm.n * AIME_K) {
+    int info = 0;
+#pragma unroll
+    for (int q = 0; q < AIME_SMALL; ++q) if (q == b) info = A.info[q];
+    const float sv = __uint_as_float(__hip_atomic_load((const unsigned *)sel + t, __ATOMIC_RELAXED, __HIP_MEMORY_SCOPE_AGENT));
+    const unsigned h0 = __hip_atomic_load(hit + 2 * t, __ATOMIC_RELAXED, __HIP_MEMORY_SCOPE_AGENT);
+    const unsigned h1 = __hip_atomic_load(hit + 2 * t + 1, __ATOMIC_RELAXED, __HIP_MEMORY_SCOPE_AGENT);
+    k = plb_slot(sv, h0, h1, b, b, sm.a, info & 255, (info >> 8) & 255, info >> 16, A.max_depth, A.hz);
+  }
+  const unsigned long long m = __ballot(k.what == PLB_TODO);
+  const int S = __popcll(m);
+  if (k.what == PLB_TODO) {
+    const int s = __popcll(m & ((1ull << t) - 1ull));
+    A.win[s] = k.win[0]; A.win[S + s] = k.win[1]; A.win[2 * S + s] = k.win[2];
+  }
+  if (t == 0) { A.n[0] = S; A.n[1] = S * sm.a; }
 }
 
 __global__ __launch_bounds__(64) void k_aime_branch(const AimeScene *__restrict__ scenes, const float *__restrict__ sel,
@@ -291,15 +329,21 @@
     }
   }
   const unsigned long long m = __ballot(h);
+  bool last = false;
   if (t == 0) {
     hit[2 * (size_t)blockIdx.x] = (unsigned)m; hit[2 * (size_t)blockIdx.x + 1] = (unsigned)(m >> 32);
     sel[blockIdx.x] = kf; sel_prob[blockIdx.x] = pj;
     if (h_sel) {
       h_hit[2 * (size_t)blockIdx.x] = (unsigned)m; h_hit[2 * (size_t)blockIdx.x + 1] = (unsigned)(m >> 32);
       h_sel[blockIdx.x] = kf; h_selp[blockIdx.x] = pj;
-      aime_decisions_done(done);
-    }
-  }
+      last = aime_decisions_arrive(done);
+    }
+  }
+  if (done.ahead.win) {
+    last = __ballot(last) != 0ull;
+    if (last) aime_branch_set(done.ahead, sm, sel, hit, t);
+  }
+  if (t == 0 && last) aime_decisions_publish(done);
 }
 
 struct AimeGather { int row0, dur, dst, a; };
@@ -336,6 +380,7 @@
 __global__ __launch_bounds__(RB_THREADS) void k_aime_rebase(RebaseArgs A) {
   const int sc = blockIdx.x, tid = threadIdx.x;
   const int a = A.a;
+  if (A.n_dev && sc >= *A.n_dev) return;
   extern __shared__ float rb_sm[];
   __shared__ float fr[8];
   __shared__ float rdv[RB_THREADS];
diff --git a/mind_amd/csrc/aime_plan.hip b/mind_amd/csrc/aime_plan.hip
--- a/mind_amd/csrc/aime_plan.hip
+++ b/mind_amd/csrc/aime_plan.hip
@@ -101,6 +101,8 @@
   int nxt = 0;
   InLayout q{0, 0, 0};
   float *d_in = nullptr, *w_pos = nullptr, *w_ang = nullptr, *w_vel = nullptr;
+  bool ahead_on = false, ahead = false, presized = false, actor_queued = false;
+  int nxt_S = 0, cur_S = 0;
   bool want_solves = false, solves_tried = false;
   int solves_rc = MIND_OK;
   PlTrace TR;
@@ -114,6 +116,7 @@
   int pl_root(), pl_root_raw(), pl_root_host(), pl_presize_next();
   int pl_round_buffers(int round), pl_round_launch(), pl_round_tables(), pl_round_decisions(const float *&h_dec);
   int pl_predict_chunk(int g0, int cb, float *d_cls, float *d_reg, float *d_vel, const float *&d_ctrs, const float *&d_vecs);
+  int pl_queue_ahead(), pl_ahead_seen();
   int pl_rebase_next(), pl_exchange_next(int round), pl_next_inputs(), pl_pack_results(), pl_hand_out();
   void pl_begin_solves();
   int pl_side_hop(hipStream_t &rs), pl_frames_back(const float *d_fr, size_t S, hipStream_t rs);
@@ -305,6 +308,10 @@
     want_gen = c->dec_gen;
     __atomic_store_n(h_gen, 0u, __ATOMIC_RELEASE);
   }
+  const int hint = (size_t)round < c->ra_hint.size() ? c->ra_hint[round] : -1;
+  ahead = presized = actor_queued = false;
+  ahead_on = h_gen && c->round_ahead && c->glue_fused && all_small && XW == 1 && round + 1 < in->max_rounds && !book.stale_candidate() &&
+             (hint < 0 || (c->round_ahead == 2 ? hint == 0 : hint == 1));
   return MIND_OK;
 }
 
@@ -363,7 +370,7 @@
     sb.lane_ctrs = droot + o.lc; sb.lane_vecs = droot + o.lv; sb.tgt_nodes = droot + o.tn; sb.tgt_rpe = droot + o.tr;
     po.lane_feat = (float *)c->pl_lf.p;
   } else {
-    const InLayout q(g.B, a, l);
+    const InLayout q(cur_S, a, l);
     const float *d = (const float *)c->pl_in[cur_in].p;
     sb.actors = d + q.actors + (size_t)g0 * a * 14 * 48; sb.actor_ctrs = d_ctrs = d + q.ctrs + (size_t)g0 * a * 2; sb.actor_vecs = d_vecs = d + q.vecs + (size_t)g0 * a * 2;
     sb.lane_ctrs = d + q.lc + (size_t)g0 * l * 2; sb.lane_vecs = d + q.lv + (size_t)g0 * l * 2;
@@ -415,7 +422,15 @@
     float *hs_ = h_mirror ? h_mirror + (size_t)c0 * 6 : nullptr, *hp_ = h_mirror ? h_mirror + (size_t)Bmax * 6 + (size_t)c0 * 6 : nullptr;
     unsigned *hh_ = h_mirror ? (unsigned *)(h_mirror + (size_t)Bmax * 12) + (size_t)c0 * 12 : nullptr;
     const float pf_ = in->prob_floor > 0.f ? in->prob_floor : 0.001f;
-    const AimeDone dn{h_gen ? (unsigned *)c->pl_cnt.p : nullptr, h_gen, want_gen};
+    AimeDone dn{h_gen ? (unsigned *)c->pl_cnt.p : nullptr, h_gen, want_gen};
+    if (ahead_on) {
+      dn.ahead.win = (int *)((char *)tabb->p + tab_bytes); dn.ahead.n = dn.ahead.win + 3 * (size_t)6 * Bmax;
+      dn.ahead.hz = HZ; dn.ahead.max_depth = in->max_depth;
+      for (int b = 0; b < cb; ++b) {
+        const PlScene &sc = book.batch[g0 + b];
+        dn.ahead.info[b] = sc.cur_t | (sc.end_t << 8) | (book.nodes[sc.node].depth << 16);
+      }
+    }
     if (c->glue_fused) {
       hipLaunchKernelGGL(k_aime_select_branch, dim3(cb * AIME_K), dim3(64), 0, st, t_sc, d_cls, t_prob, topo_c, ego_c, 1, in->dist_thres, pf_, w_c, sel_c, selp_c,
                          hit_c, hs_, hp_, hh_, sm, dn);
@@ -442,7 +457,7 @@
   }
   TR("round: glue launched, waiting for the decisions");
   if (h_gen) {
-    if ((rc = pl_presize_next())) return rc;
+    if ((rc = pl_presize_next()) || (rc = pl_queue_ahead())) return rc;
     if (!pl_wait_word(h_gen, want_gen, 0.25, pl_steady_now, nullptr, 1024)) {
       HIPCHK(c, hipStreamSynchronize(st));
       HIPCHK(c, hipMemsetAsync(c->pl_cnt.p, 0, 64, st));
@@ -452,6 +467,59 @@
   }
   TR("round: decisions on the host");
   h_dec = (const float *)c->pl_pin[2];
+  if (c->ra_debug && (rc = pl_ahead_seen())) return rc;
+  return MIND_OK;
+}
+
+int PlanRun::pl_queue_ahead() {
+  if (!ahead_on || !presized) return MIND_OK;
+  const size_t OBS = RB_T, Sb = (size_t)g.Bk * AIME_K;
+  nxt = cur_in < 0 ? 0 : cur_in ^ 1;
+  nxt_S = (int)Sb;
+  q = InLayout(Sb, a, l);
+  const size_t n_wpos = Sb * a * OBS * 2, n_wang = Sb * a * OBS;
+  w_pos = (float *)c->pl_win[nxt].p; w_ang = w_pos + n_wpos; w_vel = w_ang + n_wang;
+  d_in = (float *)c->pl_in[nxt].p;
+  const int *d_win = (const int *)((const char *)tabb->p + tab_bytes), *d_n = d_win + 3 * (size_t)6 * g.Bmax;
+  hipLaunchKernelGGL(k_aime_windows, dim3((unsigned)(Sb * a)), dim3(64), 0, st, prev_pos, prev_ang, prev_vel, (const float *)d_world, d_win, d_win, d_win, a,
+                     w_pos, w_ang, w_vel, AIME_K, d_in + q.cov, d_n);
+  RebaseArgs R = pl_rebase_args(d_in, q, 0, l);
+  R.pad_ones = 1;
+  R.pos = w_pos; R.ang = w_ang; R.vel = w_vel; R.pad = nullptr;
+  R.lane_ctrs0 = droot + ro.lc; R.lane_vecs0 = droot + ro.lv; R.travel0 = -1.f;
+  R.n_dev = d_n;
+  hipLaunchKernelGGL(k_aime_rebase, dim3((unsigned)Sb, 1 + RB_FEAT_BLOCKS(a)), dim3(RB_THREADS), 5 * a * sizeof(float), st, R);
+  HIPCHK(c, hipGetLastError());
+  ahead = true;
+  std::vector<int> sa(Sb, a), sl(Sb, l);
+  const PredChoice ch = pred_choose(c->pt, c->pair_prec, c->n_cu, c->side != nullptr, (int)Sb, sa.data(), sl.data());
+  const bool one_call = pl_chunk(a + l + 1, pred_edge_pair_bytes(c->pt, c->pair_prec), c->plan_chunk_mb, (int)Sb) >= (int)Sb;
+  if (ch.actor_form == PRED_ACTOR_MFMA && one_call && !(c->profiling && !c->ev_defer)) {
+    const size_t Ab = Sb * a, b_feat = Ab * 128 * sizeof(float);
+    int rc;
+    if (b_feat > c->actor_feat.cap) HIPCHK(c, hipStreamSynchronize(st));
+    if ((rc = ensure(c, c->actor_feat, b_feat))) return rc;
+    if (c->side) HIPCHK(c, hipEventRecord(c->ev_main, st));
+    pred_actor_mfma(c, ch.np, (int)Ab, st, d_in + q.actors, (int)Ab, (float *)c->actor_feat.p, nullptr, d_n + 1);
+    HIPCHK(c, hipGetLastError());
+    actor_queued = true;
+  }
+  TR("round: next round's head queued ahead");
+  return MIND_OK;
+}
+
+int PlanRun::pl_ahead_seen() {
+  if ((int)c->ra_seen.size() <= round_no) c->ra_seen.resize(round_no + 1);
+  std::vector<int> &v = c->ra_seen[round_no];
+  v.assign(2, 0);
+  v[0] = ahead_on ? (ahead ? 2 : 1) : 0;
+  if (!ahead_on) return MIND_OK;
+  const int *d_win = (const int *)((const char *)tabb->p + tab_bytes), *d_n = d_win + 3 * (size_t)6 * g.Bmax;
+  HIPCHK(c, hipStreamSynchronize(st));
+  HIPCHK(c, hipMemcpy(&v[1], d_n, sizeof(int), hipMemcpyDeviceToHost));
+  if (v[1] < 0 || v[1] > 6 * g.Bmax) return fail(c, MIND_ESTATE, "round_ahead: the device counted %d children of %d scenes", v[1], g.Bk);
+  v.resize(2 + 3 * (size_t)v[1]);
+  if (v[1] > 0) HIPCHK(c, hipMemcpy(&v[2], d_win, 3 * (size_t)v[1] * sizeof(int), hipMemcpyDeviceToHost));
   return MIND_OK;
 }
 
@@ -464,7 +532,9 @@
   int rc;
   if (b_in > c->pl_in[n].cap || b_win > c->pl_win[n].cap || b_rep > c->pl_lrep.cap) HIPCHK(c, hipStreamSynchronize(st));
   if ((rc = ensure(c, c->pl_in[n], b_in)) || (rc = ensure(c, c->pl_win[n], b_win)) || (rc = ensure(c, c->pl_lrep, b_rep))) return rc;
-  return pl_pin(c, 3, S * 28 * sizeof(float));
+  if ((rc = pl_pin(c, 3, S * 28 * sizeof(float)))) return rc;
+  presized = true;
+  return MIND_OK;
 }
 
 int PlanRun::pl_rebase_next() {
@@ -472,7 +542,12 @@
   const size_t OBS = RB_T, S = r.S, s0 = r.s0;
   const int Sm = r.Sm;
   int rc;
+  if (ahead) {
+    if ((int)S > nxt_S || Sm != (int)S) return fail(c, MIND_ESTATE, "round_ahead: a branch set of %d scenes behind a bound of %d", (int)S, nxt_S);
+    return MIND_OK;
+  }
   nxt = cur_in < 0 ? 0 : cur_in ^ 1;
+  nxt_S = (int)S;
   q = InLayout(S, a, l);
   if ((rc = ensure(c, c->pl_in[nxt], q.total * sizeof(float)))) return rc;
   const size_t n_wpos = S * a * OBS * 2, n_wang = S * a * OBS;
@@ -487,7 +562,7 @@
   const int *d_idx = tab_host ? (const int *)hi_ : (const int *)((const char *)tabb->p + tab_bytes);
   float *pos0 = w_pos + s0 * a * OBS * 2, *ang0 = w_ang + s0 * a * OBS, *vel0 = w_vel + s0 * a * OBS * 2;
   hipLaunchKernelGGL(k_aime_windows, dim3((unsigned)(Sm * a)), dim3(64), 0, st, prev_pos, prev_ang, prev_vel, (const float *)d_world, d_idx, d_idx + Sm,
-                     d_idx + 2 * Sm, a, pos0, ang0, vel0, AIME_K, d_in + q.cov + s0 * a);
+                     d_idx + 2 * Sm, a, pos0, ang0, vel0, AIME_K, d_in + q.cov + s0 * a, (const int *)nullptr);
   RebaseArgs R = pl_rebase_args(d_in, q, s0, l);
   R.pad_ones = 1;
   R.pos = pos0; R.ang = ang0; R.vel = vel0; R.pad = nullptr;
@@ -580,7 +655,8 @@
   }
   prev_pos = w_pos; prev_ang = w_ang; prev_vel = w_vel;
   cov_last_dev = d_in + q.cov;
-  cur_in = nxt;
+  cur_in = nxt; cur_S = nxt_S;
+  c->actor_ahead = ahead && actor_queued;
   return MIND_OK;
 }
 
@@ -700,7 +776,7 @@
   if (!c->ev_pl) HIPCHK(c, hipEventCreateWithFlags(&c->ev_pl, hipEventDisableTiming));
   if (!c->ev_tab) HIPCHK(c, hipEventCreateWithFlags(&c->ev_tab, hipEventDisableTiming));
   if (!c->pl_copy) HIPCHK(c, hipStreamCreateWithFlags(&c->pl_copy, hipStreamNonBlocking));
-  struct HookGuard { mind_ctx *c; ~HookGuard() { c->enc_pre = nullptr; c->enc_post = nullptr; } } hook_guard{c};
+  struct HookGuard { mind_ctx *c; ~HookGuard() { c->enc_pre = nullptr; c->enc_post = nullptr; c->actor_ahead = false; } } hook_guard{c};
   if ((rc = p.pl_root())) return rc;
   memset(out, 0, sizeof(*out));
   p.TR.t0 = std::chrono::steady_clock::now();
@@ -709,6 +785,7 @@
   c->ev_pending.clear(); c->ev_pool_used = 0;
   if (!c->lc.pending.empty() && (rc = lc_flush(c, false))) return rc;
   for (int k = 0; k < LC_KINDS; ++k) { c->lc_carry_ms[k] = 0.0; c->lc_carry_n[k] = 0; }
+  c->ra_seen.clear();
   for (int round = 0;; ++round) {
     PlErr e = p.book.begin_round(in->max_rounds, p.g);
     if (e) return p.fail_book(e);
@@ -716,6 +793,13 @@
     const float *h_dec;
     if ((rc = p.pl_round_buffers(round)) || (rc = p.pl_round_launch()) || (rc = p.pl_round_decisions(h_dec))) return rc;
     if ((e = p.book.round(h_dec, p.g.Bmax))) return p.fail_book(e);
+    if (c->ra_hint.size() <= (size_t)round) c->ra_hint.resize((size_t)round + 1, -1);
+    c->ra_hint[round] = p.book.rec.todo.empty() ? 0 : 1;
+    if (c->ra_debug && (size_t)round < c->ra_seen.size()) {
+      std::vector<int> &v = c->ra_seen[round];
+      v.push_back(p.book.rec.S);
+      v.insert(v.end(), p.book.rec.win.begin(), p.book.rec.win.end());
+    }
     if (p.book.rec.todo.empty()) break;
     if ((rc = p.pl_rebase_next())) return rc;
     if (p.dist && (rc = p.pl_exchange_next(round))) return rc;
@@ -791,6 +875,23 @@
 extern "C" int mind_debug_wait_word(const unsigned *word, unsigned want, double timeout_s, double (*clock)(void *), void *user, int spins_per_look) {
   if (!word || !(timeout_s >= 0.0) || spins_per_look <= 0) return MIND_EINVAL;
   return pl_wait_word(word, want, timeout_s, clock ? clock : pl_steady_now, user, (unsigned)spins_per_look) ? 1 : 0;
+}
+
+extern "C" int mind_debug_round_ahead(mind_ctx *c, int round, int *out, int cap) {
+  if (!c || round < 0 || cap < 0 || (cap > 0 && !out)) return MIND_EINVAL;
+  if ((size_t)round >= c->ra_seen.size()) return 0;
+  const std::vector<int> &v = c->ra_seen[round];
+  for (size_t i = 0; i < v.size() && (int)i < cap; ++i) out[i] = v[i];
+  return (int)v.size();
+}
+
+extern "C" int mind_debug_branch_scene(const float *sel, const unsigned *hit, int scene, int lscene, int a, int cur_t, int end_t, int parent_depth, int max_depth,
+                                       int pred_len, int *kids) {
+  if (!sel || !hit || !kids || a <= 0 || cur_t < 0 || end_t > AIME_T || cur_t > end_t || pred_len < 2 || pred_len > AIME_T) return MIND_EINVAL;
+  PlKid k[6];
+  const int n = plb_scene(sel, hit, scene, lscene, a, cur_t, end_t, parent_depth, max_depth, pred_len, k);
+  for (int j = 0; j < 6; ++j) { kids[5 * j] = k[j].what; kids[5 * j + 1] = k[j].end_t; memcpy(kids + 5 * j + 2, k[j].win, sizeof(k[j].win)); }
+  return n;
 }
 
 constexpr int PL_BOOK_HEADER = 16;
diff --git a/mind_amd/csrc/mind_hip.hip b/mind_amd/csrc/mind_hip.hip
--- a/mind_amd/csrc/mind_hip.hip
+++ b/mind_amd/csrc/mind_hip.hip
@@ -94,6 +94,11 @@
   DevBuf pl_cnt;
   bool root_head = true, round_head = true;
   std::function<int(hipStream_t)> enc_pre, enc_post;
+  int round_ahead = 1;
+  bool ra_debug = false;
+  bool actor_ahead = false;
+  std::vector<signed char> ra_hint;
+  std::vector<std::vector<int>> ra_seen;
   bool early_eval = true;
   int tab_host_max = 4096;
   bool tab_small = true;
@@ -317,6 +322,7 @@
   if (const char *we = getenv("MIND_ROOT_HEAD")) c->root_head = atoi(we) != 0;
   if (const char *we = getenv("MIND_ROUND_HEAD")) c->round_head = atoi(we) != 0;
   if (const char *we = getenv("MIND_UPLOAD_KERNEL_MAX")) c->upload_kernel_max = std::max(0, atoi(we));
+  if (const char *we = getenv("MIND_ROUND_AHEAD")) c->round_ahead = std::min(2, std::max(0, atoi(we)));
   const char *const il_env[][2] = {{"MIND_ILQR_CHUNK", "ilqr_chunk"}, {"MIND_ILQR_WGS", "ilqr_wgs"}, {"MIND_ILQR_SPEC_DERIV", "ilqr_spec_deriv"},
                                    {"MIND_ILQR_HOST_OUT_MAX", "ilqr_host_out_max"}, {"MIND_ILQR_SLOTS", "ilqr_slots"}};
   for (const auto &e : il_env)
@@ -414,6 +420,8 @@
   else if (n == "root_head") c->root_head = value != 0;
   else if (n == "round_head") c->round_head = value != 0;
   else if (n == "upload_kernel_max") c->upload_kernel_max = value < 0 ? 0 : value;
+  else if (n == "round_ahead") c->round_ahead = value < 0 ? 0 : (value > 2 ? 2 : value);
+  else if (n == "round_ahead_debug") c->ra_debug = value != 0;
   else if (n == "prof_clock") c->prof_clock = value < 0 ? 0 : (value > 2 ? 2 : value);
   else return fail(c, MIND_EINVAL, "mind_set_tuning: unknown knob '%s'", name);
   return MIND_OK;
@@ -919,7 +927,7 @@
   if (dev_src) {
     const int *di = (const int *)(d + o_idx);
     hipLaunchKernelGGL(k_aime_windows, dim3((unsigned)(S * a)), dim3(64), 0, st, prev, prev + prev_o_ang, prev + prev_o_vel, in->rows_dev,
-                       di, di + S, di + 2 * S, (int)a, d + o_pos, d + o_ang, d + o_vel, 1, (float *)nullptr);
+                       di, di + S, di + 2 * S, (int)a, d + o_pos, d + o_ang, d + o_vel, 1, (float *)nullptr, (const int *)nullptr);
   }
   c->rb_cur ^= 1; c->rb_gen += 1; c->rb_S = S; c->rb_a = a;
   if (out->gen) *out->gen = c->rb_gen;
diff --git a/mind_amd/csrc/predict.hip b/mind_amd/csrc/predict.hip
--- a/mind_amd/csrc/predict.hip
+++ b/mind_amd/csrc/predict.hip
@@ -296,6 +296,12 @@
   return MIND_OK;
 }
 
+static void pred_actor_mfma(mind_ctx *c, int np, int grid, hipStream_t st, const float *actors, int A, float *actor_feat, LcSlot *clk, const int *n_dev) {
+  if (np == 6) hipLaunchKernelGGL(k_actor_mfma<6>, dim3(grid), dim3(AM_T), mind_actor_mfma_lds_bytes(), st, actors, A, actor_feat, c->W.actorB, clk, n_dev);
+  else if (np == 3) hipLaunchKernelGGL(k_actor_mfma<3>, dim3(grid), dim3(AM_T), mind_actor_mfma_lds_bytes(), st, actors, A, actor_feat, c->W.actorB, clk, n_dev);
+  else hipLaunchKernelGGL(k_actor_mfma<1>, dim3(grid), dim3(AM_T), mind_actor_mfma_lds_bytes(), st, actors, A, actor_feat, c->W.actorB, clk, n_dev);
+}
+
 static int pred_actor_net(PredCall &p, LcSlot *clk) {
   mind_ctx *c = p.c;
   const PredChoice &ch = p.ch;
@@ -324,9 +330,7 @@
     break;
   }
   default:
-    if (ch.np == 6) hipLaunchKernelGGL(k_actor_mfma<6>, grid, dim3(AM_T), mind_actor_mfma_lds_bytes(), p.st, actors, A, actor_feat, c->W.actorB, clk);
-    else if (ch.np == 3) hipLaunchKernelGGL(k_actor_mfma<3>, grid, dim3(AM_T), mind_actor_mfma_lds_bytes(), p.st, actors, A, actor_feat, c->W.actorB, clk);
-    else hipLaunchKernelGGL(k_actor_mfma<1>, grid, dim3(AM_T), mind_actor_mfma_lds_bytes(), p.st, actors, A, actor_feat, c->W.actorB, clk);
+    pred_actor_mfma(c, ch.np, ch.actor_grid, p.st, actors, A, actor_feat, clk, nullptr);
   }
   return MIND_OK;
 }
@@ -336,8 +340,11 @@
   const mind_scene_batch *in = p.in;
   hipStream_t st = p.st, ss = p.ss;
   const int Bn = p.Bn, Ltot = p.Ltot, ntok = p.ts->ntok;
+  const bool act_ahead = c->actor_ahead;
+  c->actor_ahead = false;
+  if (act_ahead && p.ch.actor_form != PRED_ACTOR_MFMA) return fail(c, MIND_ESTATE, "round_ahead: ActorNet was queued ahead in another form than the call takes");
   if (c->side) {
-    HIPCHK(c, hipEventRecord(c->ev_main, st));
+    if (!act_ahead) HIPCHK(c, hipEventRecord(c->ev_main, st));
     HIPCHK(c, hipStreamWaitEvent(c->side, c->ev_main, 0));
   }
   const bool act_timed = c->profiling && !c->ev_defer;
@@ -354,7 +361,7 @@
   }
   c->last_actor_lw = 0; c->last_actor_launches = 1; c->last_actor_chunks = 1; c->actor_ms = 0.f;
   if (p.act_ev) HIPCHK(c, hipEventRecord(c->ev_act0, st));
-  if ((rc = pred_actor_net(p, act_clk))) return rc;
+  if (!act_ahead && (rc = pred_actor_net(p, act_clk))) return rc;
   if (p.act_ev) HIPCHK(c, hipEventRecord(c->ev_act1, st));
   if (c->enc_pre) {
     const std::function<int(hipStream_t)> pre = std::move(c->enc_pre);
```

After: 1864. About the same (-0.6%).
